# nmoehrle/mvs-texturing

Hardware: AMD Instinct MI355X
Metric: faces/sec through view-selection (data-cost + MRF) (higher is better)
Workload: dtype f32; 1 GPU; BASELINE config 3: displaced icosphere n=316 (1997120 faces), 200 Fibonacci-sphere views 2048x1536 RGB8, settings gmi/none/visibility-test (reference defaults); faces=1997120, views=200, nnz=88914367, sweeps=39, icm_iters=10, partition=library-hilbert-1, face_order_in=as built, msg_bits=8, max_labels=0

## Files before the change

include/mvs_viewsel_blocks.h:

```cpp
#ifndef MVS_VIEWSEL_BLOCKS_H
#define MVS_VIEWSEL_BLOCKS_H
#include "mvs_viewsel.h"
#ifdef __cplusplus
extern "C" {
#endif

mvs_status mvs_ctx_dc_get_max(mvs_ctx* ctx, float* dst_device);
mvs_status mvs_ctx_dc_set_max(mvs_ctx* ctx, const float* src_device);
mvs_status mvs_ctx_dc_get_histogram(mvs_ctx* ctx, uint32_t* dst_device);
mvs_status mvs_ctx_dc_set_histogram(mvs_ctx* ctx, const uint32_t* src_device);
mvs_status mvs_ctx_costs_export(mvs_ctx* ctx, uint32_t* counts_device, uint16_t* view_id_device, float* cost_device);

enum { MVS_MRF_MSG = 0, MVS_MRF_LAB = 1, MVS_MRF_GAIN = 2, MVS_MRF_BEST_LAB = 3,
       MVS_MRF_MSG_LAB = 4 };
mvs_status mvs_ctx_mrf_setup(mvs_ctx* ctx, const uint32_t* adj_ptr, const uint32_t* adj, int adj_on_device,
                             const mvs_mrf_params* params);
mvs_status mvs_ctx_mrf_sweep_phase(mvs_ctx* ctx, uint32_t phase, uint32_t node_begin, uint32_t node_end);
mvs_status mvs_ctx_mrf_setup_marked(mvs_ctx* ctx, const uint32_t* adj_ptr, const uint32_t* adj, int adj_on_device,
                                    const mvs_mrf_params* params, const uint8_t* marks_device);
mvs_status mvs_ctx_mrf_sweep_phase_part(mvs_ctx* ctx, uint32_t phase, uint32_t node_begin, uint32_t node_end, int part);
mvs_status mvs_ctx_mrf_sweep(mvs_ctx* ctx, uint32_t node_begin, uint32_t node_end);
mvs_status mvs_ctx_mrf_layout(mvs_ctx* ctx, uint32_t* in_off_host, uint64_t n_edges);
mvs_status mvs_ctx_mrf_gather(mvs_ctx* ctx, int which, const uint32_t* idx_device, uint64_t n, void* dst_device);
mvs_status mvs_ctx_mrf_scatter(mvs_ctx* ctx, int which, const uint32_t* idx_device, uint64_t n, const void* src_device);
mvs_status mvs_ctx_mrf_energy(mvs_ctx* ctx, int which_sel, uint32_t node_begin, uint32_t node_end, uint64_t* dst_device);
mvs_status mvs_ctx_mrf_keep_best(mvs_ctx* ctx);
mvs_status mvs_ctx_mrf_step(mvs_ctx* ctx, const uint64_t* energy_device);
mvs_status mvs_ctx_mrf_poll(mvs_ctx* ctx, uint32_t step, mvs_mrf_progress* out);
mvs_status mvs_ctx_mrf_icm_gain(mvs_ctx* ctx, uint32_t node_begin, uint32_t node_end);
mvs_status mvs_ctx_mrf_icm_apply(mvs_ctx* ctx, uint32_t node_begin, uint32_t node_end, uint32_t* moved_device);
mvs_status mvs_ctx_mrf_labels(mvs_ctx* ctx, uint32_t node_begin, uint32_t node_end, uint32_t* labels_device,
                              uint32_t* unseen_out);

#ifdef __cplusplus
}
#endif
#endif
```

mvs-texturing_amd/csrc/api.hip:

```cpp
#include "ctx.h"

#include <atomic>
#include <cmath>
#include <cstdio>
#include <cstdlib>
#include <cstring>
#include <chrono>
#include <mutex>
#include <string>
#include <thread>
#include <vector>

namespace mvs {
void dc_phase1(mvs_ctx* ctx, const mvs_settings* st);
void dc_phase2(mvs_ctx* ctx);
void dc_phase3(mvs_ctx* ctx, mvs_dc_stats* stats);
void undistort_image(mvs_ctx* ctx, const uint8_t* d_src, uint8_t* d_dst, int w, int h, double flen, double d0, double d1);
void dc_prune_labels(mvs_ctx* ctx, uint32_t kmax);
void dc_postprocess(mvs_ctx* ctx, uint32_t nf, uint32_t n_views, const uint32_t* h_ptr, const uint16_t* h_view_rev, const float* h_q_rev, const float* h_col_rev, const mvs_settings* st);
void mrf_setup(mvs_ctx* ctx, const mvs_mrf_params* params);
void mrf_sweep(mvs_ctx* ctx, uint32_t nb0, uint32_t ne0);
void mrf_energy(mvs_ctx* ctx, bool best, uint32_t nb0, uint32_t ne0, bool reduce = true);
void mrf_keep_best(mvs_ctx* ctx);
void mrf_exact_costs(mvs_ctx* ctx, uint32_t nb0, uint32_t ne0);
// ... 190 lines not shown
        for (unsigned k = 0; k < slots; ++k) {
            if (!buf[k]) MVS_HIP(hipHostMalloc((void**)&buf[k], SLOT, hipHostMallocPortable));
            if (!ev[k]) MVS_HIP(hipEventCreateWithFlags(&ev[k], hipEventDisableTiming));
        }
    }
    void release() {
        std::lock_guard<std::mutex> lock(m);
        for (unsigned k = 0; k < SLOTS; ++k) { if (ev[k]) (void)hipEventDestroy(ev[k]); if (buf[k]) (void)hipHostFree(buf[k]); ev[k] = nullptr; buf[k] = nullptr; used[k] = false; }
    }
};
constexpr int RING_DEVICES = 16;
UploadRing g_ring[RING_DEVICES];
unsigned upload_threads() {
    if (const char* e = getenv("MVS_UPLOAD_THREADS")) return (unsigned)std::max(1, std::min(atoi(e), (int)UploadRing::MAX_THREADS));
    return std::max(1u, std::min(UploadRing::MAX_THREADS, std::thread::hardware_concurrency() / 2));
}
void upload_through_ring(mvs_ctx* ctx, const std::vector<UploadPiece>& pieces) {
    if (ctx->device < 0 || ctx->device >= RING_DEVICES) throw StatusError(MVS_ERR_UNSUPPORTED, "upload ring: device index out of range");
    UploadRing& R = g_ring[ctx->device];
    std::lock_guard<std::mutex> lock(R.m);
    struct Chunk { const uint8_t* src; uint8_t* dst; size_t n; };
    std::vector<Chunk> chunks;
    for (const UploadPiece& p : pieces) for (size_t o = 0; o < p.bytes; o += UploadRing::SLOT) chunks.push_back(Chunk{p.src + o, p.dst + o, std::min(UploadRing::SLOT, p.bytes - o)});
    const unsigned T = (unsigned)std::max<size_t>(1, std::min<size_t>(upload_threads(), chunks.size()));
    R.ensure(2 * T);
    hipStream_t s = ctx->stream; const int device = ctx->device;
    struct Drain { hipStream_t s; UploadRing& R; ~Drain() { (void)hipStreamSynchronize(s); for (bool& u : R.used) u = false; } } drain{s, R};
    std::mutex em; std::string error; std::atomic<bool> failed{false};
    auto work = [&](unsigned t) {
        try {
            MVS_HIP(hipSetDevice(device));
            unsigned turn = 0;
            for (size_t c = t; c < chunks.size() && !failed.load(std::memory_order_relaxed); c += T, turn ^= 1u) {
                const unsigned k = 2 * t + turn;
                if (R.used[k]) MVS_HIP(hipEventSynchronize(R.ev[k]));
                memcpy(R.buf[k], chunks[c].src, chunks[c].n);
                MVS_HIP(hipMemcpyAsync(chunks[c].dst, R.buf[k], chunks[c].n, hipMemcpyHostToDevice, s));
                MVS_HIP(hipEventRecord(R.ev[k], s));
                R.used[k] = true;
            }
        } catch (const std::exception& e) { failed.store(true); std::lock_guard<std::mutex> l(em); if (error.empty()) error = e.what(); }
    };
    struct Joiner { std::vector<std::thread> th; ~Joiner() { for (auto& x : th) if (x.joinable()) x.join(); } } pool;
    pool.th.reserve(T);
    std::vector<unsigned> mine{0u};
    for (unsigned t = 1; t < T; ++t) {
        try { pool.th.emplace_back(work, t); } catch (const std::system_error&) { mine.push_back(t); }
    }
    for (unsigned t : mine) work(t);
    for (auto& x : pool.th) x.join();
    if (failed.load()) throw HipError("image upload: " + error);
}
}

extern "C" {

const char* mvs_last_error(void) { return g_last_error.c_str(); }

const char* mvs_status_string(mvs_status s) {
    switch (s) {
        case MVS_OK: return "ok";
        case MVS_ERR_INVALID: return "invalid argument";
        case MVS_ERR_TOO_MANY_FACES: return "Exeeded maximal number of faces";
        case MVS_ERR_TOO_MANY_VIEWS: return "Exeeded maximal number of views";
        case MVS_ERR_LABELING: return "Incorrect labeling";
        case MVS_ERR_HIP: return "HIP error";
        case MVS_ERR_STATE: return "invalid call order";
        case MVS_ERR_UNSUPPORTED: return "unsupported";
    }
    return "?";
}

void mvs_mrf_default_params(mvs_mrf_params* p) {
    p->max_sweeps = 200; p->min_sweeps = 20; p->window = 5; p->min_improvement = 0.005f;
    p->damping = 0.2f; p->rho = 0.8f; p->icm_iters = 50; p->region_rounds = 0;
}
void mvs_default_settings(mvs_settings* s) {
    s->data_term = MVS_DATA_TERM_GMI; s->outlier_removal = MVS_OUTLIER_NONE; s->geometric_visibility_test = 1;
}

mvs_status mvs_ctx_create(int device, mvs_ctx** out) {
    if (!out) return fail(MVS_ERR_INVALID, "out is null");
    *out = nullptr;
    MVS_API_BEGIN
    int n = 0;
    if (hipGetDeviceCount(&n) != hipSuccess || n <= 0) throw HipError("no HIP device available (this library has no CPU fallback)");
    if (device < 0 || device >= n) throw StatusError(MVS_ERR_INVALID, "bad device index");
    MVS_HIP(hipSetDevice(device));
    mvs_ctx* c = new mvs_ctx;
    c->device = device;
    MVS_HIP(hipStreamCreateWithFlags(&c->stream, hipStreamNonBlocking));
    c->own_stream = true;
    c->cos_limit = compute_cos_limit();
    if (const char* e = getenv("MVS_INFO_WAVE_AREA")) c->info_wave_area = std::max(0, atoi(e));
    if (const char* e = getenv("MVS_BVH_UPPER_MIN_FACES")) c->bvh_upper_min_faces = (uint32_t)std::max(0ll, atoll(e));
    c->counters.ensure(64);
    *out = c;
    MVS_API_END
}

void mvs_ctx_destroy(mvs_ctx* ctx) {
    if (!ctx) return;
    (void)hipSetDevice(ctx->device);
    (void)hipStreamSynchronize(ctx->stream);
    for (auto* b : ctx->own_rgb) delete b;
    mvs::gsl_release(ctx); mvs::texpatch_release(ctx); mvs::lsl_release(ctx);
    if (ctx->sweep_exec) (void)hipGraphExecDestroy(ctx->sweep_exec);
    if (ctx->cap_stream) (void)hipStreamDestroy(ctx->cap_stream);
    if (ctx->aux_stream) { (void)hipStreamSynchronize(ctx->aux_stream); (void)hipStreamDestroy(ctx->aux_stream); }
    if (ctx->ev_fork) (void)hipEventDestroy(ctx->ev_fork);
    if (ctx->ev_join) (void)hipEventDestroy(ctx->ev_join);
    if (ctx->h_kd_flags) (void)hipHostFree(ctx->h_kd_flags);
    if (ctx->h_icm) (void)hipHostFree(ctx->h_icm);
    if (ctx->h_rb) (void)hipHostFree(ctx->h_rb);
    if (ctx->h_seq) (void)hipHostFree(ctx->h_seq);
    if (ctx->h_ring) (void)hipHostFree(ctx->h_ring);
    if (ctx->own_stream && ctx->stream) (void)hipStreamDestroy(ctx->stream);
    delete ctx;
}

mvs_status mvs_ctx_set_stream(mvs_ctx* ctx, void* hip_stream) {
    if (!ctx) return fail(MVS_ERR_INVALID, "ctx is null");
    MVS_API_BEGIN
    MVS_HIP(hipStreamSynchronize(ctx->stream));
    if (ctx->own_stream && ctx->stream) MVS_HIP(hipStreamDestroy(ctx->stream));
    ctx->stream = (hipStream_t)hip_stream; ctx->own_stream = false;
    MVS_API_END
}

mvs_status mvs_ctx_synchronize(mvs_ctx* ctx) {
    if (!ctx) return fail(MVS_ERR_INVALID, "ctx is null");
    MVS_API_BEGIN
    MVS_HIP(hipStreamSynchronize(ctx->stream));
    MVS_API_END
}

mvs_status mvs_set_option(mvs_ctx* ctx, const char* name, int64_t value) {
    if (!ctx || !name) return fail(MVS_ERR_INVALID, "null argument");
    const std::string n(name);
    if (n == "count_rays") ctx->count_rays = value != 0;
    else if (n == "stats") ctx->stats = value != 0;
    else if (n == "verbose") ctx->verbose = value != 0;
    else if (n == "info_wave_area") ctx->info_wave_area = (int)std::max<int64_t>(0, std::min<int64_t>(value, 1 << 30));
    else if (n == "info_wave_area_words") ctx->info_wave_area_words = (int)std::max<int64_t>(1, std::min<int64_t>(value, 1 << 30));
    else if (n == "info_words") ctx->info_words = value != 0;
    else if (n == "info_cert_shift") ctx->info_cert_shift = (int)std::max<int64_t>(0, std::min<int64_t>(value, 40));
    else if (n == "max_labels") { if (value < 0 || value > 65535) return fail(MVS_ERR_INVALID, "max_labels: 0 (off) .. 65535"); ctx->max_labels = (int)value; }
    else if (n == "profile") ctx->profile = value != 0;
    else if (n == "prep_fused") ctx->prep_fused = value != 0;
    else if (n == "ray_xcd") ctx->ray_xcd = (int)value;
    else if (n == "mrf_xcd") ctx->mrf_xcd = (int)value;
    else if (n == "mrf_lag") ctx->mrf_lag = (int)value;
    else if (n == "mrf_force_generic") ctx->mrf_force_generic = value != 0;
    else if (n == "mrf_graph") ctx->mrf_graph = value != 0;
    else if (n == "mrf_blocks_per_cu") ctx->mrf_blocks_per_cu = std::max(0, (int)value);
    else if (n == "bvh_upper_min_faces") { ctx->kd_disabled = false; ctx->bvh_upper_min_faces = (uint32_t)std::max<int64_t>(0, std::min<int64_t>(value, 0xFFFFFFFFll)); ctx->order_pinned = false; }
    else if (n == "bvh_window") { ctx->kd_disabled = false; ctx->bvh_window = (uint32_t)std::max<int64_t>(0, std::min<int64_t>(value, 0x40000000)); ctx->order_pinned = false; }
    else if (n == "face_order") { ctx->face_order = value != 0 ? 1 : 0; ctx->order_pinned = false; }
    else return fail(MVS_ERR_INVALID, "unknown option " + n);
    return MVS_OK;
}

mvs_status mvs_ctx_get_profile(mvs_ctx* ctx, char* buf, size_t buf_size) {
    if (!ctx || !buf || buf_size < 3) return fail(MVS_ERR_INVALID, "null argument");
    MVS_API_BEGIN
    MVS_HIP(hipStreamSynchronize(ctx->stream));
    std::vector<std::string> names; std::vector<double> ms; std::vector<int> cnt;
    for (auto& sp : ctx->prof_spans) {
        float t = 0.0f;
        MVS_HIP(hipEventElapsedTime(&t, sp.a, sp.b));
        size_t k = 0;
        for (; k < names.size(); ++k) if (names[k] == sp.name) break;
        if (k == names.size()) { names.push_back(sp.name); ms.push_back(0.0); cnt.push_back(0); }
        ms[k] += t; cnt[k] += 1;
        if (sp.owns_a) ctx->prof_pool.push_back(sp.a);
        ctx->prof_pool.push_back(sp.b);
    }
    ctx->prof_spans.clear();
    std::string out = "{";
    for (size_t k = 0; k < names.size(); ++k) {
        char tmp[160];
        snprintf(tmp, sizeof(tmp), "%s\"%s\": [%.6f, %d]", k ? ", " : "", names[k].c_str(), ms[k], cnt[k]);
        out += tmp;
    }
    out += "}";
    if (out.size() + 1 > buf_size) throw StatusError(MVS_ERR_INVALID, "profile buffer too small");
    memcpy(buf, out.c_str(), out.size() + 1);
    MVS_API_END
}

mvs_status mvs_scene_set_mesh(mvs_ctx* ctx, const mvs_mesh* mesh, int on_device) {
    if (!ctx || !mesh || !mesh->verts || !mesh->faces || !mesh->face_normals) return fail(MVS_ERR_INVALID, "null argument");
    MVS_API_BEGIN
    MVS_HIP(hipSetDevice(ctx->device));
    const size_t NV = mesh->n_verts, F = mesh->n_faces;
    if (on_device) {
        ctx->d_verts = mesh->verts; ctx->d_faces = mesh->faces; ctx->d_normals = mesh->face_normals;
    } else {
        ctx->own_verts.ensure(3 * NV + 4); ctx->own_faces.ensure(3 * F + 4); ctx->own_normals.ensure(3 * F + 4);
        MVS_HIP(hipMemcpyAsync(ctx->own_verts.p, mesh->verts, 3 * NV * sizeof(float), hipMemcpyHostToDevice, ctx->stream));
        MVS_HIP(hipMemcpyAsync(ctx->own_faces.p, mesh->faces, 3 * F * sizeof(uint32_t), hipMemcpyHostToDevice, ctx->stream));
        MVS_HIP(hipMemcpyAsync(ctx->own_normals.p, mesh->face_normals, 3 * F * sizeof(float), hipMemcpyHostToDevice, ctx->stream));
        MVS_HIP(hipStreamSynchronize(ctx->stream));
        ctx->d_verts = ctx->own_verts.p; ctx->d_faces = ctx->own_faces.p; ctx->d_normals = ctx->own_normals.p;
    }
    ctx->n_verts = mesh->n_verts; ctx->n_faces = mesh->n_faces;
    ctx->face_begin = 0; ctx->face_end = mesh->n_faces;
    ctx->have_costs = false; ctx->dc_phase = 0;
    ctx->order_pinned = false; ctx->iv = nullptr; ctx->kd_disabled = false; ctx->kd_pending = 0;
    MVS_API_END
}

static mvs_status set_views_impl(mvs_ctx* ctx, const mvs_view* views, uint32_t n_views, int rgb_on_device, const mvs_image_source* src);
mvs_status mvs_scene_set_views(mvs_ctx* ctx, const mvs_view* views, uint32_t n_views, int rgb_on_device) { return set_views_impl(ctx, views, n_views, rgb_on_device, nullptr); }
mvs_status mvs_scene_set_views_from(mvs_ctx* ctx, const mvs_view* views, uint32_t n_views, const mvs_image_source* src) {
    if (!src || !src->acquire || !src->release) return fail(MVS_ERR_INVALID, "null argument");
    return set_views_impl(ctx, views, n_views, 0, src);
}
static mvs_status set_views_impl(mvs_ctx* ctx, const mvs_view* views, uint32_t n_views, int rgb_on_device, const mvs_image_source* src) {
    if (!ctx || (!views && n_views)) return fail(MVS_ERR_INVALID, "null argument");
    MVS_API_BEGIN
    MVS_HIP(hipSetDevice(ctx->device));
    if (rgb_on_device) { for (auto* b : ctx->own_rgb) delete b; ctx->own_rgb.clear(); }
    else { while (ctx->own_rgb.size() > n_views) { delete ctx->own_rgb.back(); ctx->own_rgb.pop_back(); } }
    ctx->h_views.assign(n_views, ViewParams{});
    struct Pinned {
        hipStream_t s; std::vector<void*> ptrs;
        ~Pinned() { if (ptrs.empty()) return; (void)hipStreamSynchronize(s); for (void* p : ptrs) (void)hipHostUnregister(p); }
    } pinned{ctx->stream, {}};
    UploadRoute route = rgb_on_device ? UploadRoute::Pageable : upload_route();
    if (src && route == UploadRoute::Register) route = UploadRoute::Ring;
    std::vector<UploadPiece> pieces;
    struct Held {
        const mvs_image_source* src; std::vector<uint32_t> views;
        void release_all() { for (uint32_t j : views) src->release(src->user, j); views.clear(); }
        ~Held() { if (src) release_all(); }
    } held{src, {}};
    const uint32_t in_flight = src ? std::max<uint32_t>(1u, src->max_in_flight ? src->max_in_flight : 4u) : 0u;
    auto flush_batch = [&]() {
        if (!pieces.empty()) upload_through_ring(ctx, pieces);
        pieces.clear();
        MVS_HIP(hipStreamSynchronize(ctx->stream));
        held.release_all();
    };
    for (uint32_t j = 0; j < n_views; ++j) {
        mvs_view v = views[j];
        if (src) {
            if (v.width < 2 || v.height < 2) throw StatusError(MVS_ERR_INVALID, "view " + std::to_string(j) + ": bad image");
            v.rgb = src->acquire(src->user, j);
            if (!v.rgb) throw StatusError(MVS_ERR_INVALID, "view " + std::to_string(j) + ": the image source has no image");
            held.views.push_back(j);
        }
        if (v.width < 2 || v.height < 2 || !v.rgb) throw StatusError(MVS_ERR_INVALID, "view " + std::to_string(j) + ": bad image");
        ViewParams& p = ctx->h_views[j];
        memcpy(p.pos, v.pos, sizeof(p.pos)); memcpy(p.viewdir, v.viewdir, sizeof(p.viewdir));
        memcpy(p.K, v.K, sizeof(p.K)); memcpy(p.w2c, v.w2c, sizeof(p.w2c));
        p.width = v.width; p.height = v.height;
        if (rgb_on_device) p.rgb = v.rgb;
        else {
            if (ctx->own_rgb.size() <= j) ctx->own_rgb.push_back(new DBuf<uint8_t>());
            auto* b = ctx->own_rgb[j];
            const size_t bytes = (size_t)v.width * v.height * 3;
            b->ensure(bytes + 16);
            p.rgb = b->p;
            if (route == UploadRoute::Ring && bytes >= (1u << 18)) { pieces.push_back(UploadPiece{v.rgb, b->p, bytes}); if (src && held.views.size() >= in_flight) flush_batch(); continue; }
            if (route == UploadRoute::Register && bytes >= (1u << 20) && hipHostRegister(const_cast<uint8_t*>(v.rgb), bytes, hipHostRegisterDefault) == hipSuccess) pinned.ptrs.push_back(const_cast<uint8_t*>(v.rgb));
            else (void)hipGetLastError();
            MVS_HIP(hipMemcpyAsync(b->p, v.rgb, bytes, hipMemcpyHostToDevice, ctx->stream));
            if (src && held.views.size() >= in_flight) flush_batch();
        }
    }
    if (src) flush_batch();
    if (!pieces.empty()) upload_through_ring(ctx, pieces);
    MVS_HIP(hipStreamSynchronize(ctx->stream));
    ctx->n_views = n_views;
    ctx->have_costs = false; ctx->dc_phase = 0;
    MVS_API_END
}

mvs_status mvs_scene_set_face_range(mvs_ctx* ctx, uint32_t begin, uint32_t end) {
    if (!ctx) return fail(MVS_ERR_INVALID, "ctx is null");
    if (begin > end || end > ctx->n_faces) return fail(MVS_ERR_INVALID, "bad face range");
    ctx->face_begin = begin; ctx->face_end = end;
    ctx->have_costs = false; ctx->dc_phase = 0;
    return MVS_OK;
}

mvs_status mvs_ctx_dc_phase1(mvs_ctx* ctx, const mvs_settings* settings) {
    if (!ctx || !settings) return fail(MVS_ERR_INVALID, "null argument");
    MVS_API_BEGIN
    MVS_HIP(hipSetDevice(ctx->device));
    dc_phase1(ctx, settings);
    MVS_API_END
}
mvs_status mvs_ctx_dc_phase2(mvs_ctx* ctx) {
    if (!ctx) return fail(MVS_ERR_INVALID, "ctx is null");
    MVS_API_BEGIN
    MVS_HIP(hipSetDevice(ctx->device));
    dc_phase2(ctx);
    MVS_API_END
}
mvs_status mvs_ctx_dc_phase3(mvs_ctx* ctx, mvs_dc_stats* stats) {
    if (!ctx) return fail(MVS_ERR_INVALID, "ctx is null");
    MVS_API_BEGIN
    MVS_HIP(hipSetDevice(ctx->device));
    dc_phase3(ctx, stats);
// ... 496 lines not shown
```

mvs-texturing_amd/csrc/ctx.h:

```cpp
#pragma once
#include <hip/hip_runtime.h>
#include <stdint.h>
#include <string.h>
#include <algorithm>
#include <functional>
#include <stdexcept>
#include <string>
#include <vector>

#include "../../include/mvs_viewsel.h"
#include "dmath.h"

namespace mvs {

struct HipError : std::runtime_error {
    explicit HipError(const std::string& m) : std::runtime_error(m) {}
};
struct StatusError : std::runtime_error {
    mvs_status st;
    StatusError(mvs_status s, const std::string& m) : std::runtime_error(m), st(s) {}
};

#define MVS_HIP(expr)                                                                          \
    do {                                                                                       \
// ... 48 lines not shown
    uint32_t pad_[7];
    __host__ __device__ float lo(int a, int c) const { return b[c][a]; }
    __host__ __device__ float hi(int a, int c) const { return b[c][3 + a]; }
};
static_assert(sizeof(Node4) == 128, "Node4 must be one 128-byte line");

struct BvhDev {
    const Node4* nodes;
    const float4* tris;
    uint32_t level_off[16];
    uint32_t level_cnt[16];
    int32_t top;
    uint32_t n_leaves;
};

struct ProfSpan { std::string name; hipEvent_t a, b; bool owns_a; };

struct MrfEdge {
    uint32_t in_off;
    uint32_t out_off;
    uint32_t kj;
};

struct alignas(16) NodeDesc {
    uint32_t rec;
    uint32_t id;
    uint32_t in_off[3];
    uint32_t out_off[3];
    uint32_t kk;
    uint32_t nbr[3];
};
static_assert(sizeof(NodeDesc) == 48, "NodeDesc must be 48 bytes");

struct GslDev;
struct TexPatchDev;
struct LslDev;

struct PatchTables {
    DBuf<int4> box; DBuf<float2> pc;
    DBuf<uint32_t> fcand, fidx, parent, off, len, alive, pscan, cand_pid, cand_pos, fpid, fpos, flags;
    DBuf<unsigned long long> merged; DBuf<ViewParams> views;
    uint32_t C = 0, n_patches = 0; uint64_t n_merged = 0;
};

}

struct mvs_ctx {
    int device = 0;
    hipStream_t stream = nullptr;
    bool own_stream = false;
    bool verbose = false;
    bool profile = false;
    std::vector<mvs::ProfSpan> prof_spans; std::vector<hipEvent_t> prof_pool;
    bool prep_fused = true;
    bool stats = false;
    bool count_rays = false;
    uint32_t* h_kd_flags = nullptr; int kd_pending = 0; bool kd_disabled = false;
    uint32_t* h_rb = nullptr; uint32_t* d_rb = nullptr; uint32_t rb_seq = 0;
    hipStream_t aux_stream = nullptr; hipEvent_t ev_fork = nullptr, ev_join = nullptr;
    uint32_t bvh_upper_min_faces = 1000000;
    uint32_t bvh_window = 262144;
    mvs::DBuf<float> kd_c[2][3]; mvs::DBuf<uint32_t> kd_id[2], kd_hist, kd_cursor, kd_tie, kd_pivot, kd_box;
    int ray_xcd = 1;
    int info_wave_area = 32;
    int info_wave_area_words = 384;
    bool info_words = true;
    int info_cert_shift = 0;
    uint32_t dc_stats_deferred = 0;
    int max_labels = 0;
    float cos_limit = 0.0f;

    uint32_t n_verts = 0, n_faces = 0, n_views = 0;
    uint32_t face_begin = 0, face_end = 0;
    const float* d_verts = nullptr; const uint32_t* d_faces = nullptr; const float* d_normals = nullptr;
    mvs::DBuf<float> own_verts, own_normals; mvs::DBuf<uint32_t> own_faces;
    std::vector<mvs::ViewParams> h_views;
    mvs::DBuf<mvs::ViewParams> d_views;
    std::vector<mvs::DBuf<uint8_t>*> own_rgb;
    mvs::DBuf<uint8_t> gmi_all;
    mvs::DBuf<uint8_t> lum_all;
    mvs::DBuf<uint32_t> mask_all;
    mvs::DBuf<uint32_t> mask_zero, mask_tmp;
    mvs::DBuf<uint32_t> msum_all;
    std::vector<size_t> gmi_off, mask_off, msum_off;
    mvs::DBuf<size_t> view_off;
    bool mesh_dirty = true, views_dirty = true;

    int face_order = 1;
    mvs::DBuf<float> i_verts, i_normals; mvs::DBuf<uint32_t> i_faces, f_perm, f_pos, f_tmp;
    const float* iv = nullptr; const uint32_t* ifc = nullptr; const float* inr = nullptr;
    bool mesh_ordered = false;
    bool order_pinned = false;
    const uint32_t* t_perm = nullptr; const uint32_t* t_pos = nullptr;
    mvs::DBuf<uint32_t> u_ptr, u_cnt; mvs::DBuf<uint16_t> u_view; mvs::DBuf<float> u_cost, u_q;
    bool u_valid = false, u_q_valid = false;
    mvs::DBuf<unsigned long long> fp_acc;
    mvs::HBuf<uint32_t> stage_ptr; mvs::HBuf<uint16_t> stage_view[2]; mvs::HBuf<float> stage_cost[2];

    mvs::DBuf<mvs::Node4> bvh_nodes; mvs::DBuf<float4> bvh_tris;
    mvs::DBuf<uint32_t> sort_k, sort_k2, sort_v, sort_v2; mvs::DBuf<char> sort_tmp;
    mvs::DBuf<float> lvl_box_a, lvl_box_b; mvs::DBuf<float> scene_box;
    mvs::BvhDev bvh{};
    mvs::DBuf<uint32_t> vf_ptr, vf_cursor, vf;
    mvs::DBuf<uint32_t> vperm, vpos;
    const uint32_t* tri_order = nullptr;

    mvs::DBuf<unsigned long long> pass_bits, need_bits, occl_bits, surv_bits;
    mvs::DBuf<uint32_t> pass_base;
    mvs::DBuf<uint32_t> pass_face;
    mvs::DBuf<unsigned long long> defer_bits; mvs::DBuf<uint32_t> defer_base; mvs::DBuf<uint2> defer_list; mvs::DBuf<uint32_t> rewalk_list;
    mvs::DBuf<float> pq;
    mvs::DBuf<float> pcol;
    mvs::DBuf<uint32_t> face_cnt, scan_tmp;
    mvs::DBuf<unsigned long long> counters;
    mvs::DBuf<float> max_q; mvs::DBuf<uint32_t> hist; mvs::DBuf<float> pctl;
    mvs::DBuf<uint32_t> pre_ptr; mvs::DBuf<uint16_t> pre_view; mvs::DBuf<float> pre_q; mvs::DBuf<float> pre_col;
    mvs::DBuf<uint8_t> pre_inl;
    mvs::DBuf<uint32_t> csr_ptr; mvs::DBuf<uint16_t> csr_view; mvs::DBuf<float> csr_cost; mvs::DBuf<float> csr_q;
    uint32_t csr_faces = 0, csr_views = 0; uint64_t csr_nnz = 0;
    const uint32_t* r_ptr = nullptr; const uint16_t* r_view = nullptr; const float* r_cost = nullptr;
    bool csr_q_valid = false;
    bool have_costs = false;
    mvs_settings dc_settings{}; mvs_dc_stats dc_stats{}; int dc_phase = 0;

    mvs::DBuf<unsigned long long> g_keys, g_keys2; mvs::DBuf<uint32_t> g_vals, g_vals2, g_pos, g_cnt, g_adj_ptr, g_adj, g_faces; mvs::DBuf<float> g_normals;
    uint64_t g_adj_entries = 0; bool have_adj = false;

    mvs::DBuf<uint32_t> p_label_ptr, p_comp_ptr, p_comp_faces, p_parent, p_root, p_state, p_flag, p_pos, p_roots, p_roots2, p_rlab, p_rlab2, p_adj_ptr, p_adj, p_labels;

    mvs::GslDev* gsl = nullptr; mvs::TexPatchDev* texpatch = nullptr; mvs::LslDev* lsl = nullptr;

    mvs::DBuf<uint32_t> rg_parent, rg_root, rg_size, rg_bestl, rg_lose, rg_flag, rg_pos, rg_cstart, rg_have, rg_cfirst, rg_name;
    mvs::DBuf<unsigned long long> rg_gain, rg_cur, rg_key, rg_key2, rg_ck, rg_sum; mvs::DBuf<long long> rg_cgain; mvs::DBuf<uint2> rg_cut;

    mvs::DBuf<uint32_t> m_adj_ptr, m_adj, a_stage_ptr, a_stage; const uint32_t* r_adj_ptr = nullptr; const uint32_t* r_adj = nullptr;
    uint32_t r_adj_edges = 0; bool r_adj_edges_known = false;
    mvs::DBuf<mvs::NodeDesc> m_desc; mvs::DBuf<uint8_t> m_ident; mvs::DBuf<uint32_t> m_rec; uint64_t m_rec_words = 0; int mrf_blocks_per_cu = 0 , mrf_xcd = 1;
    mvs::DBuf<mvs::MrfEdge> m_edge; mvs::DBuf<uint32_t> m_size, m_rev ; mvs::DBuf<uint16_t> m_map;
    mvs::DBuf<uint8_t> m_msg_a;
    mvs::DBuf<uint32_t> m_sel, m_sel2, m_cand; mvs::DBuf<float> m_gain;
    mvs::DBuf<uint32_t> m_lab; mvs::DBuf<float> m_cost;
    uint32_t m_stride = 0;
    bool exact_valid = false; uint32_t exact_nb = 0, exact_ne = 0;
    uint32_t* b_sel = nullptr; uint32_t* b_lab = nullptr; float* b_cost = nullptr; bool best_resolved = false;
    mvs::DBuf<unsigned long long> m_energy; mvs::DBuf<uint32_t> m_moved; mvs::DBuf<uint32_t> m_alist; bool icm_dirty_valid = false;
    uint32_t m_n_adj = 0;
    uint32_t m_energy_blocks = 0;
    bool m_energy_from_sweep = false;
    uint64_t m_total = 0; uint32_t m_kmax = 0, m_degmax = 0;
    mvs::DBuf<uint32_t> m_colour, m_perm, m_tmp_a, m_tmp_b, m_tmp_c, m_sub; mvs::DBuf<uint8_t> m_cls; uint32_t m_colours = 0, m_n_fast = 0; std::vector<uint32_t> m_sub_begin;
    const uint32_t* m_colour_in = nullptr;
    const uint8_t* m_bnd = nullptr;
    int mrf_force_generic = 0;
    uint32_t m_range_nb = 0, m_range_ne = 0; std::vector<uint32_t> m_range_q;
    uint32_t m_sweep_no = 0;
    mvs_mrf_params m_params{};
    static constexpr uint32_t RING = 16;
    static constexpr uint32_t ICM_RING = 8;
    uint32_t* h_icm = nullptr; uint32_t* d_icm = nullptr; uint32_t icm_seq = 0;
    mvs::DBuf<mvs_mrf_progress> m_state; mvs::DBuf<unsigned long long> m_hist; mvs::DBuf<uint32_t> m_ctl;
    int mrf_graph = 1; hipStream_t cap_stream = nullptr; hipGraphExec_t sweep_exec = nullptr; uint32_t graph_launches = 0, graph_updates = 0, graph_instantiations = 0;
    mvs_mrf_progress* h_ring = nullptr; mvs_mrf_progress* d_ring = nullptr ; uint32_t steps_issued = 0; int mrf_lag = 1;
    uint32_t* h_seq = nullptr; uint32_t* d_seq = nullptr; uint32_t seq_base = 0;
};

namespace mvs {
struct Prof {
    mvs_ctx* c; size_t idx; bool on;
    Prof(mvs_ctx* ctx, const char* name) : c(ctx), idx(0), on(ctx->profile) {
        if (!on) return;
        auto get = [&]() { hipEvent_t e; if (!c->prof_pool.empty()) { e = c->prof_pool.back(); c->prof_pool.pop_back(); } else { MVS_HIP(hipEventCreate(&e)); } return e; };
        ProfSpan sp{name, get(), get(), true};
        MVS_HIP(hipEventRecord(sp.a, c->stream));
        idx = c->prof_spans.size(); c->prof_spans.push_back(sp);
    }
    void end() { if (on) { MVS_HIP(hipEventRecord(c->prof_spans[idx].b, c->stream)); on = false; } }
    ~Prof() { if (on) (void)hipEventRecord(c->prof_spans[idx].b, c->stream); }
};
struct ProfChain {
    mvs_ctx* c; hipEvent_t prev; bool on;
    static hipEvent_t get(mvs_ctx* c) { hipEvent_t e; if (!c->prof_pool.empty()) { e = c->prof_pool.back(); c->prof_pool.pop_back(); } else { MVS_HIP(hipEventCreate(&e)); } return e; }
    explicit ProfChain(mvs_ctx* ctx) : c(ctx), prev(nullptr), on(ctx->profile) {}
    void begin() { if (on && !prev) { prev = get(c); MVS_HIP(hipEventRecord(prev, c->stream)); first = true; } }
    void mark(const char* name) {
        if (!on) return;
        begin();
        hipEvent_t e = get(c);
        MVS_HIP(hipEventRecord(e, c->stream));
        c->prof_spans.push_back(ProfSpan{name, prev, e, first});
        first = false; prev = e;
    }
    bool first = false;
};
struct RoctxRange { explicit RoctxRange(const char* name); ~RoctxRange(); bool on; };
int default_device();
enum { MRF_PART_ALL = 0, MRF_PART_BOUNDARY = 1, MRF_PART_INTERIOR = 2 };
void ensure_report_ring(mvs_ctx* ctx);
void report_u32(mvs_ctx* ctx, const uint32_t* d_src, uint32_t* d_dst, uint32_t seq_slot, uint32_t seq);
void wait_report(mvs_ctx* ctx, uint32_t seq_slot, uint32_t seq);
int icm_rounds(mvs_ctx* ctx, int max_rounds, const uint32_t* d_moved, const std::function<void(int)>& round);
constexpr uint32_t MRF_DAMP_PERIOD = 4;
void read_words(mvs_ctx* ctx, const void* d_src, void* out, uint32_t n_words);
void read_block(mvs_ctx* ctx, const void* d_src, void* out, size_t bytes);
void exclusive_scan_u32(mvs_ctx* ctx, const uint32_t* in, uint32_t* out, size_t n, uint32_t* d_total);
uint64_t sum_u32(mvs_ctx* ctx, const uint32_t* in, size_t n);
void gsl_release(mvs_ctx* ctx);
void texpatch_release(mvs_ctx* ctx);
void lsl_release(mvs_ctx* ctx);
void patch_check_inputs(mvs_ctx* ctx, PatchTables& T, const uint32_t* d_labels, const char* who);
void build_patch_tables(mvs_ctx* ctx, PatchTables& T, const uint32_t* d_adj_ptr, const uint32_t* d_adj, const uint32_t* d_labels, const char* who);
}
```

mvs-texturing_amd/csrc/dmath.h:

```cpp
#pragma once
#include <stdint.h>
#include <math.h>
#include <float.h>
#include <string.h>

#if defined(__HIPCC__)
#define MVS_HD __host__ __device__ __forceinline__
#else
#define MVS_HD inline
#endif

namespace mvs {

struct V3 { float x, y, z; };
struct V2 { float x, y; };

MVS_HD V3 operator+(V3 a, V3 b) { return {a.x + b.x, a.y + b.y, a.z + b.z}; }
MVS_HD V3 operator-(V3 a, V3 b) { return {a.x - b.x, a.y - b.y, a.z - b.z}; }
MVS_HD V3 operator/(V3 a, float s) { return {a.x / s, a.y / s, a.z / s}; }
MVS_HD float dot(V3 a, V3 b) { return (a.x * b.x + a.y * b.y) + a.z * b.z; }
MVS_HD float norm(V3 a) { return sqrtf(dot(a, a)); }
MVS_HD V3 normalized(V3 a) { return a / norm(a); }
MVS_HD V3 cross(V3 a, V3 b) {
    return {a.y * b.z - a.z * b.y, a.z * b.x - a.x * b.z, a.x * b.y - a.y * b.x};
// ... 250 lines not shown
    if (DATA_TERM == 1) {
        if (num_samples > 0) {
            gmi = foot_gmi_term(gmi, num_samples, s.area);
        } else {
            const double g1 = (double)linear_at(gimg, w, h, 1, s.p1.x, s.p1.y, 0) / 255.0;
            const double g2 = (double)linear_at(gimg, w, h, 1, s.p2.x, s.p2.y, 0) / 255.0;
            const double g3 = (double)linear_at(gimg, w, h, 1, s.p3.x, s.p3.y, 0) / 255.0;
            gmi = (((g1 + g2) + g3) / 3.0) * (double)s.area;
        }
    }
    if (OUTLIER) {
        if (num_samples > 0) {
            out->mean_color[0] = foot_mean(col0, num_samples);
            out->mean_color[1] = foot_mean(col1, num_samples);
            out->mean_color[2] = foot_mean(col2, num_samples);
        } else {
            for (int i = 0; i < 3; ++i) {
                const double c1 = (double)linear_at(image, w, h, 3, s.p1.x, s.p1.y, i) / 255.0;
                const double c2 = (double)linear_at(image, w, h, 3, s.p2.x, s.p2.y, i) / 255.0;
                const double c3 = (double)linear_at(image, w, h, 3, s.p3.x, s.p3.y, i) / 255.0;
                out->mean_color[i] = (float)(((c1 + c2) + c3) / 3.0);
            }
        }
    }
    out->quality = (DATA_TERM == 0) ? s.area : (float)gmi;
}

MVS_HD bool foot_value_certified(double q, double dn, double up) { return (float)(q * dn) == (float)(q * up); }
template <int DATA_TERM, bool OUTLIER>
MVS_HD bool foot_sums_certified(const FootSetup& s, uint32_t num_samples, double col0, double col1, double col2, double gmi, int shift) {
    if (num_samples == 0) return true;
    const double eps = ldexp((double)((num_samples + 13u) & ~1u), -53 + shift), dn = 1.0 - eps, up = 1.0 + eps;
    bool ok = true;
    if (DATA_TERM == 1) ok = foot_value_certified(foot_gmi_term(gmi, num_samples, s.area), dn, up);
    if (OUTLIER) ok = ok && foot_value_certified(col0 / (double)num_samples, dn, up) && foot_value_certified(col1 / (double)num_samples, dn, up) &&
                      foot_value_certified(col2 / (double)num_samples, dn, up);
    return ok;
}

MVS_HD uint32_t bytes_sum4(uint32_t v, uint32_t acc) {
#if defined(__HIP_DEVICE_COMPILE__)
    return __builtin_amdgcn_sad_u8(v, 0u, acc);
#else
    return acc + (v & 0xFFu) + ((v >> 8) & 0xFFu) + ((v >> 16) & 0xFFu) + (v >> 24);
#endif
}
template <int ROWS = 2>
MVS_HD void foot_walk_gmi_words(const ViewParams& view, const FootSetup& s, uint32_t* num_samples, uint32_t* gmi_sum) {
    const uint8_t* gimg = view.gmi;
    const int w = view.width;
    uint32_t n = 0, g = 0;
    const int y_end = (int)ceilf(s.aabb_max_y);
    for (int y = (int)floorf(s.aabb_min_y); y < y_end; y += ROWS) {
        int xb[ROWS], xe[ROWS], x0[ROWS];
        const uint8_t* row0 = gimg + (size_t)y * w;
        bool more = false;
#pragma unroll
        for (int r = 0; r < ROWS; ++r) {
            if (y + r >= y_end || !foot_row(s, y + r, &xb[r], &xe[r]) || xe[r] <= xb[r]) { xb[r] = 0; xe[r] = 0; }
            x0[r] = xb[r] - (int)(reinterpret_cast<uintptr_t>(row0 + r * w + xb[r]) & 3u);
            if (xe[r] <= xb[r]) x0[r] = xe[r];
            more = more || x0[r] < xe[r];
        }
        while (more) {
            uint32_t v[ROWS];
#pragma unroll
            for (int r = 0; r < ROWS; ++r) v[r] = (x0[r] < xe[r]) ? *reinterpret_cast<const uint32_t*>(row0 + r * w + x0[r]) : 0u;
            more = false;
#pragma unroll
            for (int r = 0; r < ROWS; ++r) {
                if (x0[r] < xe[r]) {
                    const int lo = xb[r] > x0[r] ? xb[r] - x0[r] : 0, hi = xe[r] - x0[r] < 4 ? xe[r] - x0[r] : 4;
                    const uint32_t m = (hi >= 4 ? 0xFFFFFFFFu : ((1u << (8 * hi)) - 1u)) & ~((1u << (8 * lo)) - 1u);
                    g = bytes_sum4(v[r] & m, g);
                    n += (uint32_t)(hi - lo);
                }
                x0[r] += 4;
                more = more || x0[r] < xe[r];
            }
        }
    }
    *num_samples = n; *gmi_sum = g;
}
MVS_HD bool foot_words_fit(const FootSetup& s) {
    return ((s.aabb_max_y - s.aabb_min_y) + 2.0f) * ((s.aabb_max_x - s.aabb_min_x) + 2.0f) < 16777216.0f;
}

constexpr float FOOT_DEFERRED = -1.0f;

template <int DATA_TERM, bool OUTLIER>
MVS_HD void face_info(const ViewParams& view, V3 v1, V3 v2, V3 v3, FaceInfoOut* out, float defer_area = INFINITY,
                      const double* u8_over_255 = nullptr ) {
    FootSetup s;
    foot_setup(view, v1, v2, v3, s);
    out->quality = 0.0f;
    out->mean_color[0] = out->mean_color[1] = out->mean_color[2] = 0.0f;
    if (s.area < FLT_EPSILON) return;

    uint32_t num_samples = 0;
    double col0 = 0.0, col1 = 0.0, col2 = 0.0, gmi = 0.0;
    const int w = view.width;
    const uint8_t* image = view.rgb;
    const uint8_t* gimg = view.gmi;
    const bool sampling_necessary = (DATA_TERM != 0) || OUTLIER;

    if (sampling_necessary && s.area > 0.5f) {
        if (s.area > defer_area) { out->quality = FOOT_DEFERRED; return; }
        foot_edges(s);
        const float y_end = ceilf(s.aabb_max_y);
        for (int y = (int)floorf(s.aabb_min_y); (float)y < y_end; ++y) {
            int xb, xe;
            if (!foot_row(s, y, &xb, &xe)) continue;
            for (int x = xb; x < xe; ++x) {
                if (!s.fast && !foot_inside(s, x, y)) continue;
                const size_t pix = (size_t)x + (size_t)y * w;
                if (OUTLIER) {
                    const uint8_t c0 = image[pix * 3 + 0], c1 = image[pix * 3 + 1], c2 = image[pix * 3 + 2];
                    col0 += u8_over_255 ? u8_over_255[c0] : (double)c0 / 255.0;
                    col1 += u8_over_255 ? u8_over_255[c1] : (double)c1 / 255.0;
                    col2 += u8_over_255 ? u8_over_255[c2] : (double)c2 / 255.0;
                }
                if (DATA_TERM == 1) { const uint8_t g = gimg[pix]; gmi += u8_over_255 ? u8_over_255[g] : (double)g / 255.0; }
                ++num_samples;
            }
        }
    }
    foot_finish<DATA_TERM, OUTLIER>(view, s, num_samples, col0, col1, col2, gmi, out);
}

MVS_HD void rgb_to_ycbcr(float* v) {
    const float r = v[0], g = v[1], b = v[2];
    v[0] = r * 0.299f + g * 0.587f + b * 0.114f;
    v[1] = r * -0.168736f + g * -0.331264f + b * 0.5f + 0.5f;
    v[2] = r * 0.5f + g * -0.418688f + b * -0.081312f + 0.5f;
}

MVS_HD uint8_t luminance_u8(uint8_t r, uint8_t g, uint8_t b) {
    return (uint8_t)(0.30 * (double)r + (double)(0.59f * (float)g) + (double)(0.11f * (float)b));
}
MVS_HD uint8_t isqrt_clamp255(int n) {
    const float m = (float)(n < 255 * 255 ? n : 255 * 255) + 0.5f;
#if defined(__HIP_DEVICE_COMPILE__)
    return (uint8_t)(int)__builtin_amdgcn_sqrtf(m);
#else
    return (uint8_t)(int)sqrtf(m);
#endif
}

MVS_HD uint32_t hist_bin(float value, float maxv, uint32_t num_bins) {
    const float clamped = smax(0.0f, smin(maxv, value));
    return (uint32_t)floorf(((clamped - 0.0f) / (maxv - 0.0f)) * (float)(num_bins - 1));
}

inline float host_cos_limit() {
    const double limit = 75.0f * (3.14159265358979323846264338327950288 / 180.0);
    auto f = [](uint32_t u) { float x; memcpy(&x, &u, 4); return x; };
    auto culled = [&](uint32_t u) { return (double)acosf(f(u)) > limit; };
    uint32_t lo = 0x3E000000u , hi = 0x3F000000u ;
    while (hi - lo > 1) { const uint32_t mid = lo + (hi - lo) / 2; if (culled(mid)) lo = mid; else hi = mid; }
    for (uint32_t k = 1; k <= 4096; ++k) if (!culled(hi - k) || culled(hi + k - 1)) return NAN;
    return f(hi);
}

}
```

mvs-texturing_amd/csrc/dmath_host.cpp:

```cpp
#include "dmath.h"
#include <vector>
#include <cstring>

using namespace mvs;

extern "C" {

struct dmh_view {
    float pos[3], viewdir[3], K[9], w2c[16];
    int32_t width, height;
    const uint8_t* rgb;
    const uint8_t* gmi;
    const uint32_t* mask;
};

static ViewParams to_vp(const dmh_view* v) {
    ViewParams p;
    memcpy(p.pos, v->pos, sizeof(p.pos)); memcpy(p.viewdir, v->viewdir, sizeof(p.viewdir));
    memcpy(p.K, v->K, sizeof(p.K)); memcpy(p.w2c, v->w2c, sizeof(p.w2c));
    p.width = v->width; p.height = v->height; p.mask_stride = (v->width + 31) / 32;
    p.rgb = v->rgb; p.gmi = v->gmi; p.mask = v->mask; p.msum = nullptr; p.msum_stride = 0;
    return p;
}

float dmh_cos_limit(void) { return host_cos_limit(); }

void dmh_cull_all(const dmh_view* views, uint32_t n_views, const float* verts, const uint32_t* faces, const float* normals,
                  uint32_t n_faces, float cos_limit, int8_t* reasons) {
    for (uint32_t j = 0; j < n_views; ++j) {
        const ViewParams vp = to_vp(views + j);
        for (uint32_t f = 0; f < n_faces; ++f) {
            const uint32_t* fv = faces + 3 * (size_t)f;
            const V3 v1 = {verts[3 * fv[0]], verts[3 * fv[0] + 1], verts[3 * fv[0] + 2]};
            const V3 v2 = {verts[3 * fv[1]], verts[3 * fv[1] + 1], verts[3 * fv[1] + 2]};
            const V3 v3 = {verts[3 * fv[2]], verts[3 * fv[2] + 1], verts[3 * fv[2] + 2]};
            const V3 n = {normals[3 * f], normals[3 * f + 1], normals[3 * f + 2]};
            reasons[(size_t)f * n_views + j] = (int8_t)cull_pair(vp, v1, v2, v3, n, cos_limit);
        }
    }
}

void dmh_cull_pairs(const dmh_view* base, uint32_t n, const float* pos, const float* viewdir, const float* tri9, const float* normal,
                    float cos_limit, int8_t* out) {
    for (uint32_t i = 0; i < n; ++i) {
        ViewParams vp = to_vp(base);
        for (int a = 0; a < 3; ++a) { vp.pos[a] = pos[3 * i + a]; vp.viewdir[a] = viewdir[3 * i + a]; }
        const float* t = tri9 + 9 * (size_t)i;
        const V3 v1 = {t[0], t[1], t[2]}, v2 = {t[3], t[4], t[5]}, v3 = {t[6], t[7], t[8]}, nr = {normal[3 * i], normal[3 * i + 1], normal[3 * i + 2]};
        const V3 centre = ((v1 + v2) + v3) / 3.0f;
        out[2 * i] = (int8_t)cull_pair(vp, v1, v2, v3, nr, cos_limit);
        out[2 * i + 1] = (int8_t)cull_pair_prefiltered(vp, v1, v2, v3, nr, centre, cos_limit);
    }
}

void dmh_face_info(const dmh_view* view, int data_term, int outlier, const float* v1, const float* v2, const float* v3,
                   float* quality, float* ycbcr) {
    const ViewParams vp = to_vp(view);
    FaceInfoOut fi;
    const V3 a = {v1[0], v1[1], v1[2]}, b = {v2[0], v2[1], v2[2]}, c = {v3[0], v3[1], v3[2]};
    if (data_term == 1) { if (outlier) face_info<1, true>(vp, a, b, c, &fi); else face_info<1, false>(vp, a, b, c, &fi); }
    else { if (outlier) face_info<0, true>(vp, a, b, c, &fi); else face_info<0, false>(vp, a, b, c, &fi); }
    *quality = fi.quality;
    if (outlier) rgb_to_ycbcr(fi.mean_color);
    ycbcr[0] = fi.mean_color[0]; ycbcr[1] = fi.mean_color[1]; ycbcr[2] = fi.mean_color[2];
}

int dmh_ray_any_hit(const float* verts, const uint32_t* faces, uint32_t n_faces, uint32_t n_verts, const float* origin, const float* view_pos) {
    float lo[3] = {INFINITY, INFINITY, INFINITY}, hi[3] = {-INFINITY, -INFINITY, -INFINITY};
    for (uint32_t v = 0; v < n_verts; ++v)
        for (int a = 0; a < 3; ++a) { lo[a] = fminf(lo[a], verts[3 * (size_t)v + a]); hi[a] = fmaxf(hi[a], verts[3 * (size_t)v + a]); }
    const Ray r = make_ray(V3{origin[0], origin[1], origin[2]}, V3{view_pos[0], view_pos[1], view_pos[2]}, scene_pad(lo, hi));
    for (uint32_t f = 0; f < n_faces; ++f) {
        const uint32_t* fv = faces + 3 * (size_t)f;
        const V3 a = {verts[3 * fv[0]], verts[3 * fv[0] + 1], verts[3 * fv[0] + 2]};
        const V3 b = {verts[3 * fv[1]], verts[3 * fv[1] + 1], verts[3 * fv[1] + 2]};
        const V3 c = {verts[3 * fv[2]], verts[3 * fv[2] + 1], verts[3 * fv[2] + 2]};
        if (ray_tri(r, a, b - a, c - a)) return 1;
    }
    return 0;
}

void dmh_gradient_magnitude(const uint8_t* rgb, int w, int h, uint8_t* gmi) {
    for (int y = 0; y < h; ++y)
        for (int x = 0; x < w; ++x) {
            if (y == 0 || y == h - 1 || x == 0 || x == w - 1) { gmi[(size_t)y * w + x] = 0; continue; }
            int l[3][3];
            for (int dy = -1; dy <= 1; ++dy)
                for (int dx = -1; dx <= 1; ++dx) {
                    const uint8_t* p = rgb + ((size_t)(y + dy) * w + (x + dx)) * 3;
                    l[dy + 1][dx + 1] = luminance_u8(p[0], p[1], p[2]);
                }
            const int sx = (l[0][2] - l[0][0]) + 2 * (l[1][2] - l[1][0]) + (l[2][2] - l[2][0]);
            const int sy = (l[2][0] - l[0][0]) + 2 * (l[2][1] - l[0][1]) + (l[2][2] - l[0][2]);
            gmi[(size_t)y * w + x] = isqrt_clamp255(sx * sx + sy * sy);
        }
}

uint32_t dmh_hist_bin(float value, float maxv) { return hist_bin(value, maxv, 10000u); }

void dmh_foot_cert_trials(uint64_t seed, uint32_t trials, uint32_t max_n, int shift, uint64_t* out) {
    uint64_t n_cert = 0, n_mis = 0, n_bad = 0;
#pragma omp parallel for schedule(dynamic, 64) reduction(+ : n_cert, n_mis, n_bad)
    for (uint32_t t = 0; t < trials; ++t) {
        uint64_t x = seed * 0x9E3779B97F4A7C15ull + (uint64_t)t * 0xD1B54A32D192ED03ull + 1ull;
        auto rnd = [&]() { x ^= x << 13; x ^= x >> 7; x ^= x << 17; return x; };
        const uint32_t n = 33u + (uint32_t)(rnd() % (max_n - 32u));
        const uint32_t lo = (uint32_t)(rnd() % 200u), span = 1u + (uint32_t)(rnd() % (256u - lo));
        std::vector<uint8_t> px(4 * (size_t)n);
        for (auto& p : px) p = (uint8_t)(lo + rnd() % span);
        FootSetup s{}; s.area = 0.5f * (float)n * (0.8f + 0.4f * (float)(rnd() % 1000u) / 1000.0f);
        uint64_t S[4] = {0, 0, 0, 0};
        for (uint32_t k = 0; k < n; ++k) for (int c = 0; c < 4; ++c) S[c] += px[4 * (size_t)k + c];
        const double C[4] = {(double)S[0] / 255.0, (double)S[1] / 255.0, (double)S[2] / 255.0, (double)S[3] / 255.0};
        const bool cert = foot_sums_certified<1, true>(s, n, C[0], C[1], C[2], C[3], shift);
        const float qi = (float)foot_gmi_term(C[3], n, s.area), m0 = foot_mean(C[0], n), m1 = foot_mean(C[1], n), m2 = foot_mean(C[2], n);
        bool mis = false;
        for (int order = 0; order < 3; ++order) {
            double a[4] = {0.0, 0.0, 0.0, 0.0};
            for (uint32_t k = 0; k < n; ++k) {
                const uint32_t i = order == 0 ? k : order == 1 ? n - 1 - k : (uint32_t)(((uint64_t)k * 7919u) % n);
                for (int c = 0; c < 4; ++c) a[c] += (double)px[4 * (size_t)i + c] / 255.0;
            }
            mis = mis || (float)foot_gmi_term(a[3], n, s.area) != qi || foot_mean(a[0], n) != m0 || foot_mean(a[1], n) != m1 || foot_mean(a[2], n) != m2;
        }
        n_cert += cert; n_mis += mis; n_bad += (cert && mis);
    }
    out[0] = n_cert; out[1] = n_mis; out[2] = n_bad; out[3] = trials;
}

uint64_t dmh_isqrt_mismatches(uint32_t n_max) {
    uint64_t bad = 0;
    uint32_t k = 0;
    for (uint32_t n = 0; n < n_max; ++n) {
        while ((uint64_t)(k + 1) * (k + 1) <= n) ++k;
        bad += isqrt_clamp255((int)n) != (uint8_t)(k < 255u ? k : 255u);
    }
    return bad;
}

void dmh_word_walk_trials(uint64_t seed, uint32_t trials, uint64_t* out) {
    uint64_t n_fast = 0, n_bad = 0, n_px = 0, n_over = 0;
#pragma omp parallel for schedule(dynamic, 64) reduction(+ : n_fast, n_bad, n_px, n_over)
    for (uint32_t t = 0; t < trials; ++t) {
        uint64_t x = seed * 0x9E3779B97F4A7C15ull + (uint64_t)t * 0xD1B54A32D192ED03ull + 1ull;
        auto rnd = [&]() { x ^= x << 13; x ^= x >> 7; x ^= x << 17; return x; };
        auto unit = [&]() { return (float)(rnd() % 1000003u) / 1000003.0f; };
        const int w = 33 + (int)(rnd() % 90u), h = 20 + (int)(rnd() % 60u);
        std::vector<uint8_t> buf((size_t)w * h + 16);
        for (auto& b : buf) b = (uint8_t)(rnd() >> 11);
        ViewParams vp; memset(&vp, 0, sizeof(vp));
        vp.width = w; vp.height = h; vp.gmi = buf.data() + 8;
        FootSetup s{};
        const float cx = 2.0f + unit() * (float)(w - 4), cy = 2.0f + unit() * (float)(h - 4), r = 0.6f + unit() * unit() * 30.0f;
        auto clampf = [](float v, float lo, float hi) { return v < lo ? lo : (v > hi ? hi : v); };
        V2* p[3] = {&s.p1, &s.p2, &s.p3};
        for (int k = 0; k < 3; ++k) { p[k]->x = clampf(cx + (2.0f * unit() - 1.0f) * r, 0.0f, (float)w - 1.01f); p[k]->y = clampf(cy + (2.0f * unit() - 1.0f) * r, 0.0f, (float)h - 1.01f); }
        foot_setup_px(s);
        if (s.area <= 0.5f) continue;
        foot_edges(s);
        if (!s.fast) continue;
        uint32_t n0 = 0, g0 = 0;
        const float y_end = ceilf(s.aabb_max_y);
        for (int y = (int)floorf(s.aabb_min_y); (float)y < y_end; ++y) {
            int xb, xe;
            if (!foot_row(s, y, &xb, &xe)) continue;
            for (int xx = xb; xx < xe; ++xx) { g0 += vp.gmi[(size_t)xx + (size_t)y * w]; ++n0; }
        }
        uint32_t n[3], g[3];
        foot_walk_gmi_words<2>(vp, s, &n[0], &g[0]); foot_walk_gmi_words<3>(vp, s, &n[1], &g[1]); foot_walk_gmi_words<4>(vp, s, &n[2], &g[2]);
        ++n_fast; n_px += n0;
        for (int k = 0; k < 3; ++k) n_bad += (n[k] != n0 || g[k] != g0);
        n_over += (double)n0 > ((double)s.aabb_max_y - s.aabb_min_y + 2.0) * ((double)s.aabb_max_x - s.aabb_min_x + 2.0);
    }
    out[0] = n_fast; out[1] = n_bad; out[2] = n_px; out[3] = n_over;
}

}
```

mvs-texturing_amd/csrc/k_mrf.hip:

```cpp
#include "ctx.h"
#include <rocprim/rocprim.hpp>
#include <atomic>

namespace mvs {

namespace {

constexpr uint16_t MAP_NONE = 0xFFFF;
constexpr uint32_t MSG_BASE = MVS_MRF_MSG_BASE;

typedef uint8_t msg_t;
struct MsgQ { float scale, step; };
__device__ __forceinline__ MsgQ msg_q(float lam) { return MsgQ{255.0f / lam, lam / 255.0f}; }
template <class T> __device__ __forceinline__ T ld_off(const void* base, uint32_t byte_off) { return *reinterpret_cast<const T*>(reinterpret_cast<const char*>(base) + byte_off); }
template <class T> __device__ __forceinline__ void st_off(void* base, uint32_t byte_off, T v) { *reinterpret_cast<T*>(reinterpret_cast<char*>(base) + byte_off) = v; }
__device__ __forceinline__ float min_raw(float a, float b) { float r; asm("v_min_f32 %0, %1, %2" : "=v"(r) : "v"(a), "v"(b)); return r; }
template <bool DAMP>
__device__ __forceinline__ uint32_t msg_pack_s(float raw_s, float alpha, float old_code, uint32_t byte, uint32_t word) {
    return __builtin_amdgcn_cvt_pk_u8_f32(DAMP ? __builtin_fmaf(old_code, alpha, raw_s) : raw_s, byte, word);
}
template <bool DAMP>
__device__ __forceinline__ uint32_t msg_pack(float raw, float oms, float alpha, float old_code, uint32_t byte, uint32_t word) {
    const float v = DAMP ? __builtin_fmaf(old_code, alpha, raw * oms) : raw * oms;
    return __builtin_amdgcn_cvt_pk_u8_f32(v, byte, word);
// ... 105 lines not shown
                                uint32_t* __restrict__ maxes , uint32_t* __restrict__ rev) {
    const uint32_t i = blockIdx.x * blockDim.x + threadIdx.x;
    uint32_t k = 0, deg = 0;
    if (i < F) {
        k = col_ptr[i + 1] - col_ptr[i];
        const uint32_t e0 = adj_ptr[i], e1 = adj_ptr[i + 1];
        deg = e1 - e0;
        uint32_t kmx = k;
        for (uint32_t eb = e0; eb < e1; eb += 4) {
            uint32_t j[4], kj[4], r0[4], r1[4], head[4][4];
#pragma unroll
            for (int q = 0; q < 4; ++q) j[q] = (eb + q < e1) ? adj[eb + q] : i;
#pragma unroll
            for (int q = 0; q < 4; ++q) { kj[q] = col_ptr[j[q] + 1] - col_ptr[j[q]]; r0[q] = adj_ptr[j[q]]; r1[q] = adj_ptr[j[q] + 1]; }
#pragma unroll
            for (int q = 0; q < 4; ++q)
#pragma unroll
                for (int t = 0; t < 4; ++t) head[q][t] = (r0[q] + t < r1[q]) ? adj[r0[q] + t] : 0xFFFFFFFFu;
#pragma unroll
            for (int q = 0; q < 4; ++q) {
                if (eb + q >= e1) continue;
                const uint32_t e = eb + q;
                size[e] = (k > 0 && kj[q] > 0) ? ((k + pad_mask) & ~pad_mask) : 0u;
                if (k > 0) kmx = max(kmx, kj[q]);
                uint32_t r = 0xFFFFFFFFu;
#pragma unroll
                for (int t = 3; t >= 0; --t) r = (head[q][t] == i) ? r0[q] + t : r;
                if (r == 0xFFFFFFFFu) { uint32_t rr = r0[q] + 4u; while (rr < r1[q] && adj[rr] != i) ++rr; if (rr < r1[q]) r = rr; }
                rev[e] = r;
            }
        }
        cls[i] = (uint8_t)mrf_node_class(kmx, deg, force_generic);
    }
    for (int o = 32; o > 0; o >>= 1) { k = max(k, (uint32_t)__shfl_xor(k, o, 64)); deg = max(deg, (uint32_t)__shfl_xor(deg, o, 64)); }
    if ((threadIdx.x & 63) == 0) {
        if (k > __hip_atomic_load(&maxes[0], __ATOMIC_RELAXED, __HIP_MEMORY_SCOPE_AGENT)) atomicMax(&maxes[0], k);
        if (deg > __hip_atomic_load(&maxes[1], __ATOMIC_RELAXED, __HIP_MEMORY_SCOPE_AGENT)) atomicMax(&maxes[1], deg);
    }
}

__device__ __forceinline__ uint32_t mrf_hash32(uint32_t x) { x ^= x >> 16; x *= 0x7feb352dU; x ^= x >> 15; x *= 0x846ca68bU; x ^= x >> 16; return x; }
__device__ __forceinline__ bool mrf_key_less(uint32_t a, uint32_t b) { const uint32_t ha = mrf_hash32(a), hb = mrf_hash32(b); return ha != hb ? ha < hb : a < b; }
constexpr uint32_t NO_COLOUR = 0xFFFFFFFFu;
__global__ void mrf_colour_init_kernel(uint32_t* __restrict__ colour, uint32_t* __restrict__ iota, uint32_t F) {
    const uint32_t i = blockIdx.x * blockDim.x + threadIdx.x;
    if (i < F) { colour[i] = NO_COLOUR; iota[i] = i; }
}
__global__ void mrf_colour_round_kernel(const uint32_t* __restrict__ adj_ptr, const uint32_t* __restrict__ adj, const uint32_t* __restrict__ orig, uint32_t F,
                                        uint32_t* colour, uint32_t* __restrict__ pending) {
    const uint32_t i = blockIdx.x * blockDim.x + threadIdx.x;
    if (i >= F) return;
    if (__hip_atomic_load(colour + i, __ATOMIC_RELAXED, __HIP_MEMORY_SCOPE_AGENT) != NO_COLOUR) return;
    unsigned long long used = 0ull;
    bool ready = true;
    const uint32_t oi = orig ? orig[i] : i;
    const uint32_t e0 = adj_ptr[i], e1 = adj_ptr[i + 1];
    for (uint32_t eb = e0; eb < e1 && ready; eb += 4) {
        uint32_t j[4], oj[4], cj[4];
#pragma unroll
        for (int t = 0; t < 4; ++t) j[t] = (eb + t < e1) ? adj[eb + t] : i;
#pragma unroll
        for (int t = 0; t < 4; ++t) { oj[t] = orig ? orig[j[t]] : j[t]; cj[t] = __hip_atomic_load(colour + j[t], __ATOMIC_RELAXED, __HIP_MEMORY_SCOPE_AGENT); }
#pragma unroll
        for (int t = 0; t < 4; ++t) {
            if (j[t] == i || !mrf_key_less(oj[t], oi)) continue;
            if (cj[t] == NO_COLOUR) ready = false; else used |= 1ull << cj[t];
        }
    }
    if (ready) {
        if (used == ~0ull) { pending[1] = 1u; used = 0ull; }
        __hip_atomic_store(colour + i, (uint32_t)__builtin_ctzll(~used), __ATOMIC_RELAXED, __HIP_MEMORY_SCOPE_AGENT);
    } else *pending = 1u;
}
constexpr uint32_t N_SUB = 320;
constexpr uint32_t SUB_GENERIC = 256;
constexpr uint32_t N_KEY = 2 * N_SUB;
__global__ void mrf_sortkey_kernel(const uint32_t* __restrict__ colour, const uint8_t* __restrict__ cls, const uint8_t* __restrict__ bnd, uint32_t F, uint32_t* __restrict__ key) {
    const uint32_t i = blockIdx.x * blockDim.x + threadIdx.x;
    if (i < F) { const uint32_t c = colour[i], k = cls[i]; key[i] = 2u * ((k == CLS_GENERIC) ? SUB_GENERIC + c : 4u * c + k) + ((bnd && bnd[i]) ? 0u : 1u); }
}
__global__ void mrf_sub_begin_kernel(const uint32_t* __restrict__ sorted, uint32_t F, uint32_t* __restrict__ sub_begin) {
    const uint32_t c = blockIdx.x * blockDim.x + threadIdx.x;
    if (c > N_KEY) return;
    uint32_t lo = 0, hi = F;
    while (lo < hi) { const uint32_t mid = (lo + hi) >> 1; if (sorted[mid] < c) lo = mid + 1; else hi = mid; }
    sub_begin[c] = lo;
}
__global__ void mrf_sub_range_kernel(const uint32_t* __restrict__ perm, const uint32_t* __restrict__ sub_begin,
                                     uint32_t nb, uint32_t ne, uint32_t* __restrict__ out) {
    const uint32_t c = blockIdx.x * blockDim.x + threadIdx.x;
    if (c >= N_KEY) return;
    const uint32_t cb = sub_begin[c], ce = sub_begin[c + 1];
    uint32_t lo = cb, hi = ce;
    while (lo < hi) { const uint32_t mid = (lo + hi) >> 1; if (perm[mid] < nb) lo = mid + 1; else hi = mid; }
    out[2 * c] = lo;
    hi = ce;
    while (lo < hi) { const uint32_t mid = (lo + hi) >> 1; if (perm[mid] < ne) lo = mid + 1; else hi = mid; }
    out[2 * c + 1] = lo;
}
constexpr int MAX_LAYOUT_COLOURS = 8;
__global__ void mrf_nodesize_kernel(const uint32_t* __restrict__ perm, const uint32_t* __restrict__ colour, const uint32_t* __restrict__ adj_ptr,
                                    const uint32_t* __restrict__ adj, const uint32_t* __restrict__ size, const uint32_t* __restrict__ rev, uint32_t F, uint32_t n_col,
                                    uint32_t* __restrict__ nsz) {
    const uint32_t q = blockIdx.x * blockDim.x + threadIdx.x;
    if (q > F) return;
    uint32_t acc[MAX_LAYOUT_COLOURS];
#pragma unroll
    for (int b = 0; b < MAX_LAYOUT_COLOURS; ++b) acc[b] = 0;
    if (q < F) {
        const uint32_t j = perm[q];
        const uint32_t ra = adj_ptr[j], rz = adj_ptr[j + 1];
        for (uint32_t rb = ra; rb < rz; rb += 4) {
            uint32_t i[4], e[4], b[4], sz[4];
#pragma unroll
            for (int t = 0; t < 4; ++t) { const bool on = rb + t < rz; i[t] = on ? adj[rb + t] : j; e[t] = on ? rev[rb + t] : 0xFFFFFFFFu; }
#pragma unroll
            for (int t = 0; t < 4; ++t) { b[t] = (n_col > 1) ? colour[i[t]] : 0u; sz[t] = (e[t] != 0xFFFFFFFFu) ? size[e[t]] : 0u; }
#pragma unroll
            for (int t = 0; t < 4; ++t)
#pragma unroll
                for (int c = 0; c < MAX_LAYOUT_COLOURS; ++c) acc[c] += ((uint32_t)c == b[t]) ? sz[t] : 0u;
        }
    }
#pragma unroll
    for (int b = 0; b < MAX_LAYOUT_COLOURS; ++b) if ((uint32_t)b < n_col) nsz[(size_t)b * (F + 1) + q] = acc[b];
}
__global__ void mrf_inoff_kernel(const uint32_t* __restrict__ perm, const uint32_t* __restrict__ colour, const uint32_t* __restrict__ adj_ptr,
                                 const uint32_t* __restrict__ adj, const uint32_t* __restrict__ size, const uint32_t* __restrict__ rev, const uint32_t* __restrict__ noff,
                                 uint32_t F, uint32_t n_col, uint32_t* __restrict__ in_off) {
    const uint32_t q = blockIdx.x * blockDim.x + threadIdx.x;
    if (q >= F) return;
    const uint32_t j = perm[q];
    uint32_t off[MAX_LAYOUT_COLOURS];
#pragma unroll
    for (int b = 0; b < MAX_LAYOUT_COLOURS; ++b) off[b] = ((uint32_t)b < n_col) ? noff[(size_t)b * (F + 1) + q] : 0u;
    const uint32_t ra = adj_ptr[j], rz = adj_ptr[j + 1];
    for (uint32_t rb = ra; rb < rz; rb += 4) {
        uint32_t i[4], e[4], b[4], sz[4];
#pragma unroll
        for (int t = 0; t < 4; ++t) { const bool on = rb + t < rz; i[t] = on ? adj[rb + t] : j; e[t] = on ? rev[rb + t] : 0xFFFFFFFFu; }
#pragma unroll
        for (int t = 0; t < 4; ++t) { b[t] = (n_col > 1) ? colour[i[t]] : 0u; sz[t] = (e[t] != 0xFFFFFFFFu) ? size[e[t]] : 0u; }
#pragma unroll
        for (int t = 0; t < 4; ++t) {
            if (e[t] == 0xFFFFFFFFu) continue;
            uint32_t o = 0;
#pragma unroll
            for (int c = 0; c < MAX_LAYOUT_COLOURS; ++c) { if ((uint32_t)c == b[t]) { o = off[c]; off[c] += sz[t]; } }
            in_off[e[t]] = o;
        }
    }
}

__global__ void mrf_edge_kernel(const uint32_t* __restrict__ col_ptr, const uint32_t* __restrict__ adj_ptr, const uint32_t* __restrict__ adj,
                                uint32_t F, const uint32_t* __restrict__ in_off, const uint32_t* __restrict__ size, const uint32_t* __restrict__ rev, MrfEdge* __restrict__ edge) {
    const uint32_t i = blockIdx.x * blockDim.x + threadIdx.x;
    if (i >= F) return;
    const uint32_t e0 = adj_ptr[i], e1 = adj_ptr[i + 1];
    for (uint32_t eb = e0; eb < e1; eb += 4) {
        uint32_t j[4], r[4], io[4], sz[4], oo[4], kj[4];
#pragma unroll
        for (int t = 0; t < 4; ++t) { const bool on = eb + t < e1; j[t] = on ? adj[eb + t] : i; r[t] = on ? rev[eb + t] : 0xFFFFFFFFu; io[t] = on ? in_off[eb + t] : 0u; sz[t] = on ? size[eb + t] : 0u; }
#pragma unroll
        for (int t = 0; t < 4; ++t) { oo[t] = (r[t] != 0xFFFFFFFFu) ? in_off[r[t]] : 0u; kj[t] = col_ptr[j[t] + 1] - col_ptr[j[t]]; }
#pragma unroll
        for (int t = 0; t < 4; ++t) {
            if (eb + t >= e1) continue;
            const bool has = r[t] != 0xFFFFFFFFu;
            MrfEdge m;
            m.in_off = MSG_BASE + io[t];
            m.out_off = has ? MSG_BASE + oo[t] : 0u;
            m.kj = (sz[t] > 0 && has) ? kj[t] : 0u;
            edge[eb + t] = m;
        }
    }
}

constexpr uint32_t MAP_TILE = 256;
__global__ void __launch_bounds__(256) mrf_map_kernel(const uint32_t* __restrict__ col_ptr, const uint16_t* __restrict__ view_id, const uint32_t* __restrict__ adj_ptr,
                               const uint32_t* __restrict__ adj, uint32_t F, const MrfEdge* __restrict__ edge, const uint8_t* __restrict__ cls, uint16_t* __restrict__ map) {
    __shared__ uint16_t s_l[16][MAP_TILE];
    const uint32_t i = (blockIdx.x * blockDim.x + threadIdx.x) >> 4;
    const uint32_t gl = threadIdx.x & 15;
    if (i >= F) return;
    uint16_t* tile = s_l[threadIdx.x >> 4];
    const uint32_t p0 = col_ptr[i], K = col_ptr[i + 1] - p0;
    for (uint32_t e = adj_ptr[i]; e < adj_ptr[i + 1]; ++e) {
        const MrfEdge m = edge[e];
        if (m.kj == 0 || cls[adj[e]] != CLS_GENERIC) continue;
        const uint32_t q0 = col_ptr[adj[e]];
        const bool in_lds = m.kj <= MAP_TILE;
        if (in_lds) for (uint32_t t = gl; t < m.kj; t += 16) tile[t] = view_id[q0 + t];
        for (uint32_t t = gl; t < K; t += 16) {
            const uint16_t key = view_id[p0 + t];
            uint32_t lo = 0, hi = m.kj;
            if (in_lds) { while (lo < hi) { const uint32_t mid = (lo + hi) >> 1; if (tile[mid] < key) lo = mid + 1; else hi = mid; } }
            else { while (lo < hi) { const uint32_t mid = (lo + hi) >> 1; if (view_id[q0 + mid] < key) lo = mid + 1; else hi = mid; } }
            const uint16_t found = (lo < m.kj) ? (in_lds ? tile[lo] : view_id[q0 + lo]) : (uint16_t)0;
            map[m.in_off + t] = (lo < m.kj && found == key) ? (uint16_t)lo : MAP_NONE;
        }
    }
}

constexpr uint32_t REC_BASE = 256;
constexpr float COST_SCALE = 65535.0f;
__device__ __forceinline__ uint32_t cost_code(float c) { return (uint32_t)(c * COST_SCALE + 0.5f); }
__device__ __forceinline__ float cost_value(uint32_t code) { return (float)code * (1.0f / 65535.0f); }
__device__ __forceinline__ uint32_t label_position(const uint16_t* __restrict__ view_id, uint32_t p0, uint32_t K, uint32_t l) {
    uint32_t lo = 0, hi = K;
    const uint32_t key = l - 1u;
    while (lo < hi) { const uint32_t mid = (lo + hi) >> 1; if ((uint32_t)view_id[p0 + mid] < key) lo = mid + 1; else hi = mid; }
    return lo < K ? lo : K - 1u;
}

__global__ void __launch_bounds__(256) mrf_ident_kernel(const uint32_t* __restrict__ col_ptr, const uint16_t* __restrict__ view_id, const uint32_t* __restrict__ adj_ptr,
                                                        const uint32_t* __restrict__ adj, uint32_t F, const MrfEdge* __restrict__ edge, const uint8_t* __restrict__ cls,
                                                        uint8_t* __restrict__ ident) {
    const uint32_t i = (blockIdx.x * blockDim.x + threadIdx.x) >> 4;
    const uint32_t gl = threadIdx.x & 15;
    if (i >= F || cls[i] == CLS_GENERIC) return;
    const uint32_t p0 = col_ptr[i], K = col_ptr[i + 1] - p0;
    const uint32_t e0 = adj_ptr[i], e1 = adj_ptr[i + 1];
    for (uint32_t e = e0; e < e1; e += 3) {
        uint32_t kj[3], q0[3];
#pragma unroll
        for (int k = 0; k < 3; ++k) {
            const bool on = e + k < e1;
            kj[k] = on ? edge[e + k].kj : 0u;
            q0[k] = col_ptr[on ? adj[e + k] : i];
        }
        uint32_t same = 0;
#pragma unroll
        for (int k = 0; k < 3; ++k) same |= (kj[k] != 0u && kj[k] == K) ? (1u << k) : 0u;
        if (same) {
            for (uint32_t t = gl; t < K; t += 16) {
                const uint32_t v = view_id[p0 + t];
#pragma unroll
                for (int k = 0; k < 3; ++k)
                    if ((same >> k) & 1u) { if (view_id[q0[k] + t] != v) same &= ~(1u << k); }
            }
            for (int o = 8; o > 0; o >>= 1) same &= __shfl_xor(same, o, 16);
        }
        if (gl < 3 && e + gl < e1 && kj[gl] != 0u) ident[e + gl] = (uint8_t)((same >> gl) & 1u);
    }
}
__global__ void mrf_recsize_kernel(const uint32_t* __restrict__ col_ptr, const uint32_t* __restrict__ adj_ptr, const MrfEdge* __restrict__ edge,
                                   const uint8_t* __restrict__ ident, const uint8_t* __restrict__ cls, const uint32_t* __restrict__ perm, uint32_t F,
                                   uint32_t* __restrict__ rsz, uint32_t* __restrict__ qpos) {
    const uint32_t q = blockIdx.x * blockDim.x + threadIdx.x;
    if (q > F) return;
    uint32_t w = 0;
    if (q < F) {
        const uint32_t i = perm[q], K = col_ptr[i + 1] - col_ptr[i];
        qpos[i] = q;
        if (K && cls[i] != CLS_GENERIC) {
            w = (K + 3u) & ~3u;
            const bool w8 = cls[i] == 1u;
            const uint32_t e0 = adj_ptr[i], e1 = adj_ptr[i + 1];
            for (uint32_t eb = e0; eb < e1; eb += 4) {
                uint32_t kj[4], id[4];
#pragma unroll
                for (int t = 0; t < 4; ++t) { const bool on = eb + t < e1; kj[t] = on ? edge[eb + t].kj : 0u; id[t] = on ? ident[eb + t] : 1u; }
#pragma unroll
                for (int t = 0; t < 4; ++t) if (kj[t] && !id[t]) w += w8 ? 2u * ((kj[t] + 7u) >> 3) : (kj[t] + 3u) >> 2;
            }
            w = (w + 3u) & ~3u;
        }
    }
    rsz[q] = w;
}
__global__ void __launch_bounds__(256) mrf_record_kernel(const uint32_t* __restrict__ col_ptr, const uint16_t* __restrict__ view_id, const float* __restrict__ cost,
                                                         const uint32_t* __restrict__ adj_ptr, const uint32_t* __restrict__ adj, const MrfEdge* __restrict__ edge,
                                                         const uint8_t* __restrict__ ident, const uint8_t* __restrict__ cls, const uint32_t* __restrict__ qpos, const uint32_t* __restrict__ roff,
                                                         uint32_t F, uint32_t* __restrict__ rec) {
    __shared__ uint16_t s_l[16][256];
    const uint32_t i = (blockIdx.x * blockDim.x + threadIdx.x) >> 4;
    const uint32_t gl = threadIdx.x & 15;
    if (i >= F) return;
    const uint32_t p0 = col_ptr[i], K = col_ptr[i + 1] - p0;
    const uint32_t ci = cls[i];
    if (K == 0 || ci == CLS_GENERIC) return;
    const bool w8 = ci == 1u;
    const uint32_t rs = w8 ? 8u : 8u << ci, none_byte = w8 ? 64u : (ci < 3u ? 4u * rs : 0xFFu);
    const uint32_t lmask = w8 ? 7u : 3u, lshift = w8 ? 3u : 2u;
    const uint32_t q = qpos[i];
    uint16_t* tile = s_l[threadIdx.x >> 4];
    uint32_t* out = rec + REC_BASE + roff[q];
    const uint32_t K4 = (K + 3u) & ~3u;
    const uint32_t e0 = adj_ptr[i], deg = adj_ptr[i + 1] - e0;
    uint32_t kj3[3], q03[3];
    {
        uint32_t kj[3], idn[3], nb[3];
#pragma unroll
        for (uint32_t d = 0; d < 3; ++d) { const bool on = d < deg; kj[d] = on ? edge[e0 + d].kj : 0u; idn[d] = on ? (uint32_t)ident[e0 + d] : 1u; nb[d] = on ? adj[e0 + d] : i; }
#pragma unroll
        for (uint32_t d = 0; d < 3; ++d) { kj3[d] = (kj[d] != 0u && idn[d] == 0u) ? kj[d] : 0u; q03[d] = col_ptr[nb[d]]; }
    }
    for (uint32_t t = gl; t < K4; t += 16) {
        uint32_t w = 0u;
        if (t < K) { const uint32_t v = view_id[p0 + t]; tile[t] = (uint16_t)v; w = (cost_code(cost[p0 + t]) << 16) | v; }
        out[t] = w;
    }
    uint32_t pos = K4;
#pragma unroll
    for (uint32_t d = 0; d < 3; ++d) {
        const uint32_t kj = kj3[d];
        if (kj == 0) continue;
        const uint32_t q0 = q03[d], nw = w8 ? 2u * ((kj + 7u) >> 3) : (kj + 3u) >> 2;
        for (uint32_t wI = gl; wI < nw; wI += 16) {
            uint32_t key[4], lo[4] = {0u, 0u, 0u, 0u};
#pragma unroll
            for (uint32_t r = 0; r < 4; ++r) { const uint32_t t2 = 4u * wI + r; key[r] = (t2 < kj) ? (uint32_t)view_id[q0 + t2] : 0xFFFFFFFFu; }
            for (uint32_t n = K; n > 1u;) {
                const uint32_t half = n >> 1;
#pragma unroll
                for (uint32_t r = 0; r < 4; ++r) lo[r] += ((uint32_t)tile[lo[r] + half - 1u] < key[r]) ? half : 0u;
                n -= half;
            }
            uint32_t word = 0u;
#pragma unroll
            for (uint32_t r = 0; r < 4; ++r) {
                uint32_t at = lo[r] + (((uint32_t)tile[lo[r]] < key[r]) ? 1u : 0u);
                const uint32_t byte = (at < K && (uint32_t)tile[at < K ? at : 0u] == key[r]) ? (at & lmask) * rs + (at >> lshift) : none_byte;
                word |= byte << (8 * r);
            }
            out[pos + wI] = word;
        }
        pos += nw;
    }
    for (uint32_t t = pos + gl; t < ((pos + 3u) & ~3u); t += 16) out[t] = 0u;
}
__global__ void mrf_desc_kernel(const uint32_t* __restrict__ col_ptr, const uint32_t* __restrict__ adj_ptr, const uint32_t* __restrict__ adj,
                                const MrfEdge* __restrict__ edge, const uint8_t* __restrict__ ident, const uint32_t* __restrict__ perm,
                                const uint32_t* __restrict__ colour, const uint32_t* __restrict__ roff, uint32_t n_fast, NodeDesc* __restrict__ desc) {
    const uint32_t q = blockIdx.x * blockDim.x + threadIdx.x;
    if (q >= n_fast) return;
    const uint32_t i = perm[q];
    NodeDesc nd;
    const uint32_t k = col_ptr[i + 1] - col_ptr[i];
    nd.rec = k ? REC_BASE + roff[q] : 0u; nd.id = i; nd.kk = k;
    const uint32_t e0 = adj_ptr[i], deg = adj_ptr[i + 1] - e0, ci = colour[i];
    for (int d = 0; d < 3; ++d) {
        MrfEdge m; m.in_off = 0; m.out_off = 0; m.kj = 0;
        uint32_t flag_ident = 0, flag_low = 0, nb = i;
        if ((uint32_t)d < deg) { nb = adj[e0 + d]; flag_low = (colour[nb] < ci) ? 1u : 0u; }
        if ((uint32_t)d < deg && k > 0) {
            m = edge[e0 + d];
            if (m.kj && ident[e0 + d]) flag_ident = 1u;
            if (m.kj == 0) { m.in_off = 0; m.out_off = 0; }
        }
        nd.in_off[d] = m.in_off | flag_low; nd.out_off[d] = m.out_off | flag_ident; nd.kk |= m.kj << (8 + 8 * d); nd.nbr[d] = nb;
    }
    desc[q] = nd;
}

template <int G, bool DAMP, bool XCD>
__global__ void __launch_bounds__(256) mrf_sweep4_kernel(const NodeDesc* __restrict__ desc, const uint32_t* __restrict__ rec, msg_t* msg,
                                                         const mvs_mrf_progress* __restrict__ st, uint32_t* lab2, uint32_t buf_stride,
                                                         uint32_t node_begin , uint32_t node_end, float rho, float alpha,
                                                         unsigned long long* __restrict__ partial) {
    const msg_t* mo = msg; msg_t* mn = msg;
    constexpr int NPB = 256 / G;
    constexpr int TS = G == 8 ? 40 : 4 * G + 4;
    __shared__ float s_c[NPB * TS];
    __shared__ unsigned long long s_e[8];
    const int grp = threadIdx.x / G, gl = threadIdx.x % G;
    float* __restrict__ tile = s_c + grp * TS;
    if (st->stopped) return;
    if (gl == 0) tile[4 * G] = INFINITY;
    __syncthreads();
    const uint32_t wofs = st->w * buf_stride;
    uint32_t* lab = lab2 + wofs;
    const float lam = 1.0f / rho;
    const MsgQ mq = msg_q(lam);
    const float kappa = rho * mq.step, nstep = -mq.step, oms = (1.0f - alpha) * mq.scale, lam_s = lam * oms;
    constexpr float HUGE_COST = 1e30f;
    const uint32_t stride = gridDim.x * NPB;
    uint32_t vb = blockIdx.x;
    if (XCD && (gridDim.x & 7u) == 0u) vb = (blockIdx.x & 7u) * (gridDim.x >> 3) + (blockIdx.x >> 3);
    uint32_t i = node_begin + vb * NPB + grp;
    const uint32_t last = node_end - 1;
    const uint32_t n_iter = (node_end - node_begin + stride - 1) / stride;
    const uint32_t t0 = 4u * gl;
    const uint32_t ident_word = 0x03020100u * (uint32_t)G + 0x01010101u * (uint32_t)gl;
    struct Raw { uint4 lw; uint32_t in[3], map[3], nl[3], old[3]; };
    const uint32_t t0b = 4u * t0, glb = 4u * (uint32_t)gl;
    auto issue = [&](const NodeDesc& d, Raw& r) {
        const uint32_t K = d.kk & 0xFFu, recb = 4u * d.rec;
        r.lw = ld_off<uint4>(rec, recb + t0b);
        uint32_t mposb = recb + 4u * ((K + 3u) & ~3u) + glb;
#pragma unroll
        for (int e = 0; e < 3; ++e) {
            r.in[e] = ld_off<uint32_t>(mo, (d.in_off[e] & ~3u) + t0);
            r.map[e] = ld_off<uint32_t>(rec, mposb);
            if (!(d.out_off[e] & 1u)) mposb += (((d.kk >> (8 + 8 * e)) & 0xFFu) + 3u) & ~3u;
            r.nl[e] = ld_off<uint32_t>(lab, 4u * d.nbr[e]);
            if (DAMP) r.old[e] = ld_off<uint32_t>(mo, (d.out_off[e] & ~3u) + t0); else r.old[e] = d.out_off[e];
        }
    };
    NodeDesc cur = ld_off<NodeDesc>(desc, (uint32_t)sizeof(NodeDesc) * min(i, last));
    Raw rw; issue(cur, rw);
    NodeDesc nxt = ld_off<NodeDesc>(desc, (uint32_t)sizeof(NodeDesc) * min(i + stride, last));
    uint32_t acc_e = 0u, acc_c = 0u;
#pragma unroll 2
    for (uint32_t it = 0; it < n_iter; ++it, i += stride) {
        const bool node_ok = i < node_end;
        Raw rn; issue(nxt, rn);
        const NodeDesc nn = ld_off<NodeDesc>(desc, (uint32_t)sizeof(NodeDesc) * min(i + 2u * stride, last));
        const uint32_t K = node_ok ? (cur.kk & 0xFFu) : 0u;
        bool ok[4];
#pragma unroll
        for (int r = 0; r < 4; ++r) ok[r] = t0 + r < K;
        uint32_t kj3[3], o_out[3]; bool ident[3], low[3];
#pragma unroll
        for (int d = 0; d < 3; ++d) {
            kj3[d] = node_ok ? ((cur.kk >> (8 + 8 * d)) & 0xFFu) : 0u;
            ident[d] = (cur.out_off[d] & 1u) != 0u; low[d] = (cur.in_off[d] & 1u) != 0u && kj3[d] != 0u;
            o_out[d] = cur.out_off[d] & ~3u;
        }
        const uint32_t lw[4] = {rw.lw.x, rw.lw.y, rw.lw.z, rw.lw.w};
        const uint32_t* r_in = rw.in; const uint32_t* r_map = rw.map; const uint32_t* nl = rw.nl; const uint32_t* r_old = rw.old;
        float cf[3][4], b[4];
#pragma unroll
        for (int r = 0; r < 4; ++r) {
#pragma unroll
            for (int d = 0; d < 3; ++d) cf[d][r] = (float)((r_in[d] >> (8 * r)) & 0xFFu);
            const float D = ok[r] ? cost_value(lw[r] >> 16) : HUGE_COST;
            b[r] = __builtin_fmaf(kappa, (cf[0][r] + cf[1][r]) + cf[2][r], D);
        }
        float cv[3][4];
#pragma unroll
        for (int d = 0; d < 3; ++d)
#pragma unroll
            for (int r = 0; r < 4; ++r) cv[d][r] = __builtin_fmaf(nstep, cf[d][r], b[r]) * oms;
        float gm = fminf(fminf(b[0], b[1]), fminf(b[2], b[3]));
        float cm0 = fminf(fminf(cv[0][0], cv[0][1]), fminf(cv[0][2], cv[0][3])), cm1 = fminf(fminf(cv[1][0], cv[1][1]), fminf(cv[1][2], cv[1][3])),
              cm2 = fminf(fminf(cv[2][0], cv[2][1]), fminf(cv[2][2], cv[2][3]));
        group_min_fused4<G>(gm, cm0, cm1, cm2);
        const float cmin3[3] = {cm0, cm1, cm2};
        uint32_t bt = (b[3] == gm) ? t0 + 3u : 0xFFFFFFFFu;
        bt = (b[2] == gm) ? t0 + 2u : bt; bt = (b[1] == gm) ? t0 + 1u : bt; bt = (b[0] == gm) ? t0 : bt;
        bt = group_min_fused<G>(bt);
#pragma unroll
        for (int d = 0; d < 3; ++d) {
#pragma unroll
            for (int r = 0; r < 4; ++r) tile[r * G + gl] = cv[d][r] - cmin3[d];
            const uint32_t mw = ident[d] ? ident_word : r_map[d];
            uint32_t w = 0u;
#pragma unroll
            for (int r = 0; r < 4; ++r) {
                const uint32_t mp = (mw >> (8 * r)) & 0xFFu;
                const uint32_t slot = (G < 64) ? mp : ((mp == 0xFFu) ? (uint32_t)(4 * G) : mp);
                w = msg_pack_s<DAMP>(min_raw(tile[slot], lam_s), alpha, (float)((r_old[d] >> (8 * r)) & 0xFFu), (uint32_t)r, w);
            }
            if (t0 < kj3[d]) st_off<uint32_t>(mn, o_out[d] + t0, w);
        }
        const bool owner = node_ok && ((K > 0u) ? ((bt >> 2) == (uint32_t)gl) : (gl == 0));
        if (owner) {
            const uint32_t r = bt & 3u;
            const uint32_t wsel = (r == 0u) ? lw[0] : (r == 1u) ? lw[1] : (r == 2u) ? lw[2] : lw[3];
            const uint32_t my_lab = (K > 0u) ? (wsel & 0xFFFFu) + 1u : 0u;
            const uint32_t my_code = (K > 0u) ? (wsel >> 16) : 65535u;
            const uint32_t idb = 4u * cur.id;
            st_off<uint32_t>(lab, idb, my_lab);
            acc_e += my_code;
            acc_c += (low[0] && nl[0] != my_lab) + (low[1] && nl[1] != my_lab) + (low[2] && nl[2] != my_lab);
        }
        cur = nxt; rw = rn; nxt = nn;
    }
    unsigned long long e = acc_e, c = acc_c;
    for (int o = 32; o > 0; o >>= 1) { e += __shfl_xor(e, o, 64); c += __shfl_xor(c, o, 64); }
    if ((threadIdx.x & 63) == 0) { s_e[threadIdx.x >> 6] = e; s_e[4 + (threadIdx.x >> 6)] = c; }
    __syncthreads();
    if (threadIdx.x == 0) {
        e = s_e[0] + s_e[1] + s_e[2] + s_e[3]; c = s_e[4] + s_e[5] + s_e[6] + s_e[7];
        partial[2 * blockIdx.x] = e + 65535ull * c; partial[2 * blockIdx.x + 1] = c;
    }
}


template <bool DAMP, bool XCD>
__global__ void __launch_bounds__(256) mrf_sweep8_kernel(const NodeDesc* __restrict__ desc, const uint32_t* __restrict__ rec, msg_t* msg,
                                                         const mvs_mrf_progress* __restrict__ st, uint32_t* lab2, uint32_t buf_stride,
                                                         uint32_t node_begin, uint32_t node_end, float rho, float alpha,
                                                         unsigned long long* __restrict__ partial) {
    const msg_t* mo = msg; msg_t* mn = msg;
    constexpr int G = 8, L = 8, NPB = 256 / G;
    constexpr int TS = 72;
    __shared__ float s_c[NPB * TS];
    __shared__ unsigned long long s_e[8];
    const int grp = threadIdx.x / G, gl = threadIdx.x % G;
    float* __restrict__ tile = s_c + grp * TS;
    if (st->stopped) return;
    if (gl == 0) tile[L * G] = INFINITY;
    __syncthreads();
    const uint32_t wofs = st->w * buf_stride;
    uint32_t* lab = lab2 + wofs;
    const float lam = 1.0f / rho;
    const MsgQ mq = msg_q(lam);
    const float kappa = rho * mq.step, nstep = -mq.step, oms = (1.0f - alpha) * mq.scale, lam_s = lam * oms;
    constexpr float HUGE_COST = 1e30f;
    const uint32_t stride = gridDim.x * NPB;
    uint32_t vb = blockIdx.x;
    if (XCD && (gridDim.x & 7u) == 0u) vb = (blockIdx.x & 7u) * (gridDim.x >> 3) + (blockIdx.x >> 3);
    uint32_t i = node_begin + vb * NPB + grp;
    const uint32_t last = node_end - 1;
// ... 286 lines not shown
}

__global__ void __launch_bounds__(256) mrf_icm_apply_kernel(const uint32_t* __restrict__ col_ptr, const uint16_t* __restrict__ view_id, const float* __restrict__ cost,
                                                            const uint32_t* __restrict__ adj_ptr, const uint32_t* __restrict__ adj,
                                                            const float* __restrict__ gain, const uint32_t* __restrict__ cand,
                                                            uint32_t* sel, uint32_t* lab, float* selcost,
                                                            uint32_t node_begin, uint32_t node_end, uint32_t* __restrict__ moved ,
                                                            uint32_t* __restrict__ alist ,
                                                            const uint32_t* __restrict__ orig ) {
    const uint32_t i = node_begin + blockIdx.x * blockDim.x + threadIdx.x;
    bool mv = false;
    if (i < node_end) {
        const float gi = gain[i];
        if (gi > 0.0f) {
            bool win = true;
            for (uint32_t e = adj_ptr[i]; e < adj_ptr[i + 1] && win; ++e) {
                const uint32_t j = adj[e];
                if (lab[j] == 0u) continue;
                const float gj = gain[j];
                if (gj > gi || (gj == gi && (orig ? orig[j] < orig[i] : j < i))) win = false;
            }
            if (win) mv = true;
        }
    }
    if (mv) {
        const uint32_t p0 = col_ptr[i], t = cand[i];
        sel[i] = t; lab[i] = (uint32_t)view_id[p0 + t] + 1u; selcost[i] = cost[p0 + t];
        if (alist) {
            const uint32_t e0 = adj_ptr[i], e1 = adj_ptr[i + 1];
            uint32_t w = atomicAdd(&moved[1], 1u + (e1 - e0));
            alist[w++] = i;
            for (uint32_t e = e0; e < e1; ++e) alist[w++] = adj[e];
        }
    }
    const unsigned long long b = __ballot(mv);
    if ((threadIdx.x & 63) == 0 && b) atomicAdd(moved, (uint32_t)__popcll(b));
}

__global__ void mrf_argmin_unary_kernel(const uint32_t* __restrict__ col_ptr, const uint16_t* __restrict__ view_id, const float* __restrict__ cost, uint32_t F,
                                        uint32_t* __restrict__ sel, uint32_t* __restrict__ lab, float* __restrict__ selcost) {
    const uint32_t i = blockIdx.x * blockDim.x + threadIdx.x;
    if (i >= F) return;
    const uint32_t p0 = col_ptr[i], K = col_ptr[i + 1] - p0;
    uint32_t bt = 0;
    for (uint32_t t = 1; t < K; ++t) if (cost[p0 + t] < cost[p0 + bt]) bt = t;
    sel[i] = bt;
    lab[i] = K ? (uint32_t)view_id[p0 + bt] + 1u : 0u;
    selcost[i] = K ? cost[p0 + bt] : 1.0f;
}

__global__ void mrf_labels_kernel(const uint32_t* __restrict__ lab, uint32_t node_begin, uint32_t node_end, uint32_t n_views,
                                  uint32_t* __restrict__ labels, uint32_t* __restrict__ bad_unseen ,
                                  const uint32_t* __restrict__ orig ,
                                  const uint32_t* __restrict__ foreign ) {
    const uint32_t i = node_begin + blockIdx.x * blockDim.x + threadIdx.x;
    if (i >= node_end) return;
    if (foreign && i == node_begin && *foreign) atomicAdd(&bad_unseen[0], *foreign);
    const uint32_t label = lab[i];
    if (label > n_views) atomicAdd(&bad_unseen[0], 1u);
    if (label == 0u) atomicAdd(&bad_unseen[1], 1u);
    labels[orig ? orig[i] : i - node_begin] = label;
}


__global__ void __launch_bounds__(1024) mrf_step_kernel(mvs_mrf_progress* __restrict__ st, unsigned long long* __restrict__ hist,
                                const unsigned long long* __restrict__ energy, const unsigned long long* __restrict__ partial, uint32_t n_partial,
                                unsigned long long* __restrict__ energy_out, mvs_mrf_progress* __restrict__ ring, uint32_t* __restrict__ ring_seq, uint32_t ring_slots,
                                uint32_t* __restrict__ ctl, int max_sweeps, int min_sweeps, int window, float min_improvement,
                                const unsigned long long* const* __restrict__ peer_tab = nullptr, uint32_t n_peer = 0, uint32_t peer_off = 0) {
    __shared__ unsigned long long su[16], sc[16];
    unsigned long long e_sum = 0, c_sum = 0;
    if (partial) {
        const ulonglong2* pp = reinterpret_cast<const ulonglong2*>(partial);
#pragma unroll 8
        for (uint32_t b = threadIdx.x; b < n_partial; b += 1024u) { const ulonglong2 v = pp[b]; e_sum += v.x; c_sum += v.y; }
        for (int o = 32; o > 0; o >>= 1) { e_sum += __shfl_xor(e_sum, o, 64); c_sum += __shfl_xor(c_sum, o, 64); }
        if ((threadIdx.x & 63) == 0) { su[threadIdx.x >> 6] = e_sum; sc[threadIdx.x >> 6] = c_sum; }
        __syncthreads();
    }
    if (threadIdx.x != 0 || blockIdx.x != 0) return;
    if (partial) {
        e_sum = 0; c_sum = 0;
        for (int k = 0; k < 16; ++k) { e_sum += su[k]; c_sum += sc[k]; }
        energy_out[0] = e_sum; energy_out[1] = c_sum;
    } else if (peer_tab) {
        e_sum = 0; c_sum = 0;
        for (uint32_t q = 0; q < n_peer; ++q) { e_sum += peer_tab[q][peer_off]; c_sum += peer_tab[q][peer_off + 1u]; }
        energy_out[0] = e_sum; energy_out[1] = c_sum;
    }
    mvs_mrf_progress p = *st;
    if (p.stopped) { p.improved = 0u; }
    else {
        const uint32_t sw = p.sweep + 1u;
        const unsigned long long e0 = (partial || peer_tab) ? e_sum : energy[0];
        const bool imp = e0 < p.best;
        if (imp) { p.best = e0; p.best_w = p.w; p.w ^= 1u; }
        p.sweep = sw; p.improved = imp ? 1u : 0u; p.energy = e0;
        hist[sw] = p.best;
        bool stop = false;
        if ((int)sw >= min_sweeps && (int)sw > window) {
            const unsigned long long prev = hist[sw - (uint32_t)window];
            stop = (double)(prev - p.best) < (double)min_improvement * (double)prev;
        }
        if ((int)sw >= max_sweeps) stop = true;
        if (stop) { p.stopped = 1u; p.stop_sweep = sw; }
    }
    *st = p;
    const uint32_t n = ctl[0] + 1u; ctl[0] = n;
    if (ring) {
        const uint32_t slot = n % ring_slots;
        ring[slot] = p;
        __threadfence_system();
        __hip_atomic_store(ring_seq + slot, ctl[1] + n, __ATOMIC_RELEASE, __HIP_MEMORY_SCOPE_SYSTEM);
    }
}
__global__ void report_u32_kernel(const uint32_t* __restrict__ src, uint32_t* __restrict__ dst, uint32_t* __restrict__ dst_seq, uint32_t seq) {
    *dst = *src;
    __threadfence_system();
    __hip_atomic_store(dst_seq, seq, __ATOMIC_RELEASE, __HIP_MEMORY_SCOPE_SYSTEM);
}
__global__ void report_words_kernel(const uint32_t* __restrict__ src, uint32_t n, uint32_t* __restrict__ dst, uint32_t* __restrict__ dst_seq, uint32_t seq) {
    if (threadIdx.x < n) dst[threadIdx.x] = src[threadIdx.x];
    __threadfence_system();
    __syncthreads();
    if (threadIdx.x == 0) __hip_atomic_store(dst_seq, seq, __ATOMIC_RELEASE, __HIP_MEMORY_SCOPE_SYSTEM);
}
__global__ void mrf_flip_kernel(mvs_mrf_progress* __restrict__ st) { st->best_w = st->w; st->w ^= 1u; }

}

constexpr uint32_t EPART_BLOCKS = 2048;
constexpr uint32_t RUN_PAD_MASK = 7;

void mrf_setup(mvs_ctx* ctx, const mvs_mrf_params* params) {
    hipStream_t s = ctx->stream;
    const uint32_t F = ctx->csr_faces;
    ctx->m_params = *params;
    if (!(params->rho > 0.0f && params->rho <= 1.0f) || !(params->damping >= 0.0f && params->damping < 1.0f))
        throw StatusError(MVS_ERR_INVALID, "mrf params: need 0 < rho <= 1, 0 <= damping < 1");
    if (params->window < 1 || params->min_sweeps < 0 || !(params->min_improvement >= 0.0f) || params->icm_iters < 0)
        throw StatusError(MVS_ERR_INVALID, "mrf params: need window >= 1, min_sweeps >= 0, min_improvement >= 0, icm_iters >= 0");
    uint32_t E = ctx->r_adj_edges;
    if (!ctx->r_adj_edges_known) {
        MVS_HIP(hipMemcpyAsync(&E, ctx->r_adj_ptr + F, sizeof(uint32_t), hipMemcpyDeviceToHost, s));
        MVS_HIP(hipStreamSynchronize(s));
    }
    ctx->m_size.ensure((size_t)E + 2); ctx->m_edge.ensure((size_t)E + 1); ctx->m_moved.ensure(8 + 2 * 64);
    ctx->m_n_adj = E;
    uint32_t* maxes = ctx->m_moved.p + 4;
    MVS_HIP(hipMemsetAsync(ctx->m_moved.p, 0, 8 * sizeof(uint32_t), s));
    MVS_HIP(hipMemsetAsync(ctx->m_size.p, 0, ((size_t)E + 2) * sizeof(uint32_t), s));
    const unsigned nb = (F + 255) / 256;
    const uint32_t force_generic = (ctx->csr_nnz < 4 || E == 0 || ctx->mrf_force_generic) ? 1u : 0u;
    ctx->m_cls.ensure((size_t)F + 4);
    ctx->m_rev.ensure((size_t)E + 2);
    if (F) { hipLaunchKernelGGL(mrf_size_kernel, dim3(nb), dim3(256), 0, s, ctx->r_ptr, ctx->r_adj_ptr, ctx->r_adj, F, RUN_PAD_MASK, force_generic, ctx->m_size.p, ctx->m_cls.p, maxes, ctx->m_rev.p); MVS_LAUNCH_CHECK(); }
    ctx->m_colour.ensure((size_t)F + 2); ctx->m_perm.ensure((size_t)F + 2); ctx->m_tmp_a.ensure((size_t)MAX_LAYOUT_COLOURS * ((size_t)F + 1) + 72); ctx->m_tmp_b.ensure((size_t)MAX_LAYOUT_COLOURS * ((size_t)F + 1) + 2); ctx->m_tmp_c.ensure((size_t)F + 2);
    ctx->m_colours = 0; ctx->m_sub_begin.assign(N_KEY + 1, 0); ctx->m_n_fast = 0; ctx->m_range_q.clear(); ctx->m_range_nb = ctx->m_range_ne = 0;
    ctx->m_sweep_no = 0;
    if (F) {
        uint32_t* pending = ctx->m_moved.p + 1;
        hipLaunchKernelGGL(mrf_colour_init_kernel, dim3(nb), dim3(256), 0, s, ctx->m_colour.p, ctx->m_tmp_a.p , F); MVS_LAUNCH_CHECK();
        if (ctx->m_colour_in) MVS_HIP(hipMemcpyAsync(ctx->m_colour.p, ctx->m_colour_in, (size_t)F * sizeof(uint32_t), hipMemcpyDeviceToDevice, s));
        for (int round = 0; !ctx->m_colour_in; ++round) {
            if (round >= 4096) throw StatusError(MVS_ERR_HIP, "graph colouring did not terminate");
            MVS_HIP(hipMemsetAsync(pending, 0, sizeof(uint32_t), s));
            for (int k = 0; k < (round == 0 ? 16 : 4); ++k) { hipLaunchKernelGGL(mrf_colour_round_kernel, dim3(nb), dim3(256), 0, s, ctx->r_adj_ptr, ctx->r_adj, ctx->t_perm, F, ctx->m_colour.p, pending); MVS_LAUNCH_CHECK(); }
            uint32_t hp[2] = {0, 0};
            read_words(ctx, pending, hp, 2);
            if (hp[1]) throw StatusError(MVS_ERR_UNSUPPORTED, "adjacency graph needs more than 64 colours (a node with >= 64 mutually constrained neighbours)");
            if (!hp[0]) break;
        }
        MVS_HIP(hipMemsetAsync(ctx->m_moved.p, 0, 4 * sizeof(uint32_t), s));
        hipLaunchKernelGGL(mrf_sortkey_kernel, dim3(nb), dim3(256), 0, s, ctx->m_colour.p, ctx->m_cls.p, ctx->m_bnd, F, ctx->m_tmp_c.p); MVS_LAUNCH_CHECK();
        size_t tmp_bytes = 0;
        MVS_HIP(rocprim::radix_sort_pairs(nullptr, tmp_bytes, ctx->m_tmp_c.p, ctx->m_tmp_b.p, ctx->m_tmp_a.p, ctx->m_perm.p, F, 0, 10, s));
        ctx->sort_tmp.ensure(tmp_bytes + 16);
        MVS_HIP(rocprim::radix_sort_pairs(ctx->sort_tmp.p, tmp_bytes, ctx->m_tmp_c.p, ctx->m_tmp_b.p, ctx->m_tmp_a.p, ctx->m_perm.p, F, 0, 10, s));
        ctx->m_sub.ensure(3 * (size_t)N_KEY + 8);
        hipLaunchKernelGGL(mrf_sub_begin_kernel, dim3((N_KEY + 256) / 256), dim3(256), 0, s, ctx->m_tmp_b.p, F, ctx->m_sub.p); MVS_LAUNCH_CHECK();
        read_block(ctx, ctx->m_sub.p, ctx->m_sub_begin.data(), (N_KEY + 1) * sizeof(uint32_t));
        const std::vector<uint32_t>& sb = ctx->m_sub_begin;
        uint32_t C = 0;
        for (uint32_t c = 0; c < 64; ++c) if (sb[2 * (4 * c + 4)] > sb[2 * (4 * c)] || sb[2 * (SUB_GENERIC + c + 1)] > sb[2 * (SUB_GENERIC + c)]) C = c + 1;
        ctx->m_colours = C;
        ctx->m_n_fast = sb[2 * SUB_GENERIC];
    }
    DBuf<uint32_t>& in_off = ctx->m_sel2;
    in_off.ensure(std::max<size_t>((size_t)E + 2, (size_t)F + 2));
    MVS_HIP(hipMemsetAsync(in_off.p, 0, ((size_t)E + 2) * sizeof(uint32_t), s));
    uint32_t h[3] = {0, 0, 0};
    if (F) {
        if ((uint64_t)E * 4ull + 4ull * (uint64_t)ctx->csr_nnz >= 0xFFFFFFF0ull) {
            const uint64_t total = sum_u32(ctx, ctx->m_size.p, (size_t)E + 1);
            if ((uint64_t)MSG_BASE + total >= 0xFFFFFFF0ull) throw StatusError(MVS_ERR_UNSUPPORTED, "message array exceeds 2^32 elements (shard the graph: DESIGN.md multi-GPU)");
        }
        const uint32_t n_col = (ctx->m_colours >= 2 && ctx->m_colours <= (uint32_t)MAX_LAYOUT_COLOURS) ? ctx->m_colours : 1u;
        const size_t n_ent = (size_t)n_col * ((size_t)F + 1);
        ctx->m_tmp_a.ensure(n_ent + 72); ctx->m_tmp_b.ensure(n_ent + 2);
        hipLaunchKernelGGL(mrf_nodesize_kernel, dim3((F + 256) / 256), dim3(256), 0, s, ctx->m_perm.p, ctx->m_colour.p, ctx->r_adj_ptr, ctx->r_adj, ctx->m_size.p, ctx->m_rev.p, F, n_col, ctx->m_tmp_a.p); MVS_LAUNCH_CHECK();
        exclusive_scan_u32(ctx, ctx->m_tmp_a.p, ctx->m_tmp_b.p, n_ent, nullptr);
        hipLaunchKernelGGL(mrf_inoff_kernel, dim3(nb), dim3(256), 0, s, ctx->m_perm.p, ctx->m_colour.p, ctx->r_adj_ptr, ctx->r_adj, ctx->m_size.p, ctx->m_rev.p, ctx->m_tmp_b.p, F, n_col, in_off.p); MVS_LAUNCH_CHECK();
        MVS_HIP(hipMemcpyAsync(maxes + 2, ctx->m_tmp_b.p + (n_ent - 1), sizeof(uint32_t), hipMemcpyDeviceToDevice, s));
    } else MVS_HIP(hipMemsetAsync(maxes + 2, 0, sizeof(uint32_t), s));
    { uint32_t hm[3]; read_words(ctx, maxes, hm, 3); h[1] = hm[0]; h[2] = hm[1]; h[0] = hm[2]; }
    ctx->m_total = (uint64_t)MSG_BASE + h[0]; ctx->m_kmax = h[1]; ctx->m_degmax = h[2];
    if (ctx->m_total >= 0xFFFFFFF0ull) throw StatusError(MVS_ERR_UNSUPPORTED, "message array exceeds 2^32 elements");
    if (F) { hipLaunchKernelGGL(mrf_edge_kernel, dim3(nb), dim3(256), 0, s, ctx->r_ptr, ctx->r_adj_ptr, ctx->r_adj, F, in_off.p, ctx->m_size.p, ctx->m_rev.p, ctx->m_edge.p); MVS_LAUNCH_CHECK(); }
    ctx->m_ident.ensure((size_t)E + 1);
    MVS_HIP(hipMemsetAsync(ctx->m_ident.p, 0, (size_t)E + 1, s));
    const uint32_t n_fast = ctx->m_n_fast, n_generic = F - n_fast;
    if (n_fast) {
        const size_t rec_cap = (size_t)REC_BASE + ctx->csr_nnz + 8 * (size_t)F + ctx->m_total / 4 + (size_t)ctx->m_n_adj + 1024;
        ctx->m_rec.ensure(rec_cap);
        MVS_HIP(hipMemsetAsync(ctx->m_rec.p, 0, REC_BASE * sizeof(uint32_t), s));
        hipLaunchKernelGGL(mrf_ident_kernel, dim3((unsigned)(((size_t)F * 16 + 255) / 256)), dim3(256), 0, s, ctx->r_ptr, ctx->r_view, ctx->r_adj_ptr, ctx->r_adj, F, ctx->m_edge.p, ctx->m_cls.p, ctx->m_ident.p); MVS_LAUNCH_CHECK();
        uint32_t* rsz = ctx->m_tmp_a.p; uint32_t* roff = ctx->m_tmp_b.p;
        hipLaunchKernelGGL(mrf_recsize_kernel, dim3((F + 256) / 256), dim3(256), 0, s, ctx->r_ptr, ctx->r_adj_ptr, ctx->m_edge.p, ctx->m_ident.p, ctx->m_cls.p, ctx->m_perm.p, F, rsz, ctx->m_tmp_c.p); MVS_LAUNCH_CHECK();
        exclusive_scan_u32(ctx, rsz, roff, (size_t)F + 1, nullptr);
        hipLaunchKernelGGL(mrf_record_kernel, dim3((unsigned)(((size_t)F * 16 + 255) / 256)), dim3(256), 0, s, ctx->r_ptr, ctx->r_view, ctx->r_cost, ctx->r_adj_ptr, ctx->r_adj,
                           ctx->m_edge.p, ctx->m_ident.p, ctx->m_cls.p, ctx->m_tmp_c.p , roff, F, ctx->m_rec.p); MVS_LAUNCH_CHECK();
        ctx->m_desc.ensure((size_t)F + 1);
        hipLaunchKernelGGL(mrf_desc_kernel, dim3((n_fast + 255) / 256), dim3(256), 0, s, ctx->r_ptr, ctx->r_adj_ptr, ctx->r_adj, ctx->m_edge.p, ctx->m_ident.p, ctx->m_perm.p, ctx->m_colour.p, roff, n_fast, ctx->m_desc.p); MVS_LAUNCH_CHECK();
    }
    if (n_generic) {
        ctx->m_map.ensure(ctx->m_total + 8);
        hipLaunchKernelGGL(mrf_map_kernel, dim3((unsigned)(((size_t)F * 16 + 255) / 256)), dim3(256), 0, s, ctx->r_ptr, ctx->r_view, ctx->r_adj_ptr, ctx->r_adj, F, ctx->m_edge.p, ctx->m_cls.p, ctx->m_map.p); MVS_LAUNCH_CHECK();
        ctx->pq.ensure(ctx->csr_nnz + 1);
    }
    ctx->m_msg_a.ensure(ctx->m_total + 1024);
    MVS_HIP(hipMemsetAsync(ctx->m_msg_a.p, 0, (ctx->m_total + 1024) * sizeof(msg_t), s));
    const size_t F1 = (size_t)F + 1;
    ctx->m_stride = (uint32_t)F1;
    ctx->m_sel.ensure(2 * F1); ctx->m_lab.ensure(2 * F1); ctx->m_cost.ensure(2 * F1);
    ctx->m_sel2.ensure(F1); ctx->m_cand.ensure(F1); ctx->m_gain.ensure(F1);
    MVS_HIP(hipMemsetAsync(ctx->m_sel.p, 0, 2 * F1 * sizeof(uint32_t), s));
    MVS_HIP(hipMemsetAsync(ctx->m_lab.p, 0, 2 * F1 * sizeof(uint32_t), s));
    MVS_HIP(hipMemsetAsync(ctx->m_cost.p, 0, 2 * F1 * sizeof(float), s));
    mvs_mrf_progress init; memset(&init, 0, sizeof(init)); init.best = ~0ull; init.energy = ~0ull; init.w = 0u; init.best_w = 1u;
    if (F && params->max_sweeps <= 0) {
        hipLaunchKernelGGL(mrf_argmin_unary_kernel, dim3(nb), dim3(256), 0, s, ctx->r_ptr, ctx->r_view, ctx->r_cost, F, ctx->m_sel.p, ctx->m_lab.p, ctx->m_cost.p);
        MVS_LAUNCH_CHECK();
        init.w = 1u; init.best_w = 0u;
    }
    ctx->b_sel = ctx->m_sel.p + init.best_w * F1; ctx->b_lab = ctx->m_lab.p + init.best_w * F1; ctx->b_cost = ctx->m_cost.p + init.best_w * F1;
    ctx->best_resolved = true;
    MVS_HIP(hipMemsetAsync(ctx->m_gain.p, 0, F1 * sizeof(float), s));
    const size_t epart = 4 + 2 * (size_t)EPART_BLOCKS * std::max<size_t>(ctx->m_colours, 1);
    ctx->m_energy.ensure(epart);
    MVS_HIP(hipMemsetAsync(ctx->m_energy.p, 0, epart * sizeof(unsigned long long), s));
    ctx->m_state.ensure(1); ctx->m_hist.ensure((size_t)std::max(params->max_sweeps, 0) + 2);
    ensure_report_ring(ctx);
    ctx->seq_base += ctx->steps_issued;
    ctx->h_ring[mvs_ctx::RING] = init;
    MVS_HIP(hipMemcpyAsync(ctx->m_state.p, &ctx->h_ring[mvs_ctx::RING], sizeof(init), hipMemcpyHostToDevice, s));
    ctx->m_ctl.ensure(4);
    uint32_t* stage = ctx->h_seq + (mvs_ctx::RING + mvs_ctx::ICM_RING);
    stage[0] = 0u; stage[1] = ctx->seq_base;
    MVS_HIP(hipMemcpyAsync(ctx->m_ctl.p, stage, 2 * sizeof(uint32_t), hipMemcpyHostToDevice, s));
    MVS_HIP(hipMemsetAsync(ctx->m_hist.p, 0xFF, sizeof(unsigned long long), s));
    ctx->steps_issued = 0; ctx->icm_dirty_valid = false; ctx->exact_valid = false;
}

void resolve_best(mvs_ctx* ctx) {
    if (ctx->best_resolved) return;
    if (!ctx->m_state.p) throw StatusError(MVS_ERR_STATE, "mrf setup first");
    mvs_mrf_progress p;
    static_assert(sizeof(p) % 4 == 0 && sizeof(p) <= 64, "mvs_mrf_progress travels through read_words");
    read_words(ctx, ctx->m_state.p, &p, (uint32_t)(sizeof(p) / 4));
    const size_t o = (size_t)(p.best_w & 1u) * ctx->m_stride;
    ctx->b_sel = ctx->m_sel.p + o; ctx->b_lab = ctx->m_lab.p + o; ctx->b_cost = ctx->m_cost.p + o;
    ctx->best_resolved = true;
}

void mrf_step(mvs_ctx* ctx, const unsigned long long* energy, const unsigned long long* const* peer_tab, uint32_t n_peer, uint32_t peer_off) {
    hipStream_t s = ctx->stream;
    const mvs_mrf_params& P = ctx->m_params;
    if (!ctx->h_ring) throw StatusError(MVS_ERR_STATE, "mrf step before mrf setup");
    const uint32_t n = ++ctx->steps_issued, slot = n % mvs_ctx::RING;
    const unsigned long long* partial = nullptr; uint32_t n_partial = 0;
    if (!energy && !peer_tab) { partial = ctx->m_energy.p + 4; n_partial = ctx->m_energy_from_sweep ? EPART_BLOCKS * std::max<uint32_t>(ctx->m_colours, 1u) : ctx->m_energy_blocks; }
    (void)n; (void)slot;
    hipLaunchKernelGGL(mrf_step_kernel, dim3(1), dim3(1024), 0, s, ctx->m_state.p, ctx->m_hist.p, energy, partial, n_partial, ctx->m_energy.p,
                       ctx->d_ring, ctx->d_seq, (uint32_t)mvs_ctx::RING, ctx->m_ctl.p, P.max_sweeps, P.min_sweeps, P.window, P.min_improvement, peer_tab, n_peer, peer_off);
    MVS_LAUNCH_CHECK();
    ctx->icm_dirty_valid = false; ctx->best_resolved = false; ctx->exact_valid = false;
}
void mrf_poll(mvs_ctx* ctx, uint32_t step, mvs_mrf_progress* out) {
    if (step == 0 || step > ctx->steps_issued || step + mvs_ctx::RING <= ctx->steps_issued)
        throw StatusError(MVS_ERR_INVALID, "mrf poll: step not among the last 16 issued");
    const uint32_t slot = step % mvs_ctx::RING;
    wait_report(ctx, slot, ctx->seq_base + step);
    *out = ctx->h_ring[slot];
}

void ensure_report_ring(mvs_ctx* ctx) {
    if (ctx->h_ring) return;
    constexpr uint32_t NS = mvs_ctx::RING + mvs_ctx::ICM_RING;
    MVS_HIP(hipHostMalloc((void**)&ctx->h_ring, (mvs_ctx::RING + 1) * sizeof(mvs_mrf_progress), hipHostMallocCoherent));
    MVS_HIP(hipHostGetDevicePointer((void**)&ctx->d_ring, ctx->h_ring, 0));
    MVS_HIP(hipHostMalloc((void**)&ctx->h_seq, (NS + 2) * sizeof(uint32_t), hipHostMallocCoherent));
    MVS_HIP(hipHostGetDevicePointer((void**)&ctx->d_seq, ctx->h_seq, 0));
    MVS_HIP(hipHostMalloc((void**)&ctx->h_icm, mvs_ctx::ICM_RING * sizeof(uint32_t), hipHostMallocCoherent));
    MVS_HIP(hipHostGetDevicePointer((void**)&ctx->d_icm, ctx->h_icm, 0));
    for (uint32_t k = 0; k < NS; ++k) ctx->h_seq[k] = 0u;
    ctx->seq_base = 1u; ctx->icm_seq = 0x40000000u;
}
void report_u32(mvs_ctx* ctx, const uint32_t* d_src, uint32_t* d_dst, uint32_t seq_slot, uint32_t seq) {
    hipLaunchKernelGGL(report_u32_kernel, dim3(1), dim3(1), 0, ctx->stream, d_src, d_dst, ctx->d_seq + seq_slot, seq);
    MVS_LAUNCH_CHECK();
}
void read_words(mvs_ctx* ctx, const void* d_src, void* out, uint32_t n_words) {
    if (n_words == 0 || n_words > 64) throw StatusError(MVS_ERR_INVALID, "read_words: 1 .. 64 words");
    if (!ctx->h_rb) {
        MVS_HIP(hipHostMalloc((void**)&ctx->h_rb, (128 + 1024) * sizeof(uint32_t), hipHostMallocCoherent));
        MVS_HIP(hipHostGetDevicePointer((void**)&ctx->d_rb, ctx->h_rb, 0));
        ctx->h_rb[64] = 0u; ctx->rb_seq = 0u;
    }
    const uint32_t seq = ++ctx->rb_seq ? ctx->rb_seq : ++ctx->rb_seq;
    hipLaunchKernelGGL(report_words_kernel, dim3(1), dim3(64), 0, ctx->stream, (const uint32_t*)d_src, n_words, ctx->d_rb, ctx->d_rb + 64, seq);
    MVS_LAUNCH_CHECK();
    const volatile uint32_t* p = ctx->h_rb + 64;
    for (uint64_t spins = 1; *p != seq; ++spins) {
        if ((spins & 0x3FFFu) == 0u) {
            const hipError_t q = hipStreamQuery(ctx->stream);
            if (q == hipSuccess) { if (*p == seq) break; throw HipError("a device read-back did not arrive although the stream is idle"); }
            if (q != hipErrorNotReady) MVS_HIP(q);
        }
        __builtin_ia32_pause();
    }
    std::atomic_thread_fence(std::memory_order_acquire);
    memcpy(out, ctx->h_rb, n_words * sizeof(uint32_t));
}
void read_block(mvs_ctx* ctx, const void* d_src, void* out, size_t bytes) {
    if (bytes <= 64 * sizeof(uint32_t) && bytes % 4 == 0) { read_words(ctx, d_src, out, (uint32_t)(bytes / 4)); return; }
    if (bytes > 1024 * sizeof(uint32_t)) throw StatusError(MVS_ERR_INVALID, "read_block: at most 4 KB");
    if (!ctx->h_rb) { uint32_t dummy; read_words(ctx, d_src, &dummy, 1); }
    MVS_HIP(hipMemcpyAsync(ctx->h_rb + 128, d_src, bytes, hipMemcpyDeviceToHost, ctx->stream));
    MVS_HIP(hipStreamSynchronize(ctx->stream));
    memcpy(out, ctx->h_rb + 128, bytes);
}
void wait_report(mvs_ctx* ctx, uint32_t seq_slot, uint32_t seq) {
    const volatile uint32_t* p = ctx->h_seq + seq_slot;
    for (uint64_t spins = 1; *p != seq; ++spins) {
        if ((spins & 0x3FFFu) == 0u) {
            const hipError_t q = hipStreamQuery(ctx->stream);
            if (q == hipSuccess) { if (*p == seq) break; throw HipError("a device report did not arrive although the stream is idle"); }
            if (q != hipErrorNotReady) MVS_HIP(q);
        }
        __builtin_ia32_pause();
    }
    std::atomic_thread_fence(std::memory_order_acquire);
}
int icm_rounds(mvs_ctx* ctx, int max_rounds, const uint32_t* d_moved, const std::function<void(int)>& round) {
    constexpr int R = (int)mvs_ctx::ICM_RING, LAG = 2;
    ensure_report_ring(ctx);
    int issued = 0, polled = 0, stop = -1;
    const uint32_t seq0 = ctx->icm_seq;
    auto poll = [&]() { const int k = polled++; wait_report(ctx, mvs_ctx::RING + (uint32_t)(k % R), seq0 + (uint32_t)k + 1u); if (stop < 0 && ctx->h_icm[k % R] == 0u) stop = k; };
    ProfChain pc(ctx);
    while (issued < max_rounds && stop < 0) {
        pc.begin();
        round(issued);
        report_u32(ctx, d_moved, ctx->d_icm + issued % R, mvs_ctx::RING + (uint32_t)(issued % R), seq0 + (uint32_t)issued + 1u);
        pc.mark("mrf_icm");
        ++issued;
        if (issued - polled > LAG) poll();
    }
    while (polled < issued) poll();
    ctx->icm_seq = seq0 + (uint32_t)issued;
    return stop >= 0 ? stop : max_rounds;
}

static float sweep_alpha(const mvs_ctx* ctx) {
    return ctx->m_sweep_no % MRF_DAMP_PERIOD == 1u ? ctx->m_params.damping : 0.0f;
}

using FastSweep = void (*)(const NodeDesc*, const uint32_t*, msg_t*, const mvs_mrf_progress*, uint32_t*, uint32_t, uint32_t, uint32_t, float, float, unsigned long long*);
static unsigned launch_fast(mvs_ctx* ctx, const FastSweep (&k)[2][2], unsigned npb, std::atomic<int>& resident_once,
                            uint32_t phase, uint32_t qb, uint32_t qe, unsigned slot, unsigned slot_cap) {
// ... 206 lines not shown
```

mvs-texturing_amd/csrc/mgpu.hip:

```cpp
#include "ctx.h"
#include "../../include/mvs_viewsel_blocks.h"
#include <vector>

namespace mvs {
void mrf_setup(mvs_ctx* ctx, const mvs_mrf_params* params);
void mrf_sweep(mvs_ctx* ctx, uint32_t nb0, uint32_t ne0);
void mrf_energy(mvs_ctx* ctx, bool best, uint32_t nb0, uint32_t ne0, bool reduce = true);
void mrf_keep_best(mvs_ctx* ctx);
void mrf_sweep_phase(mvs_ctx* ctx, uint32_t phase, uint32_t nb0, uint32_t ne0, int part = MRF_PART_ALL);
void mrf_step(mvs_ctx* ctx, const unsigned long long* energy, const unsigned long long* const* peer_tab = nullptr, uint32_t n_peer = 0, uint32_t peer_off = 0);
void mrf_poll(mvs_ctx* ctx, uint32_t step, mvs_mrf_progress* out);
void mrf_icm_gain(mvs_ctx* ctx, uint32_t nb0, uint32_t ne0);
void mrf_icm_apply(mvs_ctx* ctx, uint32_t nb0, uint32_t ne0);
void mrf_labels(mvs_ctx* ctx, uint32_t nb0, uint32_t ne0, uint32_t* d_labels, uint32_t out[2], bool caller_order = false);
void resolve_best(mvs_ctx* ctx);
void set_adjacency(mvs_ctx* ctx, const uint32_t* adj_ptr, const uint32_t* adj, int on_device, bool table_order);
mvs_status api_fail(mvs_status st, const std::string& msg);

namespace {
__global__ void gather_kernel(const uint32_t* __restrict__ src, const mvs_mrf_progress* __restrict__ st, uint32_t buf_stride, const uint32_t* __restrict__ idx, uint64_t n, uint32_t* __restrict__ dst) {
    if (st) src += (size_t)st->w * buf_stride;
    for (uint64_t k = (uint64_t)blockIdx.x * blockDim.x + threadIdx.x; k < n; k += (uint64_t)gridDim.x * blockDim.x) dst[k] = src[idx[k]];
}
__global__ void scatter_kernel(uint32_t* __restrict__ dst, const mvs_mrf_progress* __restrict__ st, uint32_t buf_stride, const uint32_t* __restrict__ idx, uint64_t n, const uint32_t* __restrict__ src) {
    if (st) dst += (size_t)st->w * buf_stride;
    for (uint64_t k = (uint64_t)blockIdx.x * blockDim.x + threadIdx.x; k < n; k += (uint64_t)gridDim.x * blockDim.x) dst[idx[k]] = src[k];
}
__global__ void gather_msg_kernel(const uint8_t* __restrict__ src, const uint32_t* __restrict__ idx, uint64_t n, uint32_t* __restrict__ dst) {
    for (uint64_t k = (uint64_t)blockIdx.x * blockDim.x + threadIdx.x; k < n; k += (uint64_t)gridDim.x * blockDim.x) dst[k] = src[idx[k]];
}
__global__ void scatter_msg_kernel(uint8_t* __restrict__ dst, const uint32_t* __restrict__ idx, uint64_t n, const uint32_t* __restrict__ src) {
    for (uint64_t k = (uint64_t)blockIdx.x * blockDim.x + threadIdx.x; k < n; k += (uint64_t)gridDim.x * blockDim.x) dst[idx[k]] = (uint8_t)src[k];
}
__global__ void gather2_kernel(const uint8_t* __restrict__ a, const uint32_t* __restrict__ b, const mvs_mrf_progress* __restrict__ st, uint32_t buf_stride, const uint32_t* __restrict__ idx, uint64_t n, uint32_t* __restrict__ dst) {
    b += (size_t)st->w * buf_stride;
    for (uint64_t k = (uint64_t)blockIdx.x * blockDim.x + threadIdx.x; k < n; k += (uint64_t)gridDim.x * blockDim.x) {
        const uint32_t i = idx[k];
        dst[k] = (i & 0x80000000u) ? b[i & 0x7FFFFFFFu] : a[i];
    }
}
__global__ void scatter2_kernel(uint8_t* __restrict__ a, uint32_t* __restrict__ b, const mvs_mrf_progress* __restrict__ st, uint32_t buf_stride, const uint32_t* __restrict__ idx, uint64_t n, const uint32_t* __restrict__ src) {
    b += (size_t)st->w * buf_stride;
    for (uint64_t k = (uint64_t)blockIdx.x * blockDim.x + threadIdx.x; k < n; k += (uint64_t)gridDim.x * blockDim.x) {
        const uint32_t i = idx[k];
        if (i & 0x80000000u) b[i & 0x7FFFFFFFu] = src[k]; else a[i] = (uint8_t)src[k];
    }
}
__global__ void counts_kernel(const uint32_t* __restrict__ col_ptr, uint32_t n, uint32_t* __restrict__ counts) {
    const uint32_t i = blockIdx.x * blockDim.x + threadIdx.x;
    if (i < n) counts[i] = col_ptr[i + 1] - col_ptr[i];
}
}

static uint8_t* mrf_msg(mvs_ctx* ctx) { return ctx->m_msg_a.p; }
static uint32_t* mrf_array(mvs_ctx* ctx, int which, const mvs_mrf_progress** st) {
    *st = nullptr;
    switch (which) {
        case MVS_MRF_LAB: *st = ctx->m_state.p; return ctx->m_lab.p;
        case MVS_MRF_GAIN: return (uint32_t*)ctx->m_gain.p;
        case MVS_MRF_BEST_LAB: resolve_best(ctx); return ctx->b_lab;
    }
    throw StatusError(MVS_ERR_INVALID, "bad array selector");
}
}

using namespace mvs;

#define MVS_API_BEGIN try { MVS_HIP(hipSetDevice(ctx->device));
#define MVS_API_END                                                               \
    } catch (const StatusError& e) { return api_fail(e.st, e.what()); }           \
      catch (const HipError& e) { return api_fail(MVS_ERR_HIP, e.what()); }       \
      catch (const std::exception& e) { return api_fail(MVS_ERR_HIP, e.what()); } \
    return MVS_OK;

extern "C" {

mvs_status mvs_ctx_dc_get_max(mvs_ctx* ctx, float* dst) {
    if (!ctx || !dst) return api_fail(MVS_ERR_INVALID, "null argument");
    if (ctx->dc_phase < 1) return api_fail(MVS_ERR_STATE, "dc_phase1 first");
    MVS_API_BEGIN
    MVS_HIP(hipMemcpyAsync(dst, ctx->max_q.p, sizeof(float), hipMemcpyDeviceToDevice, ctx->stream));
    MVS_API_END
}
mvs_status mvs_ctx_dc_set_max(mvs_ctx* ctx, const float* src) {
    if (!ctx || !src) return api_fail(MVS_ERR_INVALID, "null argument");
    if (ctx->dc_phase < 1) return api_fail(MVS_ERR_STATE, "dc_phase1 first");
    MVS_API_BEGIN
    MVS_HIP(hipMemcpyAsync(ctx->max_q.p, src, sizeof(float), hipMemcpyDeviceToDevice, ctx->stream));
    MVS_API_END
}
mvs_status mvs_ctx_dc_get_histogram(mvs_ctx* ctx, uint32_t* dst) {
    if (!ctx || !dst) return api_fail(MVS_ERR_INVALID, "null argument");
    if (ctx->dc_phase < 2) return api_fail(MVS_ERR_STATE, "dc_phase2 first");
    MVS_API_BEGIN
    MVS_HIP(hipMemcpyAsync(dst, ctx->hist.p, MVS_HIST_WORDS * sizeof(uint32_t), hipMemcpyDeviceToDevice, ctx->stream));
    MVS_API_END
}
mvs_status mvs_ctx_dc_set_histogram(mvs_ctx* ctx, const uint32_t* src) {
    if (!ctx || !src) return api_fail(MVS_ERR_INVALID, "null argument");
    if (ctx->dc_phase < 2) return api_fail(MVS_ERR_STATE, "dc_phase2 first");
    MVS_API_BEGIN
    MVS_HIP(hipMemcpyAsync(ctx->hist.p, src, MVS_HIST_WORDS * sizeof(uint32_t), hipMemcpyDeviceToDevice, ctx->stream));
    MVS_API_END
}

mvs_status mvs_ctx_costs_export(mvs_ctx* ctx, uint32_t* counts, uint16_t* view_id, float* cost) {
    if (!ctx || !counts) return api_fail(MVS_ERR_INVALID, "null argument");
    if (!ctx->have_costs) return api_fail(MVS_ERR_STATE, "no data costs on the device");
    MVS_API_BEGIN
    const uint32_t F = ctx->csr_faces;
    if (F) { hipLaunchKernelGGL(counts_kernel, dim3((F + 255) / 256), dim3(256), 0, ctx->stream, ctx->r_ptr, F, counts); MVS_LAUNCH_CHECK(); }
    if (ctx->csr_nnz && view_id) MVS_HIP(hipMemcpyAsync(view_id, ctx->r_view, ctx->csr_nnz * sizeof(uint16_t), hipMemcpyDeviceToDevice, ctx->stream));
    if (ctx->csr_nnz && cost) MVS_HIP(hipMemcpyAsync(cost, ctx->r_cost, ctx->csr_nnz * sizeof(float), hipMemcpyDeviceToDevice, ctx->stream));
    MVS_API_END
}

mvs_status mvs_ctx_mrf_setup(mvs_ctx* ctx, const uint32_t* adj_ptr, const uint32_t* adj, int adj_on_device, const mvs_mrf_params* params) {
    if (!ctx || !adj_ptr || !adj) return api_fail(MVS_ERR_INVALID, "null argument");
    if (!ctx->have_costs) return api_fail(MVS_ERR_STATE, "mrf setup needs data costs");
    MVS_API_BEGIN
    mvs_mrf_params P; if (params) P = *params; else mvs_mrf_default_params(&P);
    set_adjacency(ctx, adj_ptr, adj, adj_on_device, false);
    mrf_setup(ctx, &P);
    MVS_API_END
}

mvs_status mvs_ctx_mrf_sweep(mvs_ctx* ctx, uint32_t nb0, uint32_t ne0) {
    if (!ctx || nb0 > ne0 || ne0 > ctx->csr_faces) return api_fail(MVS_ERR_INVALID, "bad node range");
    MVS_API_BEGIN
    Prof pr(ctx, "mrf_sweep");
    mrf_sweep(ctx, nb0, ne0);
    MVS_API_END
}

mvs_status mvs_ctx_mrf_sweep_phase(mvs_ctx* ctx, uint32_t phase, uint32_t nb0, uint32_t ne0) {
    if (!ctx || nb0 > ne0 || ne0 > ctx->csr_faces || phase >= ctx->m_colours) return api_fail(MVS_ERR_INVALID, "bad phase or node range");
    MVS_API_BEGIN
    Prof pr(ctx, "mrf_sweep");
    mrf_sweep_phase(ctx, phase, nb0, ne0);
    MVS_API_END
}
mvs_status mvs_ctx_mrf_setup_marked(mvs_ctx* ctx, const uint32_t* adj_ptr, const uint32_t* adj, int adj_on_device, const mvs_mrf_params* params, const uint8_t* marks_device) {
    if (!ctx || !adj_ptr || !adj) return api_fail(MVS_ERR_INVALID, "null argument");
    if (!ctx->have_costs) return api_fail(MVS_ERR_STATE, "mrf setup needs data costs");
    MVS_API_BEGIN
    mvs_mrf_params P; if (params) P = *params; else mvs_mrf_default_params(&P);
    set_adjacency(ctx, adj_ptr, adj, adj_on_device, false);
    struct Marks { mvs_ctx* c; ~Marks() { c->m_bnd = nullptr; } } marks{ctx};
    ctx->m_bnd = marks_device;
    mrf_setup(ctx, &P);
    MVS_API_END
}
mvs_status mvs_ctx_mrf_sweep_phase_part(mvs_ctx* ctx, uint32_t phase, uint32_t nb0, uint32_t ne0, int part) {
    if (!ctx || nb0 > ne0 || ne0 > ctx->csr_faces || phase >= ctx->m_colours || part < 0 || part > 2) return api_fail(MVS_ERR_INVALID, "bad phase, node range or part");
    MVS_API_BEGIN
    Prof pr(ctx, part == MRF_PART_BOUNDARY ? "mrf_sweep_boundary" : "mrf_sweep");
    mrf_sweep_phase(ctx, phase, nb0, ne0, part);
    MVS_API_END
}
mvs_status mvs_ctx_mrf_layout(mvs_ctx* ctx, uint32_t* in_off_host, uint64_t n_edges) {
    if (!ctx || (n_edges && !in_off_host)) return api_fail(MVS_ERR_INVALID, "null argument");
    MVS_API_BEGIN
    if (n_edges) MVS_HIP(hipMemcpy2DAsync(in_off_host, sizeof(uint32_t), ctx->m_edge.p, sizeof(MrfEdge), sizeof(uint32_t), n_edges, hipMemcpyDeviceToHost, ctx->stream));
    MVS_HIP(hipStreamSynchronize(ctx->stream));
    MVS_API_END
}

mvs_status mvs_ctx_mrf_gather(mvs_ctx* ctx, int which, const uint32_t* idx, uint64_t n, void* dst) {
    if (!ctx || (n && (!idx || !dst))) return api_fail(MVS_ERR_INVALID, "null argument");
    MVS_API_BEGIN
    if (n && which == MVS_MRF_MSG_LAB) {
        if (ctx->m_total >= 0x80000000ull) throw StatusError(MVS_ERR_UNSUPPORTED, "combined addressing needs < 2^31 message words");
        hipLaunchKernelGGL(gather2_kernel, dim3((unsigned)std::min<uint64_t>((n + 255) / 256, 4096)), dim3(256), 0, ctx->stream, mrf_msg(ctx), ctx->m_lab.p, ctx->m_state.p, ctx->m_stride, idx, n, (uint32_t*)dst);
        MVS_LAUNCH_CHECK();
    } else if (n && which == MVS_MRF_MSG) {
        hipLaunchKernelGGL(gather_msg_kernel, dim3((unsigned)std::min<uint64_t>((n + 255) / 256, 4096)), dim3(256), 0, ctx->stream, mrf_msg(ctx), idx, n, (uint32_t*)dst);
        MVS_LAUNCH_CHECK();
    } else if (n) {
        const mvs_mrf_progress* st; const uint32_t* arr = mrf_array(ctx, which, &st);
        hipLaunchKernelGGL(gather_kernel, dim3((unsigned)std::min<uint64_t>((n + 255) / 256, 4096)), dim3(256), 0, ctx->stream, arr, st, ctx->m_stride, idx, n, (uint32_t*)dst);
        MVS_LAUNCH_CHECK();
    }
    MVS_API_END
}
mvs_status mvs_ctx_mrf_scatter(mvs_ctx* ctx, int which, const uint32_t* idx, uint64_t n, const void* src) {
    if (!ctx || (n && (!idx || !src))) return api_fail(MVS_ERR_INVALID, "null argument");
    MVS_API_BEGIN
    if (n) { ctx->icm_dirty_valid = false; ctx->exact_valid = false; }
    if (n && which == MVS_MRF_MSG_LAB) {
        hipLaunchKernelGGL(scatter2_kernel, dim3((unsigned)std::min<uint64_t>((n + 255) / 256, 4096)), dim3(256), 0, ctx->stream, mrf_msg(ctx), ctx->m_lab.p, ctx->m_state.p, ctx->m_stride, idx, n, (const uint32_t*)src);
        MVS_LAUNCH_CHECK();
    } else if (n && which == MVS_MRF_MSG) {
        hipLaunchKernelGGL(scatter_msg_kernel, dim3((unsigned)std::min<uint64_t>((n + 255) / 256, 4096)), dim3(256), 0, ctx->stream, mrf_msg(ctx), idx, n, (const uint32_t*)src);
        MVS_LAUNCH_CHECK();
    } else if (n) {
        const mvs_mrf_progress* st; uint32_t* arr = mrf_array(ctx, which, &st);
        hipLaunchKernelGGL(scatter_kernel, dim3((unsigned)std::min<uint64_t>((n + 255) / 256, 4096)), dim3(256), 0, ctx->stream, arr, st, ctx->m_stride, idx, n, (const uint32_t*)src);
        MVS_LAUNCH_CHECK();
    }
    MVS_API_END
}

mvs_status mvs_ctx_mrf_energy(mvs_ctx* ctx, int which_sel, uint32_t nb0, uint32_t ne0, uint64_t* dst) {
    if (!ctx || !dst || nb0 > ne0 || ne0 > ctx->csr_faces) return api_fail(MVS_ERR_INVALID, "bad argument");
    if (which_sel != MVS_MRF_LAB && which_sel != MVS_MRF_BEST_LAB) return api_fail(MVS_ERR_INVALID, "energy: LAB or BEST_LAB");
    MVS_API_BEGIN
    mrf_energy(ctx, which_sel == MVS_MRF_BEST_LAB, nb0, ne0);
    MVS_HIP(hipMemcpyAsync(dst, ctx->m_energy.p, 2 * sizeof(uint64_t), hipMemcpyDeviceToDevice, ctx->stream));
    MVS_API_END
}

mvs_status mvs_ctx_mrf_keep_best(mvs_ctx* ctx) {
    if (!ctx) return api_fail(MVS_ERR_INVALID, "ctx is null");
    MVS_API_BEGIN
    mrf_keep_best(ctx);
    MVS_API_END
}

mvs_status mvs_ctx_mrf_step(mvs_ctx* ctx, const uint64_t* energy_device) {
    if (!ctx) return api_fail(MVS_ERR_INVALID, "ctx is null");
    MVS_API_BEGIN
    mrf_step(ctx, (const unsigned long long*)energy_device);
    MVS_API_END
}
mvs_status mvs_ctx_mrf_poll(mvs_ctx* ctx, uint32_t step, mvs_mrf_progress* out) {
    if (!ctx || !out) return api_fail(MVS_ERR_INVALID, "null argument");
    MVS_API_BEGIN
    mrf_poll(ctx, step, out);
    MVS_API_END
}

mvs_status mvs_ctx_mrf_icm_gain(mvs_ctx* ctx, uint32_t nb0, uint32_t ne0) {
    if (!ctx || nb0 > ne0 || ne0 > ctx->csr_faces) return api_fail(MVS_ERR_INVALID, "bad node range");
    MVS_API_BEGIN
    mrf_icm_gain(ctx, nb0, ne0);
    MVS_API_END
}
mvs_status mvs_ctx_mrf_icm_apply(mvs_ctx* ctx, uint32_t nb0, uint32_t ne0, uint32_t* moved) {
    if (!ctx || !moved || nb0 > ne0 || ne0 > ctx->csr_faces) return api_fail(MVS_ERR_INVALID, "bad argument");
    MVS_API_BEGIN
    mrf_icm_apply(ctx, nb0, ne0);
    MVS_HIP(hipMemcpyAsync(moved, ctx->m_moved.p, sizeof(uint32_t), hipMemcpyDeviceToDevice, ctx->stream));
    MVS_API_END
}

mvs_status mvs_ctx_mrf_labels(mvs_ctx* ctx, uint32_t nb0, uint32_t ne0, uint32_t* labels, uint32_t* unseen_out) {
    if (!ctx || !labels || nb0 > ne0 || ne0 > ctx->csr_faces) return api_fail(MVS_ERR_INVALID, "bad argument");
    MVS_API_BEGIN
    uint32_t bu[2];
    mrf_labels(ctx, nb0, ne0, labels, bu);
    if (unseen_out) *unseen_out = bu[1];
    if (bu[0]) throw StatusError(MVS_ERR_LABELING, "Incorrect labeling");
    MVS_API_END
}

}
```

mvs-texturing_amd/viewsel.py:

```python
import ctypes as C
import os

import numpy as np

_HERE = os.path.dirname(os.path.abspath(__file__))
_LIB_PATH = os.environ.get("MVS_VIEWSEL_LIB") or os.path.join(_HERE, "csrc", "libmvs_viewsel.so")
_BLOCKS_PATH = os.path.join(_HERE, "csrc", "libmvs_blocks.so")


class MvsError(RuntimeError):
    def __init__(self, status, message):
        super().__init__("%s (status %d)" % (message, status))
        self.status = status


class CMesh(C.Structure):
    _fields_ = [("n_verts", C.c_uint32), ("n_faces", C.c_uint32), ("verts", C.c_void_p), ("faces", C.c_void_p),
                ("face_normals", C.c_void_p)]


class CView(C.Structure):
    _fields_ = [("pos", C.c_float * 3), ("viewdir", C.c_float * 3), ("K", C.c_float * 9), ("w2c", C.c_float * 16),
                ("width", C.c_int32), ("height", C.c_int32), ("rgb", C.c_void_p)]


class Settings(C.Structure):
    _fields_ = [("data_term", C.c_int32), ("outlier_removal", C.c_int32), ("geometric_visibility_test", C.c_int32)]

    DATA_TERMS = {"area": 0, "gmi": 1}
    OUTLIER = {"none": 0, "gauss_damping": 1, "gauss_clamping": 2}

    def __init__(self, data_term="gmi", outlier_removal="none", geometric_visibility_test=True):
        super().__init__(self.DATA_TERMS[data_term] if isinstance(data_term, str) else int(data_term),
                         self.OUTLIER[outlier_removal] if isinstance(outlier_removal, str) else int(outlier_removal),
                         1 if geometric_visibility_test else 0)


class CCsr(C.Structure):
    _fields_ = [("n_faces", C.c_uint32), ("n_views", C.c_uint32), ("nnz", C.c_uint64), ("col_ptr", C.c_void_p),
                ("view_id", C.c_void_p), ("cost", C.c_void_p)]


class MrfParams(C.Structure):
    _fields_ = [("max_sweeps", C.c_int32), ("min_sweeps", C.c_int32), ("window", C.c_int32),
                ("min_improvement", C.c_float), ("damping", C.c_float), ("rho", C.c_float), ("icm_iters", C.c_int32),
                ("region_rounds", C.c_int32)]


class MrfStats(C.Structure):
    _fields_ = [("energy_fixed", C.c_uint64), ("energy", C.c_double), ("cut_edges", C.c_uint64), ("sweeps", C.c_uint32),
                ("icm_iters", C.c_uint32), ("unseen", C.c_uint32), ("region_rounds", C.c_uint32), ("region_moves", C.c_uint32)]


class MrfProgress(C.Structure):
    _fields_ = [("sweep", C.c_uint32), ("stopped", C.c_uint32), ("improved", C.c_uint32), ("stop_sweep", C.c_uint32),
                ("energy", C.c_uint64), ("best", C.c_uint64), ("w", C.c_uint32), ("best_w", C.c_uint32)]


class Subgraphs(C.Structure):
    _fields_ = [("n_faces", C.c_uint32), ("n_labels", C.c_uint32), ("n_components", C.c_uint32),
                ("label_ptr", C.c_void_p), ("comp_ptr", C.c_void_p), ("comp_faces", C.c_void_p)]


class GslParams(C.Structure):
    _fields_ = [("tolerance", C.c_float), ("max_iterations", C.c_uint32), ("lam", C.c_float), ("reserved", C.c_uint32)]


class GslResult(C.Structure):
    _fields_ = [("n_verts", C.c_uint32), ("n_faces", C.c_uint32), ("x_rows", C.c_uint32), ("reserved", C.c_uint32),
                ("x_ptr", C.c_void_p), ("x_label", C.c_void_p), ("x_adjust", C.c_void_p), ("corner_adjust", C.c_void_p)]


GSL_COUNTS = ("patches", "merged", "x_rows", "a_rows", "gamma_rows", "lhs_nnz_lower", "seam_edges", "samples")
GSL_MS = ("ms_rows", "ms_patches", "ms_system", "ms_solve", "ms_output", "ms_total")


class GslStats(C.Structure):
    _fields_ = [(k, C.c_uint64) for k in GSL_COUNTS] + [("iterations", C.c_uint32 * 3), ("error", C.c_float * 3)] + [(k, C.c_float) for k in GSL_MS]


class GslSystem(C.Structure):
    _fields_ = [("x_rows", C.c_uint32), ("a_rows", C.c_uint32), ("lhs_nnz", C.c_uint64), ("lhs_ptr", C.c_void_p), ("lhs_col", C.c_void_p),
                ("lhs_val", C.c_void_p), ("rhs", C.c_void_p), ("a_col", C.c_void_p), ("b", C.c_void_p), ("x_raw", C.c_void_p)]


class PatchParams(C.Structure):
    _fields_ = [("max_pixels", C.c_uint64), ("reserved", C.c_uint64)]


class PatchSet(C.Structure):
    _fields_ = [("n_patches", C.c_uint32), ("n_listed", C.c_uint32), ("n_pixels", C.c_uint64)] + \
               [(k, C.c_void_p) for k in ("label", "box", "face_ptr", "faces", "texcoords", "pix_ptr", "image", "validity", "blending")]


PATCH_COUNTS = ("patches", "merged", "listed_faces", "degenerate_faces", "pixels", "valid_pixels", "near_pixels")
PATCH_MS = ("ms_tables", "ms_lists", "ms_mark", "ms_resolve", "ms_total")


class PatchStats(C.Structure):
    _fields_ = [(k, C.c_uint64) for k in PATCH_COUNTS] + [(k, C.c_float) for k in PATCH_MS] + [("reserved", C.c_float)]


class LslParams(C.Structure):
    _fields_ = [("tolerance", C.c_float), ("max_iterations", C.c_uint32), ("strip_width", C.c_uint32), ("lds_bytes", C.c_uint32)]


class LslResult(C.Structure):
    _fields_ = [("n_patches", C.c_uint32), ("reserved", C.c_uint32), ("n_pixels", C.c_uint64), ("image", C.c_void_p), ("validity", C.c_void_p),
                ("blending", C.c_void_p)]


LSL_COUNTS = ("seam_edges", "skipped_pairs", "vertex_infos", "edge_projections", "colour_samples", "invalid_samples", "vertex_writes", "line_writes",
              "written_pixels", "outside_frame", "invalid_writes", "strip_pixels", "fixed_pixels", "demoted", "patches_lds", "patches_global",
              "pixels_global", "iterations_total", "hit_max_iterations")
LSL_MS = ("ms_topology", "ms_colours", "ms_writes", "ms_mask", "ms_solve", "ms_total")


class LslStats(C.Structure):
    _fields_ = [(k, C.c_uint64) for k in LSL_COUNTS] + [("iterations_max", C.c_uint32), ("error_max", C.c_float)] + [(k, C.c_float) for k in LSL_MS]


class DcStats(C.Structure):
    _fields_ = [(n, C.c_uint64) for n in ("pairs", "cull_backface", "cull_angle", "cull_outside", "cull_occluded",
                                           "cull_zero_quality", "nnz_pre", "nnz", "rays", "ray_nodes", "ray_tris", "ray_packets", "ray_packets_generic")] + \
               [("max_quality", C.c_float), ("percentile", C.c_float), ("footprints_lane_group", C.c_uint64), ("footprints_rewalked", C.c_uint64), ("ray_leaf_rounds", C.c_uint64)]


def _stats_dict(s):
    return {f[0]: getattr(s, f[0]) for f in s._fields_}


def lib_path():
    return _LIB_PATH


def blocks_lib_path():
    return _BLOCKS_PATH


BLOCK_SYMBOLS = frozenset((
    "mvs_ctx_dc_get_max", "mvs_ctx_dc_set_max", "mvs_ctx_dc_get_histogram", "mvs_ctx_dc_set_histogram", "mvs_ctx_costs_export",
    "mvs_ctx_mrf_setup", "mvs_ctx_mrf_setup_marked", "mvs_ctx_mrf_sweep", "mvs_ctx_mrf_sweep_phase", "mvs_ctx_mrf_sweep_phase_part", "mvs_ctx_mrf_layout", "mvs_ctx_mrf_gather", "mvs_ctx_mrf_scatter",
    "mvs_ctx_mrf_energy", "mvs_ctx_mrf_keep_best", "mvs_ctx_mrf_step", "mvs_ctx_mrf_poll", "mvs_ctx_mrf_icm_gain", "mvs_ctx_mrf_icm_apply",
    "mvs_ctx_mrf_labels"))


_lib = None


def load_library():
    global _lib
    if _lib is not None:
        return _lib
    try:
        import torch
    except ImportError:
        pass
    if not os.path.exists(_LIB_PATH):
        raise MvsError(-1, "HIP library %s is missing: run `python mvs-texturing_amd/build.py` "
                           "(or __graft_entry__.build()); there is no CPU fallback" % _LIB_PATH)
    L = C.CDLL(_LIB_PATH)
    L.mvs_last_error.restype = C.c_char_p
    L.mvs_status_string.restype = C.c_char_p
    L.mvs_last_call_profile.restype = C.c_char_p
    vp, u32, u64, i32 = C.c_void_p, C.c_uint32, C.c_uint64, C.c_int
    sig = {
        "mvs_mrf_default_params": [C.POINTER(MrfParams)], "mvs_default_settings": [C.POINTER(Settings)],
        "mvs_data_costs": [C.POINTER(CMesh), C.POINTER(CView), u32, C.POINTER(Settings), C.POINTER(CCsr), C.POINTER(DcStats)],
        "mvs_csr_free": [C.POINTER(CCsr)], "mvs_subgraphs_free": [C.POINTER(Subgraphs)],
        "mvs_view_selection": [C.POINTER(CCsr), vp, vp, C.POINTER(MrfParams), vp, C.POINTER(MrfStats)],
        "mvs_write_spt": [C.POINTER(CCsr), C.c_char_p], "mvs_read_spt": [C.c_char_p, C.POINTER(CCsr)],
        "mvs_write_labeling_vec": [vp, u32, C.c_char_p],
        "mvs_prepare_mesh": [u32, vp, u32, vp, vp, vp, C.POINTER(u32)],
        "mvs_build_adjacency_graph": [u32, u32, vp, vp, C.POINTER(vp), C.POINTER(u64)],
        "mvs_ctx_build_adjacency": [vp, C.POINTER(vp), C.POINTER(vp), C.POINTER(u64)],
        "mvs_get_subgraphs": [u32, vp, vp, vp, u32, C.POINTER(Subgraphs)],
        "mvs_ctx_get_subgraphs": [vp, u32, vp, vp, i32, vp, i32, u32, C.POINTER(Subgraphs), i32],
        "mvs_ctx_create": [i32, C.POINTER(vp)], "mvs_ctx_destroy": [vp], "mvs_ctx_set_stream": [vp, vp],
        "mvs_ctx_synchronize": [vp], "mvs_set_option": [vp, C.c_char_p, C.c_int64],
        "mvs_ctx_get_profile": [vp, C.c_char_p, C.c_size_t],
        "mvs_scene_set_mesh": [vp, C.POINTER(CMesh), i32], "mvs_scene_set_views": [vp, C.POINTER(CView), u32, i32],
        "mvs_scene_set_face_range": [vp, u32, u32],
        "mvs_ctx_data_costs": [vp, C.POINTER(Settings), C.POINTER(DcStats)],
        "mvs_ctx_dc_phase1": [vp, C.POINTER(Settings)], "mvs_ctx_dc_get_max": [vp, vp], "mvs_ctx_dc_set_max": [vp, vp],
        "mvs_ctx_dc_phase2": [vp], "mvs_ctx_dc_get_histogram": [vp, vp], "mvs_ctx_dc_set_histogram": [vp, vp],
        "mvs_ctx_dc_phase3": [vp, C.POINTER(DcStats)],
        "mvs_ctx_costs_device": [vp, C.POINTER(CCsr)], "mvs_ctx_costs_download": [vp, C.POINTER(CCsr), C.POINTER(vp)],
        "mvs_ctx_costs_upload": [vp, C.POINTER(CCsr), i32], "mvs_ctx_costs_export": [vp, vp, vp, vp],
        "mvs_ctx_view_selection": [vp, vp, vp, i32, C.POINTER(MrfParams), vp, i32, C.POINTER(MrfStats)],
        "mvs_ctx_mrf_setup": [vp, vp, vp, i32, C.POINTER(MrfParams)], "mvs_ctx_mrf_sweep": [vp, u32, u32],
        "mvs_ctx_mrf_setup_marked": [vp, vp, vp, i32, C.POINTER(MrfParams), vp], "mvs_ctx_mrf_sweep_phase_part": [vp, u32, u32, u32, i32],
        "mvs_ctx_mrf_num_phases": [vp, C.POINTER(u32)], "mvs_ctx_mrf_diagnostics": [vp, C.POINTER(u32)], "mvs_ctx_mrf_sweep_phase": [vp, u32, u32, u32], "mvs_ctx_mrf_layout": [vp, vp, u64],
        "mvs_ctx_mrf_gather": [vp, i32, vp, u64, vp], "mvs_ctx_mrf_scatter": [vp, i32, vp, u64, vp],
        "mvs_ctx_mrf_energy": [vp, i32, u32, u32, vp], "mvs_ctx_mrf_keep_best": [vp],
        "mvs_ctx_mrf_step": [vp, vp], "mvs_ctx_mrf_poll": [vp, u32, C.POINTER(MrfProgress)],
        "mvs_ctx_mrf_icm_gain": [vp, u32, u32], "mvs_ctx_mrf_icm_apply": [vp, u32, u32, vp],
        "mvs_ctx_mrf_labels": [vp, u32, u32, vp, C.POINTER(u32)],
        "mvs_ctx_prune_labels": [vp, u32], "mvs_undistort_image": [vp, C.c_int32, C.c_int32, C.c_float, C.c_float, C.c_float, vp],
        "mvs_postprocess_face_infos": [u32, u32, vp, vp, vp, vp, C.POINTER(Settings), C.POINTER(CCsr), C.POINTER(DcStats)],
        "mvs_comm_unique_id": [vp], "mvs_comm_create_rccl": [i32, i32, i32, vp, C.POINTER(vp)], "mvs_comm_create_local": [i32, C.POINTER(vp)], "mvs_comm_create_local_devices": [i32, vp, C.POINTER(vp)],
        "mvs_comm_info": [vp, C.POINTER(i32), C.POINTER(i32), C.POINTER(i32)],
        "mvs_comm_destroy": [vp], "mvs_comm_abort": [vp], "mvs_shard_create": [vp, vp, vp, vp, vp, C.POINTER(vp)], "mvs_shard_destroy": [vp],
        "mvs_shard_data_costs": [vp, C.POINTER(Settings), C.POINTER(DcStats), C.POINTER(u64)],
        "mvs_shard_view_selection": [vp, C.POINTER(MrfParams), vp, C.POINTER(MrfStats)],
        "mvs_shard_plan_info": [vp, C.POINTER(u64), C.POINTER(u64), C.POINTER(C.c_double)],
        "mvs_shard_transport_info": [vp, C.POINTER(i32), C.POINTER(u64), C.POINTER(i32), C.POINTER(u32)],
        "mvs_shard_own_faces": [vp, vp, C.POINTER(u32)],
        "mvs_ctx_partition_faces": [vp, i32, vp, vp], "mvs_partition_faces": [C.POINTER(CMesh), i32, vp, vp],
        "mvs_ctx_table_order": [vp, vp, C.POINTER(i32)],
        "mvs_gsl_default_params": [C.POINTER(GslParams)], "mvs_gsl_result_free": [C.POINTER(GslResult)], "mvs_gsl_system_free": [C.POINTER(GslSystem)],
        "mvs_ctx_global_seam_leveling": [vp, vp, vp, i32, vp, i32, C.POINTER(GslParams), C.POINTER(GslResult), i32, C.POINTER(GslStats)],
        "mvs_ctx_gsl_system": [vp, C.POINTER(GslSystem)],
        "mvs_patch_default_params": [C.POINTER(PatchParams)], "mvs_patch_set_free": [C.POINTER(PatchSet)],
        "mvs_ctx_texture_patches": [vp, vp, vp, i32, vp, i32, vp, i32, C.POINTER(PatchParams), C.POINTER(PatchSet), i32, C.POINTER(PatchStats)],
        "mvs_lsl_default_params": [C.POINTER(LslParams)], "mvs_lsl_result_free": [C.POINTER(LslResult)],
        "mvs_ctx_local_seam_leveling": [vp, vp, vp, i32, vp, i32, C.POINTER(PatchSet), i32, C.POINTER(LslParams), C.POINTER(LslResult), i32, C.POINTER(LslStats)],
        "mvs_data_costs_stream": [C.POINTER(CMesh), C.POINTER(CView), u32, C.POINTER(Settings), vp, vp, C.POINTER(CCsr), C.POINTER(DcStats)],
        "mvs_view_selection_cached": [u64, u32, u32, u64, vp, vp, C.POINTER(MrfParams), vp, C.POINTER(MrfStats)],
    }
    blocks = None
    if os.path.exists(_BLOCKS_PATH):
        try:
            blocks = C.CDLL(_BLOCKS_PATH, mode=C.RTLD_GLOBAL)
        except OSError:
            blocks = None
    L._blocks_declared = []
    for name, argtypes in sig.items():
        if name in BLOCK_SYMBOLS:
            if blocks is None:
                continue
            fn = getattr(blocks, name)
            setattr(L, name, fn)
            L._blocks_declared.append(name)
        else:
            fn = getattr(L, name)
        fn.argtypes = argtypes
        if name not in ("mvs_mrf_default_params", "mvs_default_settings", "mvs_csr_free", "mvs_subgraphs_free", "mvs_gsl_default_params",
                        "mvs_gsl_result_free", "mvs_gsl_system_free", "mvs_patch_default_params", "mvs_patch_set_free", "mvs_lsl_default_params", "mvs_lsl_result_free", "mvs_ctx_destroy", "mvs_comm_destroy", "mvs_comm_abort", "mvs_shard_destroy"):
            fn.restype = C.c_int
    L._declared = sorted([k for k in sig.keys() if k not in BLOCK_SYMBOLS] + ["mvs_last_error", "mvs_status_string"])
    L._blocks = blocks
    _lib = L
    return L


def _check(L, st):
    if st != 0:
        raise MvsError(st, L.mvs_last_error().decode() or L.mvs_status_string(st).decode())


def _is_torch(a):
    return type(a).__module__.startswith("torch")


class DevArray:
    is_cuda = True

    def __init__(self, ptr, n):
        self.ptr, self.shape = int(ptr or 0), (int(n),)

    def data_ptr(self):
        return self.ptr

    def is_contiguous(self):
        return True


def _ptr(a):
    if a is None:
        return None, 0
    if _is_torch(a) or isinstance(a, DevArray):
        assert a.is_contiguous()
        return C.c_void_p(a.data_ptr()), 1 if a.is_cuda else 0
    assert a.flags["C_CONTIGUOUS"]
    return a.ctypes.data_as(C.c_void_p), 0


def default_mrf_params(**kw):
    p = MrfParams()
    load_library().mvs_mrf_default_params(C.byref(p))
    for k, v in kw.items():
        setattr(p, k, v)
    return p


class DataCosts:

    def __init__(self, n_faces, n_views, col_ptr, view_id, cost, quality=None):
        self.n_faces, self.n_views = int(n_faces), int(n_views)
        self.col_ptr, self.view_id, self.cost, self.quality = col_ptr, view_id, cost, quality

    cols = property(lambda self: self.n_faces)
    rows = property(lambda self: self.n_views)

    @property
    def nnz(self):
        return int(self.col_ptr[-1])

    def col(self, i):
        a, b = int(self.col_ptr[i]), int(self.col_ptr[i + 1])
        return list(zip(self.view_id[a:b].tolist(), self.cost[a:b].tolist()))

    def _struct(self):
        s = CCsr(self.n_faces, self.n_views, self.nnz, 0, 0, 0)
        s.col_ptr, dev0 = _ptr(self.col_ptr)
        s.view_id, dev1 = _ptr(self.view_id)
        s.cost, dev2 = _ptr(self.cost)
        assert dev0 == dev1 == dev2
        return s, dev0

    def save_to_file(self, path):
        L = load_library()
        s, dev = self._struct()
        assert not dev, "download first"
        _check(L, L.mvs_write_spt(C.byref(s), path.encode()))


class Context:

    def __init__(self, device=0):
        self.L = load_library()
        h = C.c_void_p()
        _check(self.L, self.L.mvs_ctx_create(device, C.byref(h)))
        self.h = h
        self.device = int(device)
        self._keep = {}

    def close(self):
        if getattr(self, "h", None):
            self.L.mvs_ctx_destroy(self.h)
            self.h = None

    __del__ = close

    def set_stream(self, stream_handle):
        _check(self.L, self.L.mvs_ctx_set_stream(self.h, C.c_void_p(stream_handle)))

    def synchronize(self):
        _check(self.L, self.L.mvs_ctx_synchronize(self.h))

    def set_option(self, name, value):
        _check(self.L, self.L.mvs_set_option(self.h, name.encode(), int(value)))

    def get_profile(self):
        import json
        buf = C.create_string_buffer(1 << 16)
        _check(self.L, self.L.mvs_ctx_get_profile(self.h, buf, len(buf)))
        return json.loads(buf.value.decode())

    def set_mesh(self, verts, faces, normals):
        pv, d0 = _ptr(verts); pf, d1 = _ptr(faces); pn, d2 = _ptr(normals)
        assert d0 == d1 == d2
        m = CMesh(int(verts.shape[0]), int(faces.shape[0]), pv, pf, pn)
        self._keep["mesh"] = (verts, faces, normals)
        self.n_faces = int(faces.shape[0])
        _check(self.L, self.L.mvs_scene_set_mesh(self.h, C.byref(m), d0))

    def set_views(self, cams, images):
        V = len(images)
        arr = (CView * V)()
        dev = None
        for j in range(V):
            v = arr[j]
            v.pos[:] = np.asarray(cams["pos"][j], dtype=np.float32).tolist()
            v.viewdir[:] = np.asarray(cams["viewdir"][j], dtype=np.float32).tolist()
            v.K[:] = np.asarray(cams["K"][j], dtype=np.float32).ravel().tolist()
            v.w2c[:] = np.asarray(cams["w2c"][j], dtype=np.float32).ravel().tolist()
            v.width, v.height = int(cams["width"][j]), int(cams["height"][j])
            p, d = _ptr(images[j])
            v.rgb = p
            assert dev is None or dev == d
            dev = d
        self._keep["views"] = images
        self.n_views = V
        _check(self.L, self.L.mvs_scene_set_views(self.h, arr, V, dev or 0))

    def set_face_range(self, begin, end):
        _check(self.L, self.L.mvs_scene_set_face_range(self.h, begin, end))

    def partition_faces(self, world=1):
        import torch
        F = self.n_faces
        perm = torch.zeros(max(F, 1), dtype=torch.int32, device="cuda:%d" % self.device)
        torch.cuda.synchronize(self.device)
        part = np.zeros(world + 1, dtype=np.uint32)
        _check(self.L, self.L.mvs_ctx_partition_faces(self.h, int(world), C.c_void_p(perm.data_ptr()), part.ctypes.data_as(C.c_void_p)))
        return perm.cpu().numpy().view(np.uint32)[:F].copy(), part

    def table_order(self):
        import torch
        F = self.n_faces
        out = torch.zeros(max(F, 1), dtype=torch.int32, device="cuda:%d" % self.device)
        torch.cuda.synchronize(self.device)
        flag = C.c_int(0)
        _check(self.L, self.L.mvs_ctx_table_order(self.h, C.c_void_p(out.data_ptr()), C.byref(flag)))
        return out.cpu().numpy().view(np.uint32)[:F].copy() if flag.value else None

    def build_adjacency(self):
        pp, pa, n = C.c_void_p(), C.c_void_p(), C.c_uint64(0)
        _check(self.L, self.L.mvs_ctx_build_adjacency(self.h, C.byref(pp), C.byref(pa), C.byref(n)))
        return DevArray(pp.value, self.n_faces + 1), DevArray(pa.value, n.value)

    def data_costs(self, settings=None):
        st = settings or Settings()
        ds = DcStats()
        _check(self.L, self.L.mvs_ctx_data_costs(self.h, C.byref(st), C.byref(ds)))
        return _stats_dict(ds)

    def costs_download(self):
        out = CCsr(); q = C.c_void_p()
        _check(self.L, self.L.mvs_ctx_costs_download(self.h, C.byref(out), C.byref(q)))
        F, nnz = out.n_faces, out.nnz
        def grab(ptr, ctype, n):
            return np.ctypeslib.as_array(C.cast(ptr, C.POINTER(ctype)), (max(n, 1),))[:n].copy()
        res = DataCosts(F, out.n_views, grab(out.col_ptr, C.c_uint32, F + 1), grab(out.view_id, C.c_uint16, nnz),
                        grab(out.cost, C.c_float, nnz), grab(q.value, C.c_float, nnz))
        self.L.mvs_csr_free(C.byref(out))
        C.CDLL(None).free(q)
        return res

    def prune_labels(self, max_labels):
        _check(self.L, self.L.mvs_ctx_prune_labels(self.h, int(max_labels)))

    def costs_upload(self, dc):
        s, dev = dc._struct()
        self._keep["costs"] = dc
        _check(self.L, self.L.mvs_ctx_costs_upload(self.h, C.byref(s), dev))

    def view_selection(self, adj_ptr, adj, params=None, labels_out=None):
        p = params or default_mrf_params()
        pa, d0 = _ptr(adj_ptr); pb, d1 = _ptr(adj)
        assert d0 == d1
        F = int(adj_ptr.shape[0]) - 1
        if labels_out is None:
            labels_out = np.zeros(F, dtype=np.uint32)
        pl, dl = _ptr(labels_out)
        ms = MrfStats()
        self._keep["adj"] = (adj_ptr, adj)
        _check(self.L, self.L.mvs_ctx_view_selection(self.h, pa, pb, d0, C.byref(p), pl, dl, C.byref(ms)))
        return labels_out, _stats_dict(ms)


    def mrf_diagnostics(self):
        out = (C.c_uint32 * 4)()
        _check(self.L, self.L.mvs_ctx_mrf_diagnostics(self.h, out))
        return dict(zip(("graph_launches", "graph_updates", "graph_instantiations", "generic_nodes"), [int(x) for x in out]))

    def get_subgraphs(self, adj_ptr, adj, labels, n_labels, on_device=False):
        pa, d0 = _ptr(adj_ptr); pb, d1 = _ptr(adj); pl, dl = _ptr(labels)
        assert d0 == d1
        F = int(adj_ptr.shape[0]) - 1
        sg = Subgraphs()
        self._keep["sg"] = (adj_ptr, adj, labels)
        _check(self.L, self.L.mvs_ctx_get_subgraphs(self.h, F, pa, pb, d0, pl, dl, int(n_labels), C.byref(sg), 1 if on_device else 0))
        if on_device:
            return DevArray(sg.label_ptr, n_labels + 1), DevArray(sg.comp_ptr, sg.n_components + 1), DevArray(sg.comp_faces, F)
        return _subgraphs_to_numpy(self.L, sg)

    def global_seam_leveling(self, adj_ptr, adj, labels, params=None, on_device=False):
        pa, d0 = _ptr(adj_ptr); pb, d1 = _ptr(adj); pl, dl = _ptr(labels)
        assert d0 == d1
        p = params or default_gsl_params()
        res, st = GslResult(), GslStats()
        self._keep["gsl"] = (adj_ptr, adj, labels)
        _check(self.L, self.L.mvs_ctx_global_seam_leveling(self.h, pa, pb, d0, pl, dl, C.byref(p), C.byref(res), 1 if on_device else 0, C.byref(st)))
        stats = {k: int(getattr(st, k)) for k in GSL_COUNTS}
        stats.update({k: float(getattr(st, k)) for k in GSL_MS})
        stats["iterations"] = [int(x) for x in st.iterations]
        stats["error"] = np.array(list(st.error), np.float32)
        NV, F, XR = int(res.n_verts), int(res.n_faces), int(res.x_rows)
        if on_device:
            return dict(x_ptr=DevArray(res.x_ptr, NV + 1), x_label=DevArray(res.x_label, XR), x_adjust=DevArray(res.x_adjust, 3 * XR),
                        corner_adjust=DevArray(res.corner_adjust, 9 * F)), stats
        out = dict(x_ptr=_grab(res.x_ptr, NV + 1, C.c_uint32), x_label=_grab(res.x_label, XR, C.c_uint32),
                   x_adjust=_grab(res.x_adjust, 3 * XR, C.c_float).reshape(XR, 3), corner_adjust=_grab(res.corner_adjust, 9 * F, C.c_float).reshape(F, 3, 3))
        self.L.mvs_gsl_result_free(C.byref(res))
        return out, stats

    def texture_patches(self, adj_ptr, adj, labels, corner_adjust=None, params=None, on_device=False):
        pa, d0 = _ptr(adj_ptr); pb, d1 = _ptr(adj); pl, dl = _ptr(labels)
        assert d0 == d1
        if corner_adjust is not None and not (_is_torch(corner_adjust) or isinstance(corner_adjust, DevArray)):
            corner_adjust = np.ascontiguousarray(corner_adjust, np.float32)
        pc, dc = _ptr(corner_adjust)
        p = params or default_patch_params()
        res, st = PatchSet(), PatchStats()
        self._keep["patches"] = (adj_ptr, adj, labels, corner_adjust)
        rc = self.L.mvs_ctx_texture_patches(self.h, pa, pb, d0, pl, dl, pc, dc, C.byref(p), C.byref(res), 1 if on_device else 0, C.byref(st))
        stats = {k: int(getattr(st, k)) for k in PATCH_COUNTS}
        stats.update({k: float(getattr(st, k)) for k in PATCH_MS})
        if rc != 0:
            try:
                _check(self.L, rc)
            except MvsError as e:
                e.stats = stats
                raise
        P, NL, NP = int(res.n_patches), int(res.n_listed), int(res.n_pixels)
        shapes = dict(label=(P, np.uint32), box=(4 * P, np.int32), face_ptr=(P + 1, np.uint32), faces=(NL, np.uint32), texcoords=(6 * NL, np.float32),
                      pix_ptr=(P + 1, np.uint64), image=(3 * NP, np.float32), validity=(NP, np.uint8), blending=(NP, np.uint8))
        if on_device:
            return {k: DevArray(getattr(res, k), n) for k, (n, _) in shapes.items()}, stats
        out = {}
        for k, (n, dt) in shapes.items():
            out[k] = np.frombuffer(C.string_at(getattr(res, k), n * np.dtype(dt).itemsize), dt).copy() if n else np.zeros(0, dt)
        self.L.mvs_patch_set_free(C.byref(res))
        out["box"] = out["box"].reshape(P, 4); out["texcoords"] = out["texcoords"].reshape(NL, 3, 2); out["image"] = out["image"].reshape(NP, 3)
        return out, stats

    def local_seam_leveling(self, adj_ptr, adj, labels, patches, params=None, on_device=False):
        pa, d0 = _ptr(adj_ptr); pb, d1 = _ptr(adj); pl, dl = _ptr(labels)
        assert d0 == d1
        dts = dict(label=np.uint32, box=np.int32, face_ptr=np.uint32, faces=np.uint32, texcoords=np.float32, pix_ptr=np.uint64, image=np.float32,
                   validity=np.uint8, blending=np.uint8)
        dev = [_is_torch(patches[k]) or isinstance(patches[k], DevArray) for k in dts]
        assert all(dev) or not any(dev), "the patch set must be all host or all device arrays"
        held = {k: patches[k] if dev[0] else np.ascontiguousarray(patches[k], dts[k]).reshape(-1) for k in dts}
        ps = PatchSet()
        if dev[0]:
            P = int(held["label"].shape[0]); ps.n_listed = int(held["faces"].shape[0]); ps.n_pixels = int(held["validity"].shape[0])
        else:
            P = held["label"].size; ps.n_listed = held["faces"].size; ps.n_pixels = held["validity"].size
        ps.n_patches = P
        for k in dts:
            setattr(ps, k, _ptr(held[k])[0] if (dev[0] or held[k].size) else None)
        p = params or default_lsl_params()
        res, st = LslResult(), LslStats()
        self._keep["lsl"] = (adj_ptr, adj, labels, held)
        rc = self.L.mvs_ctx_local_seam_leveling(self.h, pa, pb, d0, pl, dl, C.byref(ps), 1 if dev[0] else 0, C.byref(p), C.byref(res),
                                                1 if on_device else 0, C.byref(st))
        stats = {k: int(getattr(st, k)) for k in LSL_COUNTS + ("iterations_max",)}
        stats["error_max"] = float(st.error_max)
        stats.update({k: float(getattr(st, k)) for k in LSL_MS})
        if rc != 0:
            try:
                _check(self.L, rc)
            except MvsError as e:
                e.stats = stats
                raise
        NP = int(res.n_pixels)
        shapes = dict(image=(3 * NP, np.float32), validity=(NP, np.uint8), blending=(NP, np.uint8))
        if on_device:
            return {k: DevArray(getattr(res, k), n) for k, (n, _) in shapes.items()}, stats
        out = {}
        for k, (n, dt) in shapes.items():
            out[k] = np.frombuffer(C.string_at(getattr(res, k), n * np.dtype(dt).itemsize), dt).copy() if n else np.zeros(0, dt)
        self.L.mvs_lsl_result_free(C.byref(res))
        out["image"] = out["image"].reshape(NP, 3)
        return out, stats

    def gsl_system(self):
        s = GslSystem()
        _check(self.L, self.L.mvs_ctx_gsl_system(self.h, C.byref(s)))
        XR, AR, NZ = int(s.x_rows), int(s.a_rows), int(s.lhs_nnz)
        out = dict(lhs_ptr=_grab(s.lhs_ptr, XR + 1, C.c_uint32), lhs_col=_grab(s.lhs_col, NZ, C.c_uint32), lhs_val=_grab(s.lhs_val, NZ, C.c_float),
                   rhs=_grab(s.rhs, 3 * XR, C.c_float).reshape(XR, 3), a_col=_grab(s.a_col, 2 * AR, C.c_uint32).reshape(AR, 2),
                   b=_grab(s.b, 3 * AR, C.c_float).reshape(AR, 3), x_raw=_grab(s.x_raw, 3 * XR, C.c_float).reshape(XR, 3))
        self.L.mvs_gsl_system_free(C.byref(s))
        return out


def _grab(ptr, n, ctype):
    if n == 0:
        return np.zeros(0, np.uint32 if ctype is C.c_uint32 else np.float32)
    return np.ctypeslib.as_array(C.cast(ptr, C.POINTER(ctype)), (n,)).copy()


def default_gsl_params(**kw):
    p = GslParams()
    load_library().mvs_gsl_default_params(C.byref(p))
    for k, v in kw.items():
        setattr(p, k, v)
    return p


def default_patch_params(**kw):
    p = PatchParams()
    load_library().mvs_patch_default_params(C.byref(p))
    for k, v in kw.items():
        setattr(p, k, v)
    return p


def default_lsl_params(**kw):
    p = LslParams()
    load_library().mvs_lsl_default_params(C.byref(p))
    for k, v in kw.items():
        setattr(p, k, v)
    return p


def patch_view(arrays, i):
    w, h = int(arrays["box"][i, 2]), int(arrays["box"][i, 3])
    a, b = int(arrays["pix_ptr"][i]), int(arrays["pix_ptr"][i + 1])
    return arrays["image"][a:b].reshape(h, w, 3), arrays["validity"][a:b].reshape(h, w), arrays["blending"][a:b].reshape(h, w)

# ... 141 lines not shown
```

Baseline: 76.47 million faces/s.

## Use per-face view bitmaps to build MRF identity flags, records and label maps

Adds a per-face bitmap of candidate views, built in one kernel, and uses it during MRF setup. Neighbour identity tests become XORs of bitmap words, and neighbour label mappings come from rank/select, replacing the list-merging ident, record, desc and map kernels. The record and descriptor kernels are fused into one. This targets setup cost inside view-selection; it adds a bitmap buffer, a fallback option to force the list path, and a debug export API.

```diff
diff --git a/include/mvs_viewsel_blocks.h b/include/mvs_viewsel_blocks.h
--- a/include/mvs_viewsel_blocks.h
+++ b/include/mvs_viewsel_blocks.h
@@ -20,6 +20,7 @@
                                     const mvs_mrf_params* params, const uint8_t* marks_device);
 mvs_status mvs_ctx_mrf_sweep_phase_part(mvs_ctx* ctx, uint32_t phase, uint32_t node_begin, uint32_t node_end, int part);
 mvs_status mvs_ctx_mrf_sweep(mvs_ctx* ctx, uint32_t node_begin, uint32_t node_end);
+mvs_status mvs_ctx_mrf_setup_tables(mvs_ctx* ctx, int which, void* out_host, uint64_t cap_bytes, uint64_t* n_bytes);
 mvs_status mvs_ctx_mrf_layout(mvs_ctx* ctx, uint32_t* in_off_host, uint64_t n_edges);
 mvs_status mvs_ctx_mrf_gather(mvs_ctx* ctx, int which, const uint32_t* idx_device, uint64_t n, void* dst_device);
 mvs_status mvs_ctx_mrf_scatter(mvs_ctx* ctx, int which, const uint32_t* idx_device, uint64_t n, const void* src_device);
diff --git a/mvs-texturing_amd/csrc/api.hip b/mvs-texturing_amd/csrc/api.hip
--- a/mvs-texturing_amd/csrc/api.hip
+++ b/mvs-texturing_amd/csrc/api.hip
@@ -366,6 +366,7 @@
     else if (n == "mrf_xcd") ctx->mrf_xcd = (int)value;
     else if (n == "mrf_lag") ctx->mrf_lag = (int)value;
     else if (n == "mrf_force_generic") ctx->mrf_force_generic = value != 0;
+    else if (n == "mrf_force_lists") ctx->mrf_force_lists = value != 0;
     else if (n == "mrf_graph") ctx->mrf_graph = value != 0;
     else if (n == "mrf_blocks_per_cu") ctx->mrf_blocks_per_cu = std::max(0, (int)value);
     else if (n == "bvh_upper_min_faces") { ctx->kd_disabled = false; ctx->bvh_upper_min_faces = (uint32_t)std::max<int64_t>(0, std::min<int64_t>(value, 0xFFFFFFFFll)); ctx->order_pinned = false; }
diff --git a/mvs-texturing_amd/csrc/ctx.h b/mvs-texturing_amd/csrc/ctx.h
--- a/mvs-texturing_amd/csrc/ctx.h
+++ b/mvs-texturing_amd/csrc/ctx.h
@@ -224,6 +224,8 @@
     const uint32_t* m_colour_in = nullptr;
     const uint8_t* m_bnd = nullptr;
     int mrf_force_generic = 0;
+    mvs::DBuf<unsigned long long> m_bits; bool m_bitmaps = false;
+    int mrf_force_lists = 0;
     uint32_t m_range_nb = 0, m_range_ne = 0; std::vector<uint32_t> m_range_q;
     uint32_t m_sweep_no = 0;
     mvs_mrf_params m_params{};
@@ -271,6 +273,7 @@
 void report_u32(mvs_ctx* ctx, const uint32_t* d_src, uint32_t* d_dst, uint32_t seq_slot, uint32_t seq);
 void wait_report(mvs_ctx* ctx, uint32_t seq_slot, uint32_t seq);
 int icm_rounds(mvs_ctx* ctx, int max_rounds, const uint32_t* d_moved, const std::function<void(int)>& round);
+constexpr uint32_t MRF_REC_BASE = 256;
 constexpr uint32_t MRF_DAMP_PERIOD = 4;
 void read_words(mvs_ctx* ctx, const void* d_src, void* out, uint32_t n_words);
 void read_block(mvs_ctx* ctx, const void* d_src, void* out, size_t bytes);
diff --git a/mvs-texturing_amd/csrc/dmath.h b/mvs-texturing_amd/csrc/dmath.h
--- a/mvs-texturing_amd/csrc/dmath.h
+++ b/mvs-texturing_amd/csrc/dmath.h
@@ -426,6 +426,35 @@
     return (uint32_t)floorf(((clamped - 0.0f) / (maxv - 0.0f)) * (float)(num_bins - 1));
 }
 
+constexpr uint32_t BITMAP_NONE = 0xFFFFFFFFu;
+MVS_HD uint32_t bitmap_words(uint32_t n_views) { return (n_views + 63u) >> 6; }
+MVS_HD uint64_t bitmap_below(uint32_t p) { return (1ull << p) - 1ull; }
+MVS_HD uint32_t bitmap_popc(uint64_t x) { return (uint32_t)__builtin_popcountll(x); }
+MVS_HD uint32_t bitmap_rank_word(uint64_t word, uint32_t before, uint32_t v) {
+    const uint32_t p = v & 63u;
+    return ((word >> p) & 1ull) ? before + bitmap_popc(word & bitmap_below(p)) : BITMAP_NONE;
+}
+MVS_HD uint32_t bitmap_rank(const uint64_t* bits, uint32_t W, uint32_t v) {
+    const uint32_t w = v >> 6;
+    if (w >= W) return BITMAP_NONE;
+    uint32_t before = 0;
+    for (uint32_t k = 0; k < w; ++k) before += bitmap_popc(bits[k]);
+    return bitmap_rank_word(bits[w], before, v);
+}
+MVS_HD bool bitmap_equal(const uint64_t* a, const uint64_t* b, uint32_t W) {
+    uint64_t d = 0;
+    for (uint32_t k = 0; k < W; ++k) d |= a[k] ^ b[k];
+    return d == 0;
+}
+MVS_HD uint32_t bitmap_select(uint64_t x, uint32_t n) {
+    uint32_t pos = 0;
+    for (uint32_t sh = 32; sh > 0; sh >>= 1) {
+        const uint32_t c = bitmap_popc(x & bitmap_below(sh));
+        if (n >= c) { n -= c; x >>= sh; pos += sh; }
+    }
+    return pos;
+}
+
 inline float host_cos_limit() {
     const double limit = 75.0f * (3.14159265358979323846264338327950288 / 180.0);
     auto f = [](uint32_t u) { float x; memcpy(&x, &u, 4); return x; };
diff --git a/mvs-texturing_amd/csrc/dmath_host.cpp b/mvs-texturing_amd/csrc/dmath_host.cpp
--- a/mvs-texturing_amd/csrc/dmath_host.cpp
+++ b/mvs-texturing_amd/csrc/dmath_host.cpp
@@ -98,6 +98,24 @@
 
 uint32_t dmh_hist_bin(float value, float maxv) { return hist_bin(value, maxv, 10000u); }
 
+uint32_t dmh_bitmap_words(uint32_t n_views) { return bitmap_words(n_views); }
+void dmh_bitmap_of_list(const uint16_t* list, uint32_t n, uint32_t n_views, uint64_t* bits) {
+    const uint32_t W = bitmap_words(n_views);
+    for (uint32_t w = 0; w < W; ++w) bits[w] = 0;
+    for (uint32_t t = 0; t < n; ++t) if (list[t] < n_views) bits[list[t] >> 6] |= 1ull << (list[t] & 63u);
+}
+void dmh_bitmap_rank(const uint64_t* bits, uint32_t W, const uint32_t* query, uint32_t nq, uint32_t* out) {
+    for (uint32_t q = 0; q < nq; ++q) out[q] = bitmap_rank(bits, W, query[q]);
+}
+int dmh_bitmap_equal(const uint64_t* a, const uint64_t* b, uint32_t W) { return bitmap_equal(a, b, W) ? 1 : 0; }
+void dmh_bitmap_select(const uint64_t* bits, uint32_t W, uint32_t n, uint32_t* out) {
+    for (uint32_t t = 0; t < n; ++t) {
+        uint32_t w = 0, before = 0;
+        while (w + 1 < W && before + bitmap_popc(bits[w]) <= t) { before += bitmap_popc(bits[w]); ++w; }
+        out[t] = 64u * w + bitmap_select(bits[w], t - before);
+    }
+}
+
 void dmh_foot_cert_trials(uint64_t seed, uint32_t trials, uint32_t max_n, int shift, uint64_t* out) {
     uint64_t n_cert = 0, n_mis = 0, n_bad = 0;
 #pragma omp parallel for schedule(dynamic, 64) reduction(+ : n_cert, n_mis, n_bad)
diff --git a/mvs-texturing_amd/csrc/k_mrf.hip b/mvs-texturing_amd/csrc/k_mrf.hip
--- a/mvs-texturing_amd/csrc/k_mrf.hip
+++ b/mvs-texturing_amd/csrc/k_mrf.hip
@@ -281,17 +281,68 @@
     }
 }
 
+constexpr uint32_t BITMAP_MAX_WORDS = 16;
+template <class T> __device__ __forceinline__ T ld_unaligned(const void* p) { T v; __builtin_memcpy(&v, p, sizeof(T)); return v; }
+__device__ __forceinline__ void ld_views4(const uint16_t* __restrict__ view_id, uint64_t at, uint32_t n, uint64_t nnz, uint32_t (&v)[4]) {
+    if (at + 4u <= nnz) { const uint2 w = ld_unaligned<uint2>(view_id + at); v[0] = w.x & 0xFFFFu; v[1] = w.x >> 16; v[2] = w.y & 0xFFFFu; v[3] = w.y >> 16; }
+    else {
+#pragma unroll
+        for (uint32_t r = 0; r < 4; ++r) v[r] = (r < n) ? (uint32_t)view_id[at + r] : 0u;
+    }
+}
+__global__ void __launch_bounds__(256) mrf_bitmap_kernel(const uint32_t* __restrict__ col_ptr, const uint16_t* __restrict__ view_id, uint64_t nnz, uint32_t F, uint32_t V, uint32_t W,
+                                                         unsigned long long* __restrict__ bits, uint32_t* __restrict__ flag) {
+    __shared__ uint32_t s_b[16][2 * BITMAP_MAX_WORDS];
+    const uint32_t i = (blockIdx.x * blockDim.x + threadIdx.x) >> 4;
+    const uint32_t gl = threadIdx.x & 15;
+    if (i >= F) return;
+    uint32_t* tile = s_b[threadIdx.x >> 4];
+    tile[2 * gl] = 0u; tile[2 * gl + 1] = 0u;
+    __builtin_amdgcn_fence(__ATOMIC_ACQ_REL, "wavefront");
+    const uint32_t p0 = col_ptr[i], K = col_ptr[i + 1] - p0;
+    bool bad = false;
+    uint32_t carry = 0u;
+    for (uint32_t t0 = 0; t0 < K; t0 += 64) {
+        const uint32_t t = t0 + 4u * gl, n = t < K ? min(K - t, 4u) : 0u;
+        uint32_t v[4] = {0u, 0u, 0u, 0u};
+        if (n) ld_views4(view_id, (uint64_t)p0 + t, n, nnz, v);
+        uint32_t before = (uint32_t)__shfl_up((int)v[3], 1, 16);
+        if (gl == 0u) before = carry;
+#pragma unroll
+        for (uint32_t r = 0; r < 4; ++r) {
+            if (r < n) {
+                bad = bad || v[r] >= V || ((t + r) != 0u && before >= v[r]);
+                if (v[r] < V) atomicOr(&tile[v[r] >> 5], 1u << (v[r] & 31u));
+            }
+            before = v[r];
+        }
+        carry = (uint32_t)__shfl((int)v[3], 15, 16);
+    }
+    __builtin_amdgcn_fence(__ATOMIC_ACQ_REL, "wavefront");
+    if (gl < W) bits[(size_t)i * W + gl] = (unsigned long long)tile[2 * gl] | ((unsigned long long)tile[2 * gl + 1] << 32);
+    if (bad) *flag = 1u;
+}
+
 __global__ void mrf_edge_kernel(const uint32_t* __restrict__ col_ptr, const uint32_t* __restrict__ adj_ptr, const uint32_t* __restrict__ adj,
-                                uint32_t F, const uint32_t* __restrict__ in_off, const uint32_t* __restrict__ size, const uint32_t* __restrict__ rev, MrfEdge* __restrict__ edge) {
+                                uint32_t F, const uint32_t* __restrict__ in_off, const uint32_t* __restrict__ size, const uint32_t* __restrict__ rev, MrfEdge* __restrict__ edge,
+                                const uint8_t* __restrict__ cls, const unsigned long long* __restrict__ bits, uint32_t W, uint8_t* __restrict__ ident) {
     const uint32_t i = blockIdx.x * blockDim.x + threadIdx.x;
     if (i >= F) return;
     const uint32_t e0 = adj_ptr[i], e1 = adj_ptr[i + 1];
+    const bool fast = bits && cls[i] != CLS_GENERIC;
     for (uint32_t eb = e0; eb < e1; eb += 4) {
         uint32_t j[4], r[4], io[4], sz[4], oo[4], kj[4];
+        unsigned long long diff[4] = {0ull, 0ull, 0ull, 0ull};
 #pragma unroll
         for (int t = 0; t < 4; ++t) { const bool on = eb + t < e1; j[t] = on ? adj[eb + t] : i; r[t] = on ? rev[eb + t] : 0xFFFFFFFFu; io[t] = on ? in_off[eb + t] : 0u; sz[t] = on ? size[eb + t] : 0u; }
 #pragma unroll
         for (int t = 0; t < 4; ++t) { oo[t] = (r[t] != 0xFFFFFFFFu) ? in_off[r[t]] : 0u; kj[t] = col_ptr[j[t] + 1] - col_ptr[j[t]]; }
+        if (fast)
+            for (uint32_t w = 0; w < W; ++w) {
+                const unsigned long long own = bits[(size_t)i * W + w];
+#pragma unroll
+                for (int t = 0; t < 4; ++t) diff[t] |= own ^ bits[(size_t)j[t] * W + w];
+            }
 #pragma unroll
         for (int t = 0; t < 4; ++t) {
             if (eb + t >= e1) continue;
@@ -301,6 +352,7 @@
             m.out_off = has ? MSG_BASE + oo[t] : 0u;
             m.kj = (sz[t] > 0 && has) ? kj[t] : 0u;
             edge[eb + t] = m;
+            if (bits) ident[eb + t] = (uint8_t)((fast && m.kj != 0u && diff[t] == 0ull) ? 1u : 0u);
         }
     }
 }
@@ -331,7 +383,7 @@
     }
 }
 
-constexpr uint32_t REC_BASE = 256;
+constexpr uint32_t REC_BASE = MRF_REC_BASE;
 constexpr float COST_SCALE = 65535.0f;
 __device__ __forceinline__ uint32_t cost_code(float c) { return (uint32_t)(c * COST_SCALE + 0.5f); }
 __device__ __forceinline__ float cost_value(uint32_t code) { return (float)code * (1.0f / 65535.0f); }
@@ -481,6 +533,150 @@
         nd.in_off[d] = m.in_off | flag_low; nd.out_off[d] = m.out_off | flag_ident; nd.kk |= m.kj << (8 + 8 * d); nd.nbr[d] = nb;
     }
     desc[q] = nd;
+}
+
+__device__ __forceinline__ void bitmap_to_tile(unsigned long long word, uint32_t gl, unsigned long long* __restrict__ t_bits, uint32_t* __restrict__ t_pre) {
+    const uint32_t c = bitmap_popc(word);
+    uint32_t incl = c;
+#pragma unroll
+    for (int o = 1; o < 16; o <<= 1) { const uint32_t up = (uint32_t)__shfl_up((int)incl, o, 16); incl += (gl >= (uint32_t)o) ? up : 0u; }
+    t_bits[gl] = word; t_pre[gl] = incl - c;
+}
+__global__ void __launch_bounds__(256) mrf_record_bits_kernel(const uint32_t* __restrict__ col_ptr, const uint16_t* __restrict__ view_id, const float* __restrict__ cost,
+                                                              const uint32_t* __restrict__ adj_ptr, const uint32_t* __restrict__ adj, const MrfEdge* __restrict__ edge,
+                                                              const uint8_t* __restrict__ ident, const uint8_t* __restrict__ cls, const uint32_t* __restrict__ qpos, const uint32_t* __restrict__ roff,
+                                                              const uint32_t* __restrict__ colour, const unsigned long long* __restrict__ bits, uint32_t W, uint64_t nnz, uint32_t F, uint32_t n_fast,
+                                                              uint32_t* __restrict__ rec, NodeDesc* __restrict__ desc) {
+    __shared__ unsigned long long s_bits[16][4][BITMAP_MAX_WORDS];
+    __shared__ uint32_t s_pre[16][4][BITMAP_MAX_WORDS];
+    const uint32_t i = (blockIdx.x * blockDim.x + threadIdx.x) >> 4;
+    const uint32_t gl = threadIdx.x & 15;
+    if (i >= F) return;
+    const uint32_t ci = cls[i];
+    if (ci == CLS_GENERIC) return;
+    const uint32_t p0 = col_ptr[i], K = col_ptr[i + 1] - p0;
+    const uint32_t q = qpos[i], ro = roff[q], col_i = colour[i];
+    const uint32_t e0 = adj_ptr[i], deg = min(adj_ptr[i + 1] - e0, 3u);
+    MrfEdge m[3]; uint32_t idn[3], nb[3], col_n[3], kj3[3];
+#pragma unroll
+    for (uint32_t d = 0; d < 3; ++d) {
+        const bool on = d < deg;
+        m[d].in_off = on ? edge[e0 + d].in_off : 0u; m[d].out_off = on ? edge[e0 + d].out_off : 0u; m[d].kj = on ? edge[e0 + d].kj : 0u;
+        idn[d] = on ? (uint32_t)ident[e0 + d] : 0u; nb[d] = on ? adj[e0 + d] : i;
+    }
+#pragma unroll
+    for (uint32_t d = 0; d < 3; ++d) {
+        col_n[d] = colour[nb[d]];
+        if (K == 0u || m[d].kj == 0u) { m[d].in_off = 0u; m[d].out_off = 0u; m[d].kj = 0u; }
+        kj3[d] = idn[d] ? 0u : m[d].kj;
+    }
+    const bool maps = (kj3[0] | kj3[1] | kj3[2]) != 0u;
+    unsigned long long bw[4] = {0ull, 0ull, 0ull, 0ull};
+    if (maps && gl < W) {
+        bw[0] = bits[(size_t)i * W + gl];
+#pragma unroll
+        for (uint32_t d = 0; d < 3; ++d) if (kj3[d]) bw[d + 1] = bits[(size_t)nb[d] * W + gl];
+    }
+    if (gl == 0u && q < n_fast) {
+        NodeDesc nd;
+        nd.rec = K ? REC_BASE + ro : 0u; nd.id = i; nd.kk = K;
+#pragma unroll
+        for (uint32_t d = 0; d < 3; ++d) {
+            const uint32_t flag_low = (d < deg && col_n[d] < col_i) ? 1u : 0u, flag_ident = (m[d].kj && idn[d]) ? 1u : 0u;
+            nd.in_off[d] = m[d].in_off | flag_low; nd.out_off[d] = m[d].out_off | flag_ident; nd.kk |= m[d].kj << (8 + 8 * d); nd.nbr[d] = nb[d];
+        }
+        desc[q] = nd;
+    }
+    if (K == 0u) return;
+    const bool w8 = ci == 1u;
+    const uint32_t rs = w8 ? 8u : 8u << ci, none_byte = w8 ? 64u : (ci < 3u ? 4u * rs : 0xFFu);
+    const uint32_t lmask = w8 ? 7u : 3u, lshift = w8 ? 3u : 2u;
+    uint32_t* out = rec + REC_BASE + ro;
+    const uint32_t K4 = (K + 3u) & ~3u;
+    for (uint32_t t = 4u * gl; t < K4; t += 64) {
+        const uint32_t n = min(K - t, 4u);
+        const uint64_t at = (uint64_t)p0 + t;
+        uint32_t v[4]; float c[4];
+        ld_views4(view_id, at, n, nnz, v);
+        if (at + 4u <= nnz) { const float4 cc = ld_unaligned<float4>(cost + at); c[0] = cc.x; c[1] = cc.y; c[2] = cc.z; c[3] = cc.w; }
+        else {
+#pragma unroll
+            for (uint32_t r = 0; r < 4; ++r) c[r] = (r < n) ? cost[at + r] : 0.0f;
+        }
+        uint4 w;
+        w.x = (cost_code(c[0]) << 16) | v[0];
+        w.y = (n > 1u) ? (cost_code(c[1]) << 16) | v[1] : 0u;
+        w.z = (n > 2u) ? (cost_code(c[2]) << 16) | v[2] : 0u;
+        w.w = (n > 3u) ? (cost_code(c[3]) << 16) | v[3] : 0u;
+        *reinterpret_cast<uint4*>(out + t) = w;
+    }
+    uint32_t pos = K4;
+    if (maps) {
+        unsigned long long (*t_bits)[BITMAP_MAX_WORDS] = s_bits[threadIdx.x >> 4];
+        uint32_t (*t_pre)[BITMAP_MAX_WORDS] = s_pre[threadIdx.x >> 4];
+#pragma unroll
+        for (uint32_t b = 0; b < 4; ++b) bitmap_to_tile(bw[b], gl, t_bits[b], t_pre[b]);
+        __builtin_amdgcn_fence(__ATOMIC_ACQ_REL, "wavefront");
+#pragma unroll
+        for (uint32_t d = 0; d < 3; ++d) {
+            const uint32_t kj = kj3[d];
+            if (kj == 0u) continue;
+            const uint32_t nw = w8 ? 2u * ((kj + 7u) >> 3) : (kj + 3u) >> 2;
+            for (uint32_t wI = gl; wI < nw; wI += 16) {
+                const uint32_t n = 4u * wI;
+                uint32_t word = none_byte * 0x01010101u;
+                if (n < kj) {
+                    uint32_t w = 0u;
+                    for (uint32_t ww = 1u; ww < W; ++ww) w = (t_pre[d + 1][ww] <= n) ? ww : w;
+                    unsigned long long x = t_bits[d + 1][w];
+                    x &= ~bitmap_below(bitmap_select(x, n - t_pre[d + 1][w]));
+                    word = 0u;
+#pragma unroll
+                    for (uint32_t r = 0; r < 4; ++r) {
+                        uint32_t byte = none_byte;
+                        if (n + r < kj) {
+                            while (x == 0ull && w + 1u < W) { ++w; x = t_bits[d + 1][w]; }
+                            if (x != 0ull) {
+                                const uint32_t p = (uint32_t)__builtin_ctzll(x);
+                                x &= x - 1ull;
+                                const uint32_t at = bitmap_rank_word(t_bits[0][w], t_pre[0][w], p);
+                                if (at != BITMAP_NONE) byte = (at & lmask) * rs + (at >> lshift);
+                            }
+                        }
+                        word |= byte << (8 * r);
+                    }
+                }
+                out[pos + wI] = word;
+            }
+            pos += nw;
+        }
+    }
+    for (uint32_t t = pos + gl; t < ((pos + 3u) & ~3u); t += 16) out[t] = 0u;
+}
+__global__ void __launch_bounds__(256) mrf_map_bits_kernel(const uint32_t* __restrict__ col_ptr, const uint16_t* __restrict__ view_id, const uint32_t* __restrict__ adj_ptr,
+                                                           const uint32_t* __restrict__ adj, uint32_t F, const MrfEdge* __restrict__ edge, const uint8_t* __restrict__ cls,
+                                                           const unsigned long long* __restrict__ bits, uint32_t W, uint16_t* __restrict__ map) {
+    __shared__ unsigned long long s_bits[16][BITMAP_MAX_WORDS];
+    __shared__ uint32_t s_pre[16][BITMAP_MAX_WORDS];
+    const uint32_t i = (blockIdx.x * blockDim.x + threadIdx.x) >> 4;
+    const uint32_t gl = threadIdx.x & 15;
+    if (i >= F) return;
+    unsigned long long* t_bits = s_bits[threadIdx.x >> 4];
+    uint32_t* t_pre = s_pre[threadIdx.x >> 4];
+    const uint32_t p0 = col_ptr[i], K = col_ptr[i + 1] - p0;
+    for (uint32_t e = adj_ptr[i]; e < adj_ptr[i + 1]; ++e) {
+        const MrfEdge m = edge[e];
+        const uint32_t j = adj[e];
+        if (m.kj == 0 || cls[j] != CLS_GENERIC) continue;
+        __builtin_amdgcn_fence(__ATOMIC_ACQ_REL, "wavefront");
+        bitmap_to_tile(gl < W ? bits[(size_t)j * W + gl] : 0ull, gl, t_bits, t_pre);
+        __builtin_amdgcn_fence(__ATOMIC_ACQ_REL, "wavefront");
+        for (uint32_t t = gl; t < K; t += 16) {
+            const uint32_t v = view_id[p0 + t], w = v >> 6;
+            const uint32_t at = (w < W) ? bitmap_rank_word(t_bits[w], t_pre[w], v) : BITMAP_NONE;
+            map[m.in_off + t] = (at != BITMAP_NONE) ? (uint16_t)at : MAP_NONE;
+        }
+    }
 }
 
 template <int G, bool DAMP, bool XCD>
@@ -1073,6 +1269,12 @@
     MVS_HIP(hipMemsetAsync(ctx->m_size.p, 0, ((size_t)E + 2) * sizeof(uint32_t), s));
     const unsigned nb = (F + 255) / 256;
     const uint32_t force_generic = (ctx->csr_nnz < 4 || E == 0 || ctx->mrf_force_generic) ? 1u : 0u;
+    const uint32_t W = bitmap_words(ctx->csr_views);
+    bool bitmaps = F && W >= 1 && W <= BITMAP_MAX_WORDS && !ctx->mrf_force_lists;
+    if (bitmaps) {
+        ctx->m_bits.ensure((size_t)F * W + 1);
+        hipLaunchKernelGGL(mrf_bitmap_kernel, dim3((unsigned)(((size_t)F * 16 + 255) / 256)), dim3(256), 0, s, ctx->r_ptr, ctx->r_view, (uint64_t)ctx->csr_nnz, F, ctx->csr_views, W, ctx->m_bits.p, maxes + 3); MVS_LAUNCH_CHECK();
+    }
     ctx->m_cls.ensure((size_t)F + 4);
     ctx->m_rev.ensure((size_t)E + 2);
     if (F) { hipLaunchKernelGGL(mrf_size_kernel, dim3(nb), dim3(256), 0, s, ctx->r_ptr, ctx->r_adj_ptr, ctx->r_adj, F, RUN_PAD_MASK, force_generic, ctx->m_size.p, ctx->m_cls.p, maxes, ctx->m_rev.p); MVS_LAUNCH_CHECK(); }
@@ -1124,29 +1326,38 @@
         hipLaunchKernelGGL(mrf_inoff_kernel, dim3(nb), dim3(256), 0, s, ctx->m_perm.p, ctx->m_colour.p, ctx->r_adj_ptr, ctx->r_adj, ctx->m_size.p, ctx->m_rev.p, ctx->m_tmp_b.p, F, n_col, in_off.p); MVS_LAUNCH_CHECK();
         MVS_HIP(hipMemcpyAsync(maxes + 2, ctx->m_tmp_b.p + (n_ent - 1), sizeof(uint32_t), hipMemcpyDeviceToDevice, s));
     } else MVS_HIP(hipMemsetAsync(maxes + 2, 0, sizeof(uint32_t), s));
-    { uint32_t hm[3]; read_words(ctx, maxes, hm, 3); h[1] = hm[0]; h[2] = hm[1]; h[0] = hm[2]; }
+    { uint32_t hm[4]; read_words(ctx, maxes, hm, 4); h[1] = hm[0]; h[2] = hm[1]; h[0] = hm[2]; if (hm[3]) bitmaps = false; }
+    ctx->m_bitmaps = bitmaps;
+    const unsigned long long* bits = bitmaps ? ctx->m_bits.p : nullptr;
     ctx->m_total = (uint64_t)MSG_BASE + h[0]; ctx->m_kmax = h[1]; ctx->m_degmax = h[2];
     if (ctx->m_total >= 0xFFFFFFF0ull) throw StatusError(MVS_ERR_UNSUPPORTED, "message array exceeds 2^32 elements");
-    if (F) { hipLaunchKernelGGL(mrf_edge_kernel, dim3(nb), dim3(256), 0, s, ctx->r_ptr, ctx->r_adj_ptr, ctx->r_adj, F, in_off.p, ctx->m_size.p, ctx->m_rev.p, ctx->m_edge.p); MVS_LAUNCH_CHECK(); }
     ctx->m_ident.ensure((size_t)E + 1);
-    MVS_HIP(hipMemsetAsync(ctx->m_ident.p, 0, (size_t)E + 1, s));
+    if (!bitmaps) MVS_HIP(hipMemsetAsync(ctx->m_ident.p, 0, (size_t)E + 1, s));
+    if (F) { hipLaunchKernelGGL(mrf_edge_kernel, dim3(nb), dim3(256), 0, s, ctx->r_ptr, ctx->r_adj_ptr, ctx->r_adj, F, in_off.p, ctx->m_size.p, ctx->m_rev.p, ctx->m_edge.p, ctx->m_cls.p, bits, W, ctx->m_ident.p); MVS_LAUNCH_CHECK(); }
     const uint32_t n_fast = ctx->m_n_fast, n_generic = F - n_fast;
     if (n_fast) {
         const size_t rec_cap = (size_t)REC_BASE + ctx->csr_nnz + 8 * (size_t)F + ctx->m_total / 4 + (size_t)ctx->m_n_adj + 1024;
         ctx->m_rec.ensure(rec_cap);
         MVS_HIP(hipMemsetAsync(ctx->m_rec.p, 0, REC_BASE * sizeof(uint32_t), s));
-        hipLaunchKernelGGL(mrf_ident_kernel, dim3((unsigned)(((size_t)F * 16 + 255) / 256)), dim3(256), 0, s, ctx->r_ptr, ctx->r_view, ctx->r_adj_ptr, ctx->r_adj, F, ctx->m_edge.p, ctx->m_cls.p, ctx->m_ident.p); MVS_LAUNCH_CHECK();
+        if (!bitmaps) { hipLaunchKernelGGL(mrf_ident_kernel, dim3((unsigned)(((size_t)F * 16 + 255) / 256)), dim3(256), 0, s, ctx->r_ptr, ctx->r_view, ctx->r_adj_ptr, ctx->r_adj, F, ctx->m_edge.p, ctx->m_cls.p, ctx->m_ident.p); MVS_LAUNCH_CHECK(); }
         uint32_t* rsz = ctx->m_tmp_a.p; uint32_t* roff = ctx->m_tmp_b.p;
         hipLaunchKernelGGL(mrf_recsize_kernel, dim3((F + 256) / 256), dim3(256), 0, s, ctx->r_ptr, ctx->r_adj_ptr, ctx->m_edge.p, ctx->m_ident.p, ctx->m_cls.p, ctx->m_perm.p, F, rsz, ctx->m_tmp_c.p); MVS_LAUNCH_CHECK();
         exclusive_scan_u32(ctx, rsz, roff, (size_t)F + 1, nullptr);
-        hipLaunchKernelGGL(mrf_record_kernel, dim3((unsigned)(((size_t)F * 16 + 255) / 256)), dim3(256), 0, s, ctx->r_ptr, ctx->r_view, ctx->r_cost, ctx->r_adj_ptr, ctx->r_adj,
-                           ctx->m_edge.p, ctx->m_ident.p, ctx->m_cls.p, ctx->m_tmp_c.p , roff, F, ctx->m_rec.p); MVS_LAUNCH_CHECK();
         ctx->m_desc.ensure((size_t)F + 1);
-        hipLaunchKernelGGL(mrf_desc_kernel, dim3((n_fast + 255) / 256), dim3(256), 0, s, ctx->r_ptr, ctx->r_adj_ptr, ctx->r_adj, ctx->m_edge.p, ctx->m_ident.p, ctx->m_perm.p, ctx->m_colour.p, roff, n_fast, ctx->m_desc.p); MVS_LAUNCH_CHECK();
+        if (bitmaps) {
+            hipLaunchKernelGGL(mrf_record_bits_kernel, dim3((unsigned)(((size_t)F * 16 + 255) / 256)), dim3(256), 0, s, ctx->r_ptr, ctx->r_view, ctx->r_cost, ctx->r_adj_ptr, ctx->r_adj,
+                               ctx->m_edge.p, ctx->m_ident.p, ctx->m_cls.p, ctx->m_tmp_c.p , roff, ctx->m_colour.p, bits, W, (uint64_t)ctx->csr_nnz, F, n_fast, ctx->m_rec.p, ctx->m_desc.p); MVS_LAUNCH_CHECK();
+        } else {
+            hipLaunchKernelGGL(mrf_record_kernel, dim3((unsigned)(((size_t)F * 16 + 255) / 256)), dim3(256), 0, s, ctx->r_ptr, ctx->r_view, ctx->r_cost, ctx->r_adj_ptr, ctx->r_adj,
+                               ctx->m_edge.p, ctx->m_ident.p, ctx->m_cls.p, ctx->m_tmp_c.p , roff, F, ctx->m_rec.p); MVS_LAUNCH_CHECK();
+            hipLaunchKernelGGL(mrf_desc_kernel, dim3((n_fast + 255) / 256), dim3(256), 0, s, ctx->r_ptr, ctx->r_adj_ptr, ctx->r_adj, ctx->m_edge.p, ctx->m_ident.p, ctx->m_perm.p, ctx->m_colour.p, roff, n_fast, ctx->m_desc.p); MVS_LAUNCH_CHECK();
+        }
     }
     if (n_generic) {
         ctx->m_map.ensure(ctx->m_total + 8);
-        hipLaunchKernelGGL(mrf_map_kernel, dim3((unsigned)(((size_t)F * 16 + 255) / 256)), dim3(256), 0, s, ctx->r_ptr, ctx->r_view, ctx->r_adj_ptr, ctx->r_adj, F, ctx->m_edge.p, ctx->m_cls.p, ctx->m_map.p); MVS_LAUNCH_CHECK();
+        if (bitmaps) hipLaunchKernelGGL(mrf_map_bits_kernel, dim3((unsigned)(((size_t)F * 16 + 255) / 256)), dim3(256), 0, s, ctx->r_ptr, ctx->r_view, ctx->r_adj_ptr, ctx->r_adj, F, ctx->m_edge.p, ctx->m_cls.p, bits, W, ctx->m_map.p);
+        else hipLaunchKernelGGL(mrf_map_kernel, dim3((unsigned)(((size_t)F * 16 + 255) / 256)), dim3(256), 0, s, ctx->r_ptr, ctx->r_view, ctx->r_adj_ptr, ctx->r_adj, F, ctx->m_edge.p, ctx->m_cls.p, ctx->m_map.p);
+        MVS_LAUNCH_CHECK();
         ctx->pq.ensure(ctx->csr_nnz + 1);
     }
     ctx->m_msg_a.ensure(ctx->m_total + 1024);
diff --git a/mvs-texturing_amd/csrc/mgpu.hip b/mvs-texturing_amd/csrc/mgpu.hip
--- a/mvs-texturing_amd/csrc/mgpu.hip
+++ b/mvs-texturing_amd/csrc/mgpu.hip
@@ -158,6 +158,29 @@
     mrf_sweep_phase(ctx, phase, nb0, ne0, part);
     MVS_API_END
 }
+mvs_status mvs_ctx_mrf_setup_tables(mvs_ctx* ctx, int which, void* out_host, uint64_t cap_bytes, uint64_t* n_bytes) {
+    if (!ctx || !n_bytes || which < 0 || which > 3) return api_fail(MVS_ERR_INVALID, "bad argument");
+    if (!ctx->m_state.p) return api_fail(MVS_ERR_STATE, "mrf setup first");
+    MVS_API_BEGIN
+    const uint32_t F = ctx->csr_faces, n_fast = ctx->m_n_fast;
+    const void* src = nullptr; uint64_t n = 0, route = ctx->m_bitmaps ? 1u : 0u;
+    if (which == 0) { n = sizeof(route); }
+    else if (which == 1 && n_fast) {
+        uint32_t words = 0;
+        MVS_HIP(hipMemcpyAsync(&words, ctx->m_tmp_b.p + F, sizeof(uint32_t), hipMemcpyDeviceToHost, ctx->stream));
+        MVS_HIP(hipStreamSynchronize(ctx->stream));
+        src = ctx->m_rec.p; n = ((uint64_t)MRF_REC_BASE + words) * sizeof(uint32_t);
+    }
+    else if (which == 2 && n_fast) { src = ctx->m_desc.p; n = (uint64_t)n_fast * sizeof(NodeDesc); }
+    else if (which == 3) { src = ctx->m_ident.p; n = ctx->m_n_adj; }
+    *n_bytes = n;
+    if (out_host && n) {
+        if (cap_bytes < n) throw StatusError(MVS_ERR_INVALID, "setup tables: buffer too small");
+        if (which == 0) memcpy(out_host, &route, sizeof(route));
+        else { MVS_HIP(hipMemcpyAsync(out_host, src, n, hipMemcpyDeviceToHost, ctx->stream)); MVS_HIP(hipStreamSynchronize(ctx->stream)); }
+    }
+    MVS_API_END
+}
 mvs_status mvs_ctx_mrf_layout(mvs_ctx* ctx, uint32_t* in_off_host, uint64_t n_edges) {
     if (!ctx || (n_edges && !in_off_host)) return api_fail(MVS_ERR_INVALID, "null argument");
     MVS_API_BEGIN
diff --git a/mvs-texturing_amd/viewsel.py b/mvs-texturing_amd/viewsel.py
--- a/mvs-texturing_amd/viewsel.py
+++ b/mvs-texturing_amd/viewsel.py
@@ -142,7 +142,7 @@
     "mvs_ctx_dc_get_max", "mvs_ctx_dc_set_max", "mvs_ctx_dc_get_histogram", "mvs_ctx_dc_set_histogram", "mvs_ctx_costs_export",
     "mvs_ctx_mrf_setup", "mvs_ctx_mrf_setup_marked", "mvs_ctx_mrf_sweep", "mvs_ctx_mrf_sweep_phase", "mvs_ctx_mrf_sweep_phase_part", "mvs_ctx_mrf_layout", "mvs_ctx_mrf_gather", "mvs_ctx_mrf_scatter",
     "mvs_ctx_mrf_energy", "mvs_ctx_mrf_keep_best", "mvs_ctx_mrf_step", "mvs_ctx_mrf_poll", "mvs_ctx_mrf_icm_gain", "mvs_ctx_mrf_icm_apply",
-    "mvs_ctx_mrf_labels"))
+    "mvs_ctx_mrf_labels", "mvs_ctx_mrf_setup_tables"))
 
 
 _lib = None
@@ -196,6 +196,7 @@
         "mvs_ctx_mrf_step": [vp, vp], "mvs_ctx_mrf_poll": [vp, u32, C.POINTER(MrfProgress)],
         "mvs_ctx_mrf_icm_gain": [vp, u32, u32], "mvs_ctx_mrf_icm_apply": [vp, u32, u32, vp],
         "mvs_ctx_mrf_labels": [vp, u32, u32, vp, C.POINTER(u32)],
+        "mvs_ctx_mrf_setup_tables": [vp, i32, vp, u64, C.POINTER(u64)],
         "mvs_ctx_prune_labels": [vp, u32], "mvs_undistort_image": [vp, C.c_int32, C.c_int32, C.c_float, C.c_float, C.c_float, vp],
         "mvs_postprocess_face_infos": [u32, u32, vp, vp, vp, vp, C.POINTER(Settings), C.POINTER(CCsr), C.POINTER(DcStats)],
         "mvs_comm_unique_id": [vp], "mvs_comm_create_rccl": [i32, i32, i32, vp, C.POINTER(vp)], "mvs_comm_create_local": [i32, C.POINTER(vp)], "mvs_comm_create_local_devices": [i32, vp, C.POINTER(vp)],
@@ -441,6 +442,18 @@
         return labels_out, _stats_dict(ms)
 
 
+    def mrf_setup_tables(self):
+        out = {}
+        for which, key, dt in ((0, "bitmaps", np.uint64), (1, "rec", np.uint32), (2, "desc", np.uint32), (3, "ident", np.uint8)):
+            n = C.c_uint64(0)
+            _check(self.L, self.L.mvs_ctx_mrf_setup_tables(self.h, which, None, 0, C.byref(n)))
+            buf = np.zeros(n.value // np.dtype(dt).itemsize, dtype=dt)
+            if n.value:
+                _check(self.L, self.L.mvs_ctx_mrf_setup_tables(self.h, which, buf.ctypes.data_as(C.c_void_p), n.value, C.byref(n)))
+            out[key] = buf
+        out["bitmaps"] = bool(out["bitmaps"][0]); out["desc"] = out["desc"].reshape(-1, 12)
+        return out
+
     def mrf_diagnostics(self):
         out = (C.c_uint32 * 4)()
         _check(self.L, self.L.mvs_ctx_mrf_diagnostics(self.h, out))
```

Measured after the change: 77.51 million faces/s, median of 6. +1.4%, better.
